# enoche/MMRec

Hardware: AMD Instinct MI355X
Metric: GCN-layer edges/sec (3-layer user-item CSR SpMM, d=64, fp32) (higher is better)
Workload: dtype f32

## Files before the change

### include/mmrec_hip.h

```cpp
#ifndef MMREC_HIP_H
#define MMREC_HIP_H

#include <stddef.h>
#include <stdint.h>

#ifdef __cplusplus
extern "C" {
#endif

#define MMREC_ABI_VERSION 16
#define MMREC_EMB_DIM 64

#define MMREC_ERR_BAD_ARG 10001
#define MMREC_ERR_UNSUPPORTED 10002

typedef void* mmrec_stream_t;

int mmrec_abi_version(void);
const char* mmrec_error_string(int err);

#ifndef MMREC_SPMM_CHUNK
#define MMREC_SPMM_CHUNK 512
#endif
#define MMREC_SPMM_LONG_ROW_DEFAULT 32

int mmrec_spmm_csr_f32(const int32_t* rowptr, const int32_t* colidx, const float* vals,
                       const float* X, float* Y, const float* Z, const float* acc_in, float* acc_out,
                       int32_t n_rows, int32_t d, float alpha, float beta, float acc_scale,
                       int32_t long_row_threshold, const int32_t* long_rows,
                       const int32_t* long_chunk_ptr, int32_t n_long, int32_t n_chunks,
                       float* partials, int32_t* long_tickets, mmrec_stream_t stream);

int mmrec_spmm_rows_f32(const int32_t* rowptr, const int32_t* colidx, const float* vals, const float* X,
                        const float* Z, int32_t z_compact, const int64_t* rows, int32_t n_list, int32_t d,
                        int32_t long_row_threshold, float* Y, mmrec_stream_t stream);
int mmrec_spmm_rows_any_f32(const int32_t* rowptr, const int32_t* colidx, const float* vals, const float* X,
                            const float* Z, int32_t z_compact, const int64_t* rows, int32_t n_list, int32_t d,
                            int32_t long_row_threshold, int32_t max_row_chunks, float* Y, mmrec_stream_t stream);
int mmrec_spmm_push_rows_f32(const int32_t* rowptr, const int32_t* colidx, const float* vals, const float* G,
                             float g_scale, const int64_t* rows, int32_t n_list, int32_t d, float* dX, float* dZ,
                             mmrec_stream_t stream);

int mmrec_spmm_csr_f32_layergcn(const int32_t* rowptr, const int32_t* colidx, const float* vals, const float* X,
                                float* Y, const float* ego, float* scaled, float* w, const float* acc_in,
                                float* acc_out, int32_t n_rows, int32_t d, int32_t long_row_threshold,
                                const int32_t* long_rows, const int32_t* long_chunk_ptr, int32_t n_long,
                                int32_t n_chunks, float* partials, int32_t* long_tickets, mmrec_stream_t stream);
int mmrec_spmm_csr_sched_f32(const int32_t* rowptr, const int32_t* colidx, const float* vals, const float* X, float* Y,
                             const float* Z, const float* acc_in, float* acc_out, int32_t n_rows, int32_t d, float alpha,
                             float beta, float acc_scale, int32_t long_row_threshold, const int32_t* long_rows,
                             const int32_t* long_chunk_ptr, int32_t n_long, int32_t n_chunks, float* partials,
                             int32_t* long_tickets, const int32_t* sched_row, const int32_t* sched_span,
                             const int32_t* sched_col, const float* sched_val, int32_t n_short, mmrec_stream_t stream);
int mmrec_spmm_csr_sched_f32_layergcn(const int32_t* rowptr, const int32_t* colidx, const float* vals, const float* X,
                                      float* Y, const float* ego, float* scaled, float* w, const float* acc_in,
                                      float* acc_out, int32_t n_rows, int32_t d, int32_t long_row_threshold,
                                      const int32_t* long_rows, const int32_t* long_chunk_ptr, int32_t n_long,
                                      int32_t n_chunks, float* partials, int32_t* long_tickets, const int32_t* sched_row,
                                      const int32_t* sched_span, const int32_t* sched_col, const float* sched_val,
                                      int32_t n_short, mmrec_stream_t stream);
int mmrec_spmm_row_keys(const int32_t* rowptr, const int32_t* colidx, const int32_t* col_degree, int32_t n_rows,
                        int32_t long_row_threshold, int32_t key_deg_max, int32_t* key, int32_t* key_degree,
                        mmrec_stream_t stream);
int mmrec_spmm_plan_count(const int32_t* rowptr_host, int32_t n_rows, int32_t long_row_threshold,
                          int32_t* n_long, int32_t* n_chunks);
int mmrec_spmm_plan_fill(const int32_t* rowptr_host, int32_t n_rows, int32_t long_row_threshold,
                         int32_t* long_rows, int32_t* long_chunk_ptr);

int mmrec_cos_scale_fwd_f32(const float* E, const float* Ego, float* Out, float* w, float* acc,
                            int32_t n_rows, int32_t d, mmrec_stream_t stream);
int mmrec_cos_scale_bwd_f32(const float* dOut, const float* E, const float* Ego, const float* w,
                            float* dE, float* dEgo_accum, int32_t n_rows, int32_t d,
                            mmrec_stream_t stream);

#define MMREC_BPR_LOGSIG 0
#define MMREC_BPR_GAMMA 1

size_t mmrec_bpr_workspace_bytes(int32_t batch);
int mmrec_bpr_fwd_f32(const float* U, const float* P, const float* N, const int64_t* users,
                      const int64_t* pos, const int64_t* neg, int32_t batch, int32_t d,
                      int32_t variant, float scale, float* loss_out, float* coef, void* workspace,
                      mmrec_stream_t stream);
int mmrec_bpr_bwd_f32(const float* U, const float* P, const float* N, const int64_t* users,
                      const int64_t* pos, const int64_t* neg, int32_t batch, int32_t d,
                      const float* coef, const float* grad_scalar, float scale, float* dU, float* dP,
                      float* dN, mmrec_stream_t stream);

int mmrec_bpr_dots_f32(const float* U, const float* P, const float* N, const int64_t* users,
                       const int64_t* pos, const int64_t* neg, int32_t batch, int32_t d, float* dots,
                       mmrec_stream_t stream);
int mmrec_bpr_loss_from_dots_f32(const float* dots, int32_t batch, int32_t variant, float scale,
                                 float* loss_out, float* coef, void* workspace, mmrec_stream_t stream);

int mmrec_gather_sqnorm_fwd_f32(const float* E, const int64_t* ids, int32_t batch, int32_t d,
                                float* out, void* workspace, mmrec_stream_t stream);
int mmrec_gather_scale_add_bwd_f32(const float* E, const int64_t* ids, int32_t batch, int32_t d,
                                   const float* coef_scalar, float* dE, mmrec_stream_t stream);
#define MMREC_ROWS_REG_MAX_TERMS 6
size_t mmrec_rows_reg_workspace_bytes(int32_t n_terms, int32_t max_batch);
int mmrec_rows_reg_fwd_f32(const float* const* E, const int64_t* const* ids, const int32_t* batch, int32_t n_terms, int32_t d,
                           int32_t mode, float scale, float* out, float* coef, void* workspace, mmrec_stream_t stream);
int mmrec_rows_reg_bwd_f32(const float* const* E, const int64_t* const* ids, const int32_t* batch, int32_t n_terms, int32_t d,
                           const float* coef, const float* g, float* const* dE, mmrec_stream_t stream);

#define MMREC_BPR_MAX_TERMS 4
size_t mmrec_bpr_multi_workspace_bytes(int32_t n_terms, int32_t batch);
int mmrec_bpr_multi_fwd_f32(const float* U, const int64_t* users, const float* const* I, const int64_t* const* pos,
                            const int64_t* const* neg, const float* w, int32_t n_terms, int32_t batch, int32_t d, int32_t variant,
                            float scale, float* total, float* losses, float* coef, void* workspace, mmrec_stream_t stream);
int mmrec_bpr_multi_bwd_f32(const float* U, const int64_t* users, const float* const* I, const int64_t* const* pos,
                            const int64_t* const* neg, const float* w, int32_t n_terms, int32_t batch, int32_t d, const float* coef,
                            const float* grad_scalar, float scale, float* dU, float* const* dI, mmrec_stream_t stream);

#define MMREC_COSINE_MAX_TERMS 8
size_t mmrec_cosine_multi_workspace_bytes(int32_t n_terms, int32_t max_batch);
int mmrec_cosine_multi_fwd_f32(const float* const* X, const int64_t* const* ix, const float* const* Y, const int64_t* const* iy,
                               const float* w, const int32_t* batch, int32_t n_terms, int32_t d, float* out, float* coef,
                               void* workspace, mmrec_stream_t stream);
int mmrec_cosine_multi_bwd_f32(const float* const* X, const int64_t* const* ix, const float* const* Y, const int64_t* const* iy,
                               const float* w, const int32_t* batch, int32_t n_terms, int32_t d, const float* coef,
                               const float* grad_scalar, float* const* dX, mmrec_stream_t stream);

int mmrec_row_normalize_fwd_f32(const float* X, int64_t n, int32_t d, float eps, float* Y, float* inv, mmrec_stream_t stream);
int mmrec_row_normalize_bwd_f32(const float* Y, const float* G, const float* inv, int64_t n, int32_t d, float* dX,
                                mmrec_stream_t stream);

int mmrec_cat_leaky_fwd_f32(const float* A, const float* B, const float* R, int64_t n, int32_t wa, int32_t wb, float slope,
                            float* out, mmrec_stream_t stream);
int mmrec_cat_leaky_bwd_f32(const float* A, const float* B, const float* dOut, int64_t n, int32_t wa, int32_t wb, float slope,
                            float* dA, float* dB, float* dR, mmrec_stream_t stream);


size_t mmrec_infonce_workspace_bytes(int32_t batch);
int mmrec_infonce_fwd_f32(const float* E1, const float* E2, const int64_t* ids, int32_t batch,
                          int32_t d, float tau, float* loss, void* workspace, mmrec_stream_t stream);
int mmrec_infonce_bwd_f32(const int64_t* ids, int32_t batch, int32_t d, float tau,
                          const float* grad_loss, float* dE1, float* dE2, void* workspace,
                          mmrec_stream_t stream);

size_t mmrec_linear_workspace_bytes(int32_t n, int32_t F, int32_t out);
int mmrec_linear_fwd_f32(const float* X, const float* W, const float* b, float* Y, int32_t n,
                         int32_t F, int32_t out, void* workspace, mmrec_stream_t stream);
int mmrec_linear_fwd_split_f32(const float* X, const float* W, const float* b, float* Y, int32_t n, int32_t F,
                               int32_t out, void* workspace, mmrec_stream_t stream);
size_t mmrec_linear_bwd_split_workspace_bytes(int32_t n, int32_t F, int32_t out);
int mmrec_linear_bwd_split_f32(const float* dY, const float* X, const float* W, float* dW, float* db, float* dX, int32_t n,
                               int32_t F, int32_t out, void* workspace, mmrec_stream_t stream);
int mmrec_linear_bwd_w_f32(const float* dY, const float* X, float* dW, float* db, int32_t n,
                           int32_t F, int32_t out, void* workspace, mmrec_stream_t stream);
int mmrec_linear_bwd_x_f32(const float* dY, const float* W, float* dX, int32_t n, int32_t F,
                           int32_t out, mmrec_stream_t stream);
size_t mmrec_linear_rows_workspace_bytes(int32_t n, int32_t F, int32_t out);
int mmrec_linear_rows_fwd_f32(const float* T, int64_t n_table, const int64_t* ids, const float* W, const float* b, float* Y,
                              int32_t n, int32_t F, int32_t out, int32_t split, void* workspace, mmrec_stream_t stream);
int mmrec_linear_rows_bwd_f32(const float* dY, const float* T, int64_t n_table, const int64_t* ids, const float* W, float* dW,
                              float* db, float* dX, int32_t n, int32_t F, int32_t out, void* workspace, mmrec_stream_t stream);
int mmrec_gemm_nt_f32(const float* A, const float* B, const float* bias, float* C, int32_t M, int32_t N,
                      int32_t K, int32_t ldc, mmrec_stream_t stream);

int mmrec_edge_dot_f32(const float* A, int64_t n_a, const float* B, int64_t n_b,
                       const int64_t* rows, const int64_t* cols, int64_t n_edges, int32_t d,
                       float* out, mmrec_stream_t stream);
int mmrec_edge_dot_bwd_f32(const float* g, const float* A, int64_t n_a, const float* B, int64_t n_b,
                           const int64_t* rows, const int64_t* cols, int64_t n_edges, int32_t d,
                           float* dA, float* dB, mmrec_stream_t stream);

int32_t mmrec_segment_softmax_group_max(void);
int mmrec_segment_softmax_f32(const int32_t* rowptr, int32_t n_rows, const int64_t* perm, const int32_t* long_rows,
                              int32_t n_long, const float* score, int64_t n_edges, float eps, float* out,
                              mmrec_stream_t stream);
int mmrec_segment_softmax_bwd_f32(const int32_t* rowptr, int32_t n_rows, const int64_t* perm, const int32_t* long_rows,
                                  int32_t n_long, const float* alpha, const float* g, int64_t n_edges, float* ds,
                                  mmrec_stream_t stream);

int32_t mmrec_edge_attention_group_max(void);
int mmrec_edge_attention_f32(const int32_t* rowptr, int32_t n_rows, const int32_t* colidx, const int64_t* perm,
                             const int32_t* long_rows, int32_t n_long, const float* Q, int64_t n_q, const float* KV,
                             int64_t n_kv, int32_t d, int64_t n_edges, float eps, float* Y, float* alpha,
                             mmrec_stream_t stream);

int mmrec_edge_attention_bwd_f32(const int32_t* rowptr, int32_t n_rows, const int32_t* colidx, const int64_t* perm,
                                 const int32_t* long_rows, int32_t n_long, const int32_t* rowptr_t, const int32_t* rowidx_t,
                                 const int64_t* perm_t, const int32_t* long_cols, int32_t n_long_t, const float* Q, int64_t n_q,
                                 const float* KV, int64_t n_kv, const float* Y, const float* alpha, const float* dY,
                                 const float* dAlpha, int32_t d, int64_t n_edges, float* ds, float* dQ, float* dKV,
                                 const float* dKV_base, mmrec_stream_t stream);

#define MMREC_TOPK_MAX 128
#define MMREC_TOPK_MAX_OTHER 64
#define MMREC_TOPK_NO_FILTER 1
size_t mmrec_topk_workspace_bytes(int32_t nq, int32_t nc, int32_t kd, int32_t k);
int mmrec_score_topk_f32(const float* Q, const float* C, int32_t nq, int32_t nc, int32_t kd,
                         const int32_t* mask_rowptr, const int32_t* mask_col, int32_t k,
                         int64_t* out_idx, float* out_val, void* workspace, int32_t flags,
                         mmrec_stream_t stream);
size_t mmrec_topk_prepared_bytes(int32_t nc, int32_t kd);
int mmrec_topk_prepare_f32(const float* C, int32_t nc, int32_t kd, void* prepared, mmrec_stream_t stream);
int mmrec_score_topk_prepared_f32(const float* Q, const float* C, const void* prepared, int32_t nq, int32_t nc,
                                  int32_t kd, const int32_t* mask_rowptr, const int32_t* mask_col, int32_t k,
                                  int64_t* out_idx, float* out_val, void* workspace, int32_t flags,
                                  mmrec_stream_t stream);
#define MMREC_TOPK_HINT_COLD 1
#define MMREC_TOPK_HINT_KEEP 2
int mmrec_score_topk_hinted_f32(const float* Q, const float* C, const void* prepared, int32_t nq, int32_t nc,
                                int32_t kd, const int32_t* mask_rowptr, const int32_t* mask_col, int32_t k,
                                int32_t* hint, int32_t hint_k, const int64_t* hint_rows,
                                int64_t* out_idx, float* out_val, void* workspace, int32_t* queue_counts,
                                int32_t flags, mmrec_stream_t stream);

int mmrec_scatter_add_rows_sorted_f32(const int64_t* order, const int64_t* ids, const float* rows, int32_t n, int32_t d,
                                      float* out, mmrec_stream_t stream);

int mmrec_degree_count_i32(const int64_t* ids, int64_t n, int32_t* counts, int32_t n_bins,
                           mmrec_stream_t stream);
int mmrec_edge_norm_f32(const int64_t* eu, const int64_t* ei, int64_t n_edges, const int32_t* deg_u,
                        const int32_t* deg_i, float* val, mmrec_stream_t stream);
int mmrec_bipartite_expand(const int64_t* eu, const int64_t* ei, const float* w, int64_t n_edges,
                           int32_t n_users, int32_t* rows, int32_t* cols, float* vals,
                           mmrec_stream_t stream);
size_t mmrec_coo_to_csr_workspace_bytes(int64_t nnz, int32_t n_rows);
int mmrec_coo_to_csr(const int32_t* rows, const int32_t* cols, const float* vals, int64_t nnz,
                     int32_t n_rows, int32_t* rowptr, int32_t* colidx, float* vals_out,
                     void* workspace, mmrec_stream_t stream);

int mmrec_sample_negatives_i64(const int64_t* users, int32_t batch, const int32_t* hist_rowptr,
                               const int32_t* hist_col, const int32_t* cand_items, int32_t n_cand,
                               uint64_t seed, uint64_t counter, int64_t* out_neg,
                               mmrec_stream_t stream);
int mmrec_topk_metrics_f64(const int64_t* topk_idx, int32_t n_users, int32_t k,
                           const int32_t* gt_rowptr, const int32_t* gt_col, const double* discount,
                           const double* idcg_cum, const int32_t* ks, int32_t n_ks, uint8_t* hit_out,
                           double* out_per_user, mmrec_stream_t stream);

int mmrec_adam_step_f32(float* p, const float* g, float* m, float* v, int64_t n, float lr, float beta1,
                        float beta2, float eps, float weight_decay, int64_t step,
                        mmrec_stream_t stream);

int mmrec_adam_prepare(int64_t* step_dev, const float* lr_dev, float beta1, float beta2, float* hyper_dev,
                       mmrec_stream_t stream);
int mmrec_adam_step_dev_f32(float* p, const float* g, float* m, float* v, int64_t n, const float* hyper_dev,
                            float beta1, float beta2, float eps, float weight_decay,
                            mmrec_stream_t stream);

int mmrec_adam_multi_step_f32(float* const* p, const float* const* g, float* const* m, float* const* v,
                              const int64_t* n, int32_t n_tensors, const float* lr, const int64_t* step,
                              float beta1, float beta2, float eps, float weight_decay, mmrec_stream_t stream);
int mmrec_adam_multi_step_dev_f32(float* const* p, const float* const* g, float* const* m, float* const* v,
                                  const int64_t* n, int32_t n_tensors, const float* hyper_dev, float beta1,
                                  float beta2, float eps, float weight_decay, mmrec_stream_t stream);

int mmrec_host_sample_negatives(uint32_t* mt_state, int32_t* mt_index, const int64_t* users, int32_t batch,
                                const int64_t* hist_rowptr, const int64_t* hist_items, const int64_t* all_items,
                                int32_t n_all_items, int64_t* out);

int mmrec_host_random_sample_range(uint32_t* mt_state, int32_t* mt_index, int32_t n, int32_t k, int64_t* out,
                                   int32_t* scratch);

size_t mmrec_cosine_workspace_bytes(int32_t batch);
int mmrec_cosine_fwd_f32(const float* X, const int64_t* ix, const float* Y, const int64_t* iy, int32_t batch, int32_t d,
                         float scale, float* out, float* coef, void* workspace, mmrec_stream_t stream);
int mmrec_cosine_bwd_f32(const float* X, const int64_t* ix, const float* Y, const int64_t* iy, int32_t batch, int32_t d,
                         const float* coef, const float* grad_scalar, float scale, float* dX, mmrec_stream_t stream);

#define MMREC_ADAM_ROWS_MAX_IDS 16000
int mmrec_adam_hist_set(float* hist, int32_t t, float lr, float beta1, float beta2, mmrec_stream_t stream);
int mmrec_adam_rows_owner(const int64_t* ids, int32_t n, int32_t* owner, mmrec_stream_t stream);
int mmrec_adam_rows_catchup_f32(float* p, float* m, float* v, const int64_t* ids, int32_t* owner, int32_t n_ids,
                                int32_t n_rows, int32_t F, int32_t* last_step, const float* hist, int32_t t_now,
                                float beta1, float beta2, float eps, float weight_decay, mmrec_stream_t stream);
int mmrec_adam_rows_step_f32(float* p, float* m, float* v, const int64_t* ids, int32_t* owner, const float* g,
                             int32_t n_ids, int32_t F, int32_t* last_step, int32_t t, float lr, float beta1,
                             float beta2, float eps, float weight_decay, int32_t presummed, mmrec_stream_t stream);
int mmrec_adam_hist_set_dev(float* hist, int32_t capacity, const int64_t* step_dev, const float* hyper_dev,
                            int32_t* overflow, mmrec_stream_t stream);
int mmrec_adam_rows_catchup_dev_f32(float* p, float* m, float* v, const int64_t* ids, int32_t* owner, int32_t n_ids,
                                    int32_t n_rows, int32_t F, int32_t* last_step, const float* hist, int32_t capacity,
                                    const int64_t* step_dev, float beta1, float beta2, float eps, float weight_decay,
                                    mmrec_stream_t stream);
int mmrec_adam_rows_step_dev_f32(float* p, float* m, float* v, const int64_t* ids, int32_t* owner, const float* g,
                                 int32_t n_ids, int32_t F, int32_t* last_step, int32_t capacity, const int64_t* step_dev,
                                 const float* hyper_dev, float beta1, float beta2, float eps, float weight_decay,
                                 int32_t presummed, mmrec_stream_t stream);
int mmrec_adam_rows_fastforward_f32(float* p, float* m, float* v, const int64_t* ids, int32_t* owner, int32_t n_ids,
                                    int32_t n_rows, int32_t F, int32_t* last_step, const float* hist, int32_t t_now,
                                    float beta1, float beta2, float eps, float weight_decay, mmrec_stream_t stream);
int mmrec_adam_rows_fastforward_dev_f32(float* p, float* m, float* v, const int64_t* ids, int32_t* owner, int32_t n_ids,
                                        int32_t n_rows, int32_t F, int32_t* last_step, const float* hist,
                                        int32_t capacity, const int64_t* step_dev, float beta1, float beta2, float eps,
                                        float weight_decay, mmrec_stream_t stream);

#ifdef __cplusplus
}
#endif
#endif
```

### mmrec_amd/_lib.py

```python
from __future__ import annotations

import ctypes
import os
from ctypes import c_char_p, c_float, c_int32, c_int64, c_size_t, c_uint64, c_void_p

import torch

_PKG = os.path.dirname(os.path.abspath(__file__))
LIB_PATH = os.environ.get("MMREC_HIP_LIB") or os.path.join(_PKG, "lib", "libmmrec_hip.so")
ABI_VERSION = 16

_P = c_void_p

SIGNATURES = {
    "mmrec_abi_version": (c_int32, []),
    "mmrec_error_string": (c_char_p, [c_int32]),
    "mmrec_spmm_csr_f32": (c_int32, [_P, _P, _P, _P, _P, _P, _P, _P, c_int32, c_int32, c_float,
                                     c_float, c_float, c_int32, _P, _P, c_int32, c_int32, _P, _P, _P]),
    "mmrec_spmm_csr_f32_layergcn": (c_int32, [_P, _P, _P, _P, _P, _P, _P, _P, _P, _P, c_int32, c_int32, c_int32,
                                              _P, _P, c_int32, c_int32, _P, _P, _P]),
    "mmrec_spmm_csr_sched_f32": (c_int32, [_P, _P, _P, _P, _P, _P, _P, _P, c_int32, c_int32, c_float,
                                           c_float, c_float, c_int32, _P, _P, c_int32, c_int32, _P, _P,
                                           _P, _P, _P, _P, c_int32, _P]),
    "mmrec_spmm_csr_sched_f32_layergcn": (c_int32, [_P, _P, _P, _P, _P, _P, _P, _P, _P, _P, c_int32, c_int32, c_int32,
                                                    _P, _P, c_int32, c_int32, _P, _P, _P, _P, _P, _P, c_int32, _P]),
    "mmrec_spmm_row_keys": (c_int32, [_P, _P, _P, c_int32, c_int32, c_int32, _P, _P, _P]),
    "mmrec_spmm_plan_count": (c_int32, [_P, c_int32, c_int32, _P, _P]),
    "mmrec_spmm_plan_fill": (c_int32, [_P, c_int32, c_int32, _P, _P]),
    "mmrec_cos_scale_fwd_f32": (c_int32, [_P, _P, _P, _P, _P, c_int32, c_int32, _P]),
    "mmrec_cos_scale_bwd_f32": (c_int32, [_P, _P, _P, _P, _P, _P, c_int32, c_int32, _P]),
    "mmrec_bpr_workspace_bytes": (c_size_t, [c_int32]),
    "mmrec_bpr_fwd_f32": (c_int32, [_P, _P, _P, _P, _P, _P, c_int32, c_int32, c_int32, c_float, _P,
                                    _P, _P, _P]),
    "mmrec_spmm_rows_f32": (c_int32, [_P, _P, _P, _P, _P, c_int32, _P, c_int32, c_int32, c_int32, _P, _P]),
    "mmrec_spmm_rows_any_f32": (c_int32, [_P, _P, _P, _P, _P, c_int32, _P, c_int32, c_int32, c_int32, c_int32, _P, _P]),
    "mmrec_spmm_push_rows_f32": (c_int32, [_P, _P, _P, _P, c_float, _P, c_int32, c_int32, _P, _P, _P]),
    "mmrec_bpr_dots_f32": (c_int32, [_P, _P, _P, _P, _P, _P, c_int32, c_int32, _P, _P]),
    "mmrec_bpr_loss_from_dots_f32": (c_int32, [_P, c_int32, c_int32, c_float, _P, _P, _P, _P]),
    "mmrec_bpr_bwd_f32": (c_int32, [_P, _P, _P, _P, _P, _P, c_int32, c_int32, _P, _P, c_float, _P, _P,
                                    _P, _P]),
    "mmrec_gather_sqnorm_fwd_f32": (c_int32, [_P, _P, c_int32, c_int32, _P, _P, _P]),
    "mmrec_gather_scale_add_bwd_f32": (c_int32, [_P, _P, c_int32, c_int32, _P, _P, _P]),
    "mmrec_infonce_workspace_bytes": (c_size_t, [c_int32]),
    "mmrec_infonce_fwd_f32": (c_int32, [_P, _P, _P, c_int32, c_int32, c_float, _P, _P, _P]),
    "mmrec_infonce_bwd_f32": (c_int32, [_P, c_int32, c_int32, c_float, _P, _P, _P, _P, _P]),
    "mmrec_linear_workspace_bytes": (c_size_t, [c_int32, c_int32, c_int32]),
    "mmrec_linear_fwd_f32": (c_int32, [_P, _P, _P, _P, c_int32, c_int32, c_int32, _P, _P]),
    "mmrec_linear_fwd_split_f32": (c_int32, [_P, _P, _P, _P, c_int32, c_int32, c_int32, _P, _P]),
    "mmrec_linear_bwd_split_workspace_bytes": (c_size_t, [c_int32, c_int32, c_int32]),
    "mmrec_linear_bwd_split_f32": (c_int32, [_P, _P, _P, _P, _P, _P, c_int32, c_int32, c_int32, _P, _P]),
    "mmrec_linear_bwd_w_f32": (c_int32, [_P, _P, _P, _P, c_int32, c_int32, c_int32, _P, _P]),
    "mmrec_linear_bwd_x_f32": (c_int32, [_P, _P, _P, c_int32, c_int32, c_int32, _P]),
    "mmrec_linear_rows_workspace_bytes": (c_size_t, [c_int32, c_int32, c_int32]),
    "mmrec_linear_rows_fwd_f32": (c_int32, [_P, c_int64, _P, _P, _P, _P, c_int32, c_int32, c_int32, c_int32, _P, _P]),
    "mmrec_linear_rows_bwd_f32": (c_int32, [_P, _P, c_int64, _P, _P, _P, _P, _P, c_int32, c_int32, c_int32, _P, _P]),
    "mmrec_edge_dot_f32": (c_int32, [_P, c_int64, _P, c_int64, _P, _P, c_int64, c_int32, _P, _P]),
    "mmrec_edge_dot_bwd_f32": (c_int32, [_P, _P, c_int64, _P, c_int64, _P, _P, c_int64, c_int32, _P, _P, _P]),
    "mmrec_segment_softmax_group_max": (c_int32, []),
    "mmrec_segment_softmax_f32": (c_int32, [_P, c_int32, _P, _P, c_int32, _P, c_int64, c_float, _P, _P]),
    "mmrec_segment_softmax_bwd_f32": (c_int32, [_P, c_int32, _P, _P, c_int32, _P, _P, c_int64, _P, _P]),
    "mmrec_edge_attention_group_max": (c_int32, []),
    "mmrec_edge_attention_f32": (c_int32, [_P, c_int32, _P, _P, _P, c_int32, _P, c_int64, _P, c_int64, c_int32, c_int64, c_float,
                                           _P, _P, _P]),
    "mmrec_edge_attention_bwd_f32": (c_int32, [_P, c_int32, _P, _P, _P, c_int32, _P, _P, _P, _P, c_int32, _P, c_int64, _P, c_int64,
                                               _P, _P, _P, _P, c_int32, c_int64, _P, _P, _P, _P, _P]),
    "mmrec_gemm_nt_f32": (c_int32, [_P, _P, _P, _P, c_int32, c_int32, c_int32, c_int32, _P]),
    "mmrec_topk_workspace_bytes": (c_size_t, [c_int32, c_int32, c_int32, c_int32]),
    "mmrec_score_topk_f32": (c_int32, [_P, _P, c_int32, c_int32, c_int32, _P, _P, c_int32, _P, _P, _P,
                                       c_int32, _P]),
    "mmrec_scatter_add_rows_sorted_f32": (c_int32, [_P, _P, _P, c_int32, c_int32, _P, _P]),
    "mmrec_topk_prepared_bytes": (c_size_t, [c_int32, c_int32]),
    "mmrec_topk_prepare_f32": (c_int32, [_P, c_int32, c_int32, _P, _P]),
    "mmrec_score_topk_prepared_f32": (c_int32, [_P, _P, _P, c_int32, c_int32, c_int32, _P, _P, c_int32, _P, _P, _P,
                                                c_int32, _P]),
    "mmrec_score_topk_hinted_f32": (c_int32, [_P, _P, _P, c_int32, c_int32, c_int32, _P, _P, c_int32, _P, c_int32, _P,
                                              _P, _P, _P, _P, c_int32, _P]),
    "mmrec_degree_count_i32": (c_int32, [_P, c_int64, _P, c_int32, _P]),
    "mmrec_edge_norm_f32": (c_int32, [_P, _P, c_int64, _P, _P, _P, _P]),
    "mmrec_bipartite_expand": (c_int32, [_P, _P, _P, c_int64, c_int32, _P, _P, _P, _P]),
    "mmrec_coo_to_csr_workspace_bytes": (c_size_t, [c_int64, c_int32]),
    "mmrec_coo_to_csr": (c_int32, [_P, _P, _P, c_int64, c_int32, _P, _P, _P, _P, _P]),
    "mmrec_sample_negatives_i64": (c_int32, [_P, c_int32, _P, _P, _P, c_int32, c_uint64, c_uint64, _P, _P]),
    "mmrec_topk_metrics_f64": (c_int32, [_P, c_int32, c_int32, _P, _P, _P, _P, _P, c_int32, _P, _P, _P]),
    "mmrec_adam_step_f32": (c_int32, [_P, _P, _P, _P, c_int64, c_float, c_float, c_float, c_float, c_float,
                                      c_int64, _P]),
    "mmrec_adam_prepare": (c_int32, [_P, _P, c_float, c_float, _P, _P]),
    "mmrec_adam_step_dev_f32": (c_int32, [_P, _P, _P, _P, c_int64, _P, c_float, c_float, c_float, c_float, _P]),
    "mmrec_adam_multi_step_f32": (c_int32, [_P, _P, _P, _P, _P, c_int32, _P, _P, c_float, c_float, c_float,
                                            c_float, _P]),
    "mmrec_adam_multi_step_dev_f32": (c_int32, [_P, _P, _P, _P, _P, c_int32, _P, c_float, c_float, c_float,
                                                c_float, _P]),
    "mmrec_host_sample_negatives": (c_int32, [_P, _P, _P, c_int32, _P, _P, _P, c_int32, _P]),
    "mmrec_host_random_sample_range": (c_int32, [_P, _P, c_int32, c_int32, _P, _P]),
    "mmrec_cosine_workspace_bytes": (c_size_t, [c_int32]),
    "mmrec_cosine_fwd_f32": (c_int32, [_P, _P, _P, _P, c_int32, c_int32, c_float, _P, _P, _P, _P]),
    "mmrec_cosine_bwd_f32": (c_int32, [_P, _P, _P, _P, c_int32, c_int32, _P, _P, c_float, _P, _P]),
    "mmrec_bpr_multi_workspace_bytes": (c_size_t, [c_int32, c_int32]),
    "mmrec_bpr_multi_fwd_f32": (c_int32, [_P, _P, _P, _P, _P, _P, c_int32, c_int32, c_int32, c_int32, c_float, _P, _P, _P, _P, _P]),
    "mmrec_bpr_multi_bwd_f32": (c_int32, [_P, _P, _P, _P, _P, _P, c_int32, c_int32, c_int32, _P, _P, c_float, _P, _P, _P]),
    "mmrec_cosine_multi_workspace_bytes": (c_size_t, [c_int32, c_int32]),
    "mmrec_cosine_multi_fwd_f32": (c_int32, [_P, _P, _P, _P, _P, _P, c_int32, c_int32, _P, _P, _P, _P]),
    "mmrec_cosine_multi_bwd_f32": (c_int32, [_P, _P, _P, _P, _P, _P, c_int32, c_int32, _P, _P, _P, _P]),
    "mmrec_row_normalize_fwd_f32": (c_int32, [_P, c_int64, c_int32, c_float, _P, _P, _P]),
    "mmrec_row_normalize_bwd_f32": (c_int32, [_P, _P, _P, c_int64, c_int32, _P, _P]),
    "mmrec_cat_leaky_fwd_f32": (c_int32, [_P, _P, _P, c_int64, c_int32, c_int32, c_float, _P, _P]),
    "mmrec_cat_leaky_bwd_f32": (c_int32, [_P, _P, _P, c_int64, c_int32, c_int32, c_float, _P, _P, _P, _P]),
    "mmrec_rows_reg_workspace_bytes": (c_size_t, [c_int32, c_int32]),
    "mmrec_rows_reg_fwd_f32": (c_int32, [_P, _P, _P, c_int32, c_int32, c_int32, c_float, _P, _P, _P, _P]),
    "mmrec_rows_reg_bwd_f32": (c_int32, [_P, _P, _P, c_int32, c_int32, _P, _P, _P, _P]),
    "mmrec_adam_hist_set": (c_int32, [_P, c_int32, c_float, c_float, c_float, _P]),
    "mmrec_adam_rows_owner": (c_int32, [_P, c_int32, _P, _P]),
    "mmrec_adam_rows_catchup_f32": (c_int32, [_P, _P, _P, _P, _P, c_int32, c_int32, c_int32, _P, _P, c_int32, c_float,
                                              c_float, c_float, c_float, _P]),
    "mmrec_adam_rows_step_f32": (c_int32, [_P, _P, _P, _P, _P, _P, c_int32, c_int32, _P, c_int32, c_float, c_float,
                                           c_float, c_float, c_float, c_int32, _P]),
    "mmrec_adam_hist_set_dev": (c_int32, [_P, c_int32, _P, _P, _P, _P]),
    "mmrec_adam_rows_catchup_dev_f32": (c_int32, [_P, _P, _P, _P, _P, c_int32, c_int32, c_int32, _P, _P, c_int32, _P, c_float,
                                                  c_float, c_float, c_float, _P]),
    "mmrec_adam_rows_step_dev_f32": (c_int32, [_P, _P, _P, _P, _P, _P, c_int32, c_int32, _P, c_int32, _P, _P, c_float, c_float,
                                               c_float, c_float, c_int32, _P]),
    "mmrec_adam_rows_fastforward_f32": (c_int32, [_P, _P, _P, _P, _P, c_int32, c_int32, c_int32, _P, _P, c_int32, c_float,
                                                  c_float, c_float, c_float, _P]),
    "mmrec_adam_rows_fastforward_dev_f32": (c_int32, [_P, _P, _P, _P, _P, c_int32, c_int32, c_int32, _P, _P, c_int32, _P,
                                                      c_float, c_float, c_float, c_float, _P]),
}

_lib = None


class MMRecHipError(RuntimeError):
    pass


def load():
    global _lib
    if _lib is not None:
        return _lib
    if not os.path.exists(LIB_PATH):
        raise MMRecHipError(
            "libmmrec_hip.so not found at %s: run `python -m mmrec_amd.build`; there is no CPU or "
            "eager fallback for the hot path" % LIB_PATH)
    lib = ctypes.CDLL(LIB_PATH)
    for name, (res, args) in SIGNATURES.items():
        fn = getattr(lib, name)
        fn.restype = res
        fn.argtypes = args
    got = lib.mmrec_abi_version()
    if got != ABI_VERSION:
        raise MMRecHipError("libmmrec_hip.so ABI %d != expected %d: rebuild" % (got, ABI_VERSION))
    _lib = lib
    return lib


def check(err: int, what: str):
    if err != 0:
        msg = load().mmrec_error_string(int(err))
        raise MMRecHipError("%s failed: [%d] %s" % (what, err, msg.decode() if msg else "?"))
```

### mmrec_amd/csrc/spmm.hip

```cpp
#include "common.h"
#include "spmm_narrow.h"

#ifndef MMREC_SPMM_RPG
#define MMREC_SPMM_RPG(n_rows) ((n_rows) <= (1 << 18) ? 1 : 4)
#endif

namespace {

__device__ __forceinline__ void st_coherent(float4* p, float4 v) {
    unsigned long long* q = reinterpret_cast<unsigned long long*>(p);
    const unsigned long long lo = ((unsigned long long)__float_as_uint(v.y) << 32) | __float_as_uint(v.x);
    const unsigned long long hi = ((unsigned long long)__float_as_uint(v.w) << 32) | __float_as_uint(v.z);
    __hip_atomic_store(q, lo, __ATOMIC_RELAXED, __HIP_MEMORY_SCOPE_AGENT);
    __hip_atomic_store(q + 1, hi, __ATOMIC_RELAXED, __HIP_MEMORY_SCOPE_AGENT);
}
__device__ __forceinline__ float4 ld_coherent(const float4* p) {
    unsigned long long* q = reinterpret_cast<unsigned long long*>(const_cast<float4*>(p));
    const unsigned long long lo = __hip_atomic_load(q, __ATOMIC_RELAXED, __HIP_MEMORY_SCOPE_AGENT);
    const unsigned long long hi = __hip_atomic_load(q + 1, __ATOMIC_RELAXED, __HIP_MEMORY_SCOPE_AGENT);
    return make_float4(__uint_as_float((unsigned)lo), __uint_as_float((unsigned)(lo >> 32)),
                       __uint_as_float((unsigned)hi), __uint_as_float((unsigned)(hi >> 32)));
}

struct RowEpilogue {
    const float* Z;
    float* Y;
    const float* acc_in;
    float* acc_out;
    float alpha, beta, acc_scale;
    const float* ego;
    float* scaled;
    float* w_out;
};

struct RowSchedule {
    const int32_t* row;
    const int2* span;
    const int32_t* col;
    const float* val;
    int n_short;
};

template <int DCH, bool LG>
__device__ __forceinline__ void store_row(const RowEpilogue& ep, int row, int lane16, const float4 (&sum)[DCH]) {
    if (DCH == 1 && LG) {
        const size_t off = (size_t)row * 16 + lane16;
        const float4 y = f4_scale(ep.alpha, sum[0]);
        const float4 g = reinterpret_cast<const float4*>(ep.ego)[off];
        const float dot = row16_sum(f4_dot(y, g));
        const float ne = fmaxf(sqrtf(row16_sum(f4_dot(y, y))), 1e-8f);
        const float ng = fmaxf(sqrtf(row16_sum(f4_dot(g, g))), 1e-8f);
        const float w = dot / (ne * ng);
        const float4 o = f4_scale(w, y);
        if (ep.Y) reinterpret_cast<float4*>(ep.Y)[off] = y;
        reinterpret_cast<float4*>(ep.scaled)[off] = o;
        if (lane16 == 0) ep.w_out[row] = w;
        if (ep.acc_out)
            reinterpret_cast<float4*>(ep.acc_out)[off] =
                ep.acc_in ? f4_add(reinterpret_cast<const float4*>(ep.acc_in)[off], o) : o;
        return;
    }
#pragma unroll
    for (int ch = 0; ch < DCH; ++ch) {
        const size_t off = (size_t)row * (16 * DCH) + ch * 16 + lane16;
        float4 y = f4_scale(ep.alpha, sum[ch]);
        if (ep.Z) y = f4_fma(ep.beta, reinterpret_cast<const float4*>(ep.Z)[off], y);
        if (ep.Y) reinterpret_cast<float4*>(ep.Y)[off] = y;
        if (ep.acc_out) {
            const float4 a = reinterpret_cast<const float4*>(ep.acc_in)[off];
            reinterpret_cast<float4*>(ep.acc_out)[off] = f4_scale(ep.acc_scale, f4_add(a, y));
        }
    }
}

template <int DCH>
__device__ __forceinline__ void gather_span(const int32_t* __restrict__ colidx,
                                            const float* __restrict__ vals,
                                            const float4* __restrict__ X4, int s, int e, int lane16,
                                            float4 (&acc)[DCH]) {
    constexpr int NB = DCH == 1 ? 8 : (DCH <= 2 ? 4 : (DCH <= 4 ? 2 : 1));
    for (int base = s; base < e; base += 16) {
        const int k = base + lane16;
        int c = 0;
        float v = 0.f;
        if (k < e) {
            c = colidx[k];
            v = vals[k];
        }
        const int cnt = min(16, e - base);
        for (int j0 = 0; j0 < cnt; j0 += NB) {
            float4 x[NB][DCH];
            float vv[NB];
#pragma unroll
            for (int u = 0; u < NB; ++u) {
                const int j = j0 + u;
                const int cj = __shfl(c, j, 16);
                vv[u] = __shfl(v, j, 16);
#pragma unroll
                for (int ch = 0; ch < DCH; ++ch)
                    x[u][ch] = (j < cnt) ? X4[(size_t)cj * (16 * DCH) + ch * 16 + lane16] : f4_zero();
            }
#pragma unroll
            for (int u = 0; u < NB; ++u)
#pragma unroll
                for (int ch = 0; ch < DCH; ++ch) acc[ch] = f4_fma(vv[u], x[u][ch], acc[ch]);
        }
    }
}

template <int DCH, bool COHERENT, bool LG>
__device__ __forceinline__ void reduce_long_row(const float* __restrict__ partials, int c0, int c1, int row,
                                                const RowEpilogue& ep, float4 (*red)[16 * DCH]) {
    const int lane16 = threadIdx.x & 15, g = threadIdx.x >> 4;
#pragma unroll
    for (int ch = 0; ch < DCH; ++ch) {
        float4 t = f4_zero();
        for (int c = c0 + g; c < c1; c += 16) {
            const float4* src = reinterpret_cast<const float4*>(partials) + (size_t)c * (16 * DCH) + ch * 16 + lane16;
            t = f4_add(t, COHERENT ? ld_coherent(src) : *src);
        }
        red[g][ch * 16 + lane16] = t;
    }
    __syncthreads();
    if (g == 0) {
        float4 r[DCH];
#pragma unroll
        for (int ch = 0; ch < DCH; ++ch) {
            r[ch] = red[0][ch * 16 + lane16];
#pragma unroll
            for (int k = 1; k < 16; ++k) r[ch] = f4_add(r[ch], red[k][ch * 16 + lane16]);
        }
        store_row<DCH, LG>(ep, row, lane16, r);
    }
}

template <int DCH, bool LG, bool SCHED>
__global__ __launch_bounds__(256) void spmm_rows_kernel(
    const int32_t* __restrict__ rowptr, const int32_t* __restrict__ colidx,
    const float* __restrict__ vals, const float* __restrict__ X, RowEpilogue ep, int n_rows,
    int long_t, int rows_per_group, const int32_t* __restrict__ long_rows,
    const int32_t* __restrict__ long_chunk_ptr, int n_long, int n_chunks,
    float* __restrict__ partials, int32_t* __restrict__ tickets, RowSchedule sched) {
    __shared__ float4 red[16][16 * DCH];
    __shared__ int s_last;
    const int lane16 = threadIdx.x & 15;
    const int g = threadIdx.x >> 4;
    const float4* X4 = reinterpret_cast<const float4*>(X);
    if ((int)blockIdx.x < n_chunks) {
        const int chunk = blockIdx.x;
        int lo = 0, hi = n_long;
        while (hi - lo > 1) {
            const int mid = (lo + hi) >> 1;
            if (long_chunk_ptr[mid] <= chunk) lo = mid; else hi = mid;
        }
        const int row = long_rows[lo];
        const int cs = rowptr[row] + (chunk - long_chunk_ptr[lo]) * MMREC_SPMM_CHUNK;
        const int ce = min(cs + MMREC_SPMM_CHUNK, rowptr[row + 1]);
        float4 acc[DCH];
#pragma unroll
        for (int ch = 0; ch < DCH; ++ch) acc[ch] = f4_zero();
        for (int base = cs + g * 16; base < ce; base += 256)
            gather_span<DCH>(colidx, vals, X4, base, min(base + 16, ce), lane16, acc);
#pragma unroll
        for (int ch = 0; ch < DCH; ++ch) red[g][ch * 16 + lane16] = acc[ch];
        __syncthreads();
        if (g == 0) {
            float4 t[DCH];
#pragma unroll
            for (int ch = 0; ch < DCH; ++ch) {
                t[ch] = red[0][ch * 16 + lane16];
#pragma unroll
                for (int i = 1; i < 16; ++i) t[ch] = f4_add(t[ch], red[i][ch * 16 + lane16]);
            }
            if (long_chunk_ptr[lo + 1] - long_chunk_ptr[lo] == 1) {
                store_row<DCH, LG>(ep, row, lane16, t);
            } else {
#pragma unroll
                for (int ch = 0; ch < DCH; ++ch) {
                    float4* dst = reinterpret_cast<float4*>(partials) + (size_t)chunk * (16 * DCH) + ch * 16 + lane16;
                    if (tickets) st_coherent(dst, t[ch]); else *dst = t[ch];
                }
            }
        }
        const int c0 = long_chunk_ptr[lo], c1 = long_chunk_ptr[lo + 1];
        if (!tickets || c1 - c0 == 1) return;
        if (threadIdx.x < 64) {
            __atomic_signal_fence(__ATOMIC_SEQ_CST);
            __builtin_amdgcn_s_waitcnt(0);
            __atomic_signal_fence(__ATOMIC_SEQ_CST);
            __builtin_amdgcn_fence(__ATOMIC_RELEASE, "workgroup");
            if (threadIdx.x == 0)
                s_last = __hip_atomic_fetch_add(tickets + lo, 1, __ATOMIC_RELAXED, __HIP_MEMORY_SCOPE_AGENT) == c1 - c0 - 1;
        }
        __syncthreads();
        if (!s_last) return;
        __builtin_amdgcn_fence(__ATOMIC_ACQUIRE, "workgroup");
        reduce_long_row<DCH, true, LG>(partials, c0, c1, row, ep, red);
        if (threadIdx.x == 0) __hip_atomic_store(tickets + lo, 0, __ATOMIC_RELAXED, __HIP_MEMORY_SCOPE_AGENT);
        return;
    }
    if (SCHED) {
        const int slot0 = ((int)blockIdx.x - n_chunks) * 16 * rows_per_group + g;
#pragma unroll 1
        for (int i = 0; i < rows_per_group; ++i) {
            const int slot = slot0 + i * 16;
            if (slot >= sched.n_short) break;
            const int row = sched.row[slot];
            const int2 se = sched.span[slot];
            float4 acc[DCH];
#pragma unroll
            for (int ch = 0; ch < DCH; ++ch) acc[ch] = f4_zero();
            gather_span<DCH>(sched.col, sched.val, X4, se.x, se.y, lane16, acc);
            store_row<DCH, LG>(ep, row, lane16, acc);
        }
        return;
    }
    const int row0 = ((int)blockIdx.x - n_chunks) * 16 * rows_per_group + g;
#pragma unroll 1
    for (int i = 0; i < rows_per_group; ++i) {
        const int row = row0 + i * 16;
        if (row >= n_rows) break;
        const int s = rowptr[row], e = rowptr[row + 1];
        if (e - s > long_t) continue;
        float4 acc[DCH];
#pragma unroll
        for (int ch = 0; ch < DCH; ++ch) acc[ch] = f4_zero();
        gather_span<DCH>(colidx, vals, X4, s, e, lane16, acc);
        store_row<DCH, LG>(ep, row, lane16, acc);
    }
}

template <int DCH, bool LG>
__global__ __launch_bounds__(256) void spmm_long_reduce_kernel(
    const int32_t* __restrict__ long_rows, const int32_t* __restrict__ long_chunk_ptr, int n_long,
    const float* __restrict__ partials, RowEpilogue ep) {
    __shared__ float4 red[16][16 * DCH];
    const int i = blockIdx.x;
    const int c0 = long_chunk_ptr[i], c1 = long_chunk_ptr[i + 1];
    if (c1 - c0 <= 1) return;
    reduce_long_row<DCH, false, LG>(partials, c0, c1, long_rows[i], ep, red);
}

template <int DCH, bool LG = false, bool SCHED = false>
void launch_spmm(hipStream_t s, int blocks, int nch, const int32_t* rowptr, const int32_t* colidx,
                 const float* vals, const float* X, const RowEpilogue& ep, int n_rows, int long_t,
                 int rows_per_group, const int32_t* long_rows, const int32_t* long_chunk_ptr, int n_long,
                 float* partials, int32_t* tickets, const RowSchedule& sched = RowSchedule{}) {
    if (blocks + nch > 0)
        hipLaunchKernelGGL((spmm_rows_kernel<DCH, LG, SCHED>), dim3(blocks + nch), dim3(256), 0, s, rowptr, colidx, vals, X,
                           ep, n_rows, long_t, rows_per_group, long_rows, long_chunk_ptr, n_long, nch, partials, tickets,
                           sched);
    if (!tickets && n_long > 0 && nch > n_long)
        hipLaunchKernelGGL((spmm_long_reduce_kernel<DCH, LG>), dim3(n_long), dim3(256), 0, s, long_rows,
                           long_chunk_ptr, n_long, partials, ep);
}

__global__ __launch_bounds__(256) void cos_scale_fwd_kernel(const float* __restrict__ E,
                                                            const float* __restrict__ Ego,
                                                            float* __restrict__ Out,
                                                            float* __restrict__ W,
                                                            float* __restrict__ acc, int n_rows) {
    const int lane16 = threadIdx.x & 15;
    const int row = blockIdx.x * 16 + (threadIdx.x >> 4);
    if (row >= n_rows) return;
    const size_t off = (size_t)row * 16 + lane16;
    const float4 e = reinterpret_cast<const float4*>(E)[off];
    const float4 g = reinterpret_cast<const float4*>(Ego)[off];
    const float dot = row16_sum(f4_dot(e, g));
    const float ne = fmaxf(sqrtf(row16_sum(f4_dot(e, e))), 1e-8f);
    const float ng = fmaxf(sqrtf(row16_sum(f4_dot(g, g))), 1e-8f);
    const float w = dot / (ne * ng);
    const float4 o = f4_scale(w, e);
    reinterpret_cast<float4*>(Out)[off] = o;
    if (lane16 == 0) W[row] = w;
    if (acc) reinterpret_cast<float4*>(acc)[off] = f4_add(reinterpret_cast<float4*>(acc)[off], o);
}

__global__ __launch_bounds__(256) void cos_scale_bwd_kernel(
    const float* __restrict__ dOut, const float* __restrict__ E, const float* __restrict__ Ego,
    const float* __restrict__ W, float* __restrict__ dE, float* __restrict__ dEgo, int n_rows) {
    const int lane16 = threadIdx.x & 15;
    const int row = blockIdx.x * 16 + (threadIdx.x >> 4);
    if (row >= n_rows) return;
    const size_t off = (size_t)row * 16 + lane16;
    const float4 e = reinterpret_cast<const float4*>(E)[off];
    const float4 g = reinterpret_cast<const float4*>(Ego)[off];
    const float4 d = reinterpret_cast<const float4*>(dOut)[off];
    const float w = W[row];
    const float ne_raw = sqrtf(row16_sum(f4_dot(e, e)));
    const float ng_raw = sqrtf(row16_sum(f4_dot(g, g)));
    const float ne = fmaxf(ne_raw, 1e-8f), ng = fmaxf(ng_raw, 1e-8f);
    const float dw = row16_sum(f4_dot(d, e));
    const float inv = 1.0f / (ne * ng);
    const float ce = (ne_raw > 1e-8f) ? w / (ne * ne) : 0.f;
    const float cg = (ng_raw > 1e-8f) ? w / (ng * ng) : 0.f;
    float4 de = f4_scale(w, d);
    de = f4_fma(dw * inv, g, de);
    de = f4_fma(-dw * ce, e, de);
    reinterpret_cast<float4*>(dE)[off] = de;
    float4 dg = reinterpret_cast<float4*>(dEgo)[off];
    dg = f4_fma(dw * inv, e, dg);
    dg = f4_fma(-dw * cg, g, dg);
    reinterpret_cast<float4*>(dEgo)[off] = dg;
}

__global__ __launch_bounds__(256) void spmm_row_keys_kernel(const int32_t* __restrict__ rowptr,
                                                            const int32_t* __restrict__ colidx,
                                                            const int32_t* __restrict__ col_degree, int n_rows, int long_t,
                                                            int deg_max, int32_t* __restrict__ key,
                                                            int32_t* __restrict__ key_degree) {
    const int lane16 = threadIdx.x & 15;
    const int row = blockIdx.x * 16 + (threadIdx.x >> 4);
    if (row >= n_rows) return;
    const int s = rowptr[row], e = rowptr[row + 1];
    int bd = 0, bp = INT32_MAX, bc = -1;
    if (e - s <= long_t)
        for (int k = s + lane16; k < e; k += 16) {
            const int c = colidx[k];
            const int dg = col_degree[c];
            if (dg <= deg_max && dg > bd) {
                bd = dg;
                bp = k;
                bc = c;
            }
        }
#pragma unroll
    for (int m = 8; m > 0; m >>= 1) {
        const int od = __shfl_xor(bd, m, 16), op = __shfl_xor(bp, m, 16), oc = __shfl_xor(bc, m, 16);
        if (od > bd || (od == bd && op < bp)) {
            bd = od;
            bp = op;
            bc = oc;
        }
    }
    if (lane16 == 0) {
        key[row] = bc;
        key_degree[row] = bd;
    }
}

}

extern "C" int mmrec_spmm_csr_f32(const int32_t* rowptr, const int32_t* colidx, const float* vals,
                                  const float* X, float* Y, const float* Z, const float* acc_in,
                                  float* acc_out, int32_t n_rows, int32_t d, float alpha, float beta,
                                  float acc_scale, int32_t long_row_threshold,
                                  const int32_t* long_rows, const int32_t* long_chunk_ptr,
                                  int32_t n_long, int32_t n_chunks, float* partials, int32_t* long_tickets,
                                  mmrec_stream_t stream) {
    const bool narrow = d == 8 || d == 16 || d == 32;
    if (!narrow && (d <= 0 || d % MMREC_EMB_DIM || d / MMREC_EMB_DIM > 6)) return MMREC_ERR_UNSUPPORTED;
    if (n_rows < 0 || n_long < 0 || n_chunks < 0 || long_row_threshold < 0) return MMREC_ERR_BAD_ARG;
    if (n_rows == 0) return 0;
    if (!rowptr || !X || (!Y && !acc_out)) return MMREC_ERR_BAD_ARG;
    if (acc_out && !acc_in) return MMREC_ERR_BAD_ARG;
    if (n_long > 0 && (!long_rows || !long_chunk_ptr || !partials || n_chunks <= 0))
        return MMREC_ERR_BAD_ARG;
    if (Y == X || acc_out == X) return MMREC_ERR_BAD_ARG;
    if (narrow)
        return spmm_narrow_launch(rowptr, colidx, vals, X, Y, Z, acc_in, acc_out, n_rows, d, alpha, beta, acc_scale,
                                  n_long > 0 ? long_row_threshold : INT32_MAX, long_rows, long_chunk_ptr, n_long,
                                  n_long > 0 ? n_chunks : 0, partials, mmrec_stream(stream));
    RowEpilogue ep{Z, Y, acc_in, acc_out, alpha, Z ? beta : 0.f, acc_scale, nullptr, nullptr, nullptr};
    hipStream_t s = mmrec_stream(stream);
    const int rows_per_group = MMREC_SPMM_RPG(n_rows);
    const int blocks = (n_rows + 16 * rows_per_group - 1) / (16 * rows_per_group);
    const int long_t = n_long > 0 ? long_row_threshold : INT32_MAX;
    const int nch = n_long > 0 ? n_chunks : 0;
    int32_t* tickets = n_long > 0 ? long_tickets : nullptr;
#define MMREC_SPMM_CASE(D)                                                                               \
    case D:                                                                                              \
        launch_spmm<D>(s, blocks, nch, rowptr, colidx, vals, X, ep, n_rows, long_t, rows_per_group,      \
                       long_rows, long_chunk_ptr, n_long, partials, tickets);                            \
        break;
    switch (d / MMREC_EMB_DIM) {
        MMREC_SPMM_CASE(1) MMREC_SPMM_CASE(2) MMREC_SPMM_CASE(3) MMREC_SPMM_CASE(4) MMREC_SPMM_CASE(5)
        MMREC_SPMM_CASE(6)
    }
#undef MMREC_SPMM_CASE
    MMREC_RETURN_LAUNCH_STATUS();
}

extern "C" int mmrec_spmm_rows_f32(const int32_t* rowptr, const int32_t* colidx, const float* vals, const float* X,
                                   const float* Z, int32_t z_compact, const int64_t* rows, int32_t n_list, int32_t d,
                                   int32_t long_row_threshold, float* Y, mmrec_stream_t stream) {
    if (d != 8 && d != 16 && d != 32 && d != 64) return MMREC_ERR_UNSUPPORTED;
    if (n_list < 0 || long_row_threshold < 0) return MMREC_ERR_BAD_ARG;
    if (n_list == 0) return 0;
    if (!rowptr || !X || !rows || !Y || Y == X) return MMREC_ERR_BAD_ARG;
    return spmm_pull_rows_launch(rowptr, colidx, vals, X, Z, z_compact, rows, n_list, d, long_row_threshold, Y, mmrec_stream(stream));
}

extern "C" int mmrec_spmm_rows_any_f32(const int32_t* rowptr, const int32_t* colidx, const float* vals, const float* X,
                                       const float* Z, int32_t z_compact, const int64_t* rows, int32_t n_list, int32_t d,
                                       int32_t long_row_threshold, int32_t max_row_chunks, float* Y, mmrec_stream_t stream) {
    if (d != 8 && d != 16 && d != 32 && d != 64) return MMREC_ERR_UNSUPPORTED;
    if (n_list < 0 || long_row_threshold < 0 || max_row_chunks < 1) return MMREC_ERR_BAD_ARG;
    if (n_list == 0) return 0;
    if (!rowptr || !X || !rows || !Y || Y == X) return MMREC_ERR_BAD_ARG;
    return spmm_pull_rows_launch(rowptr, colidx, vals, X, Z, z_compact, rows, n_list, d, long_row_threshold, Y, mmrec_stream(stream),
                                 max_row_chunks);
}

extern "C" int mmrec_spmm_push_rows_f32(const int32_t* rowptr, const int32_t* colidx, const float* vals, const float* G,
                                        float g_scale, const int64_t* rows, int32_t n_list, int32_t d, float* dX, float* dZ,
                                        mmrec_stream_t stream) {
    if (d != 8 && d != 16 && d != 32 && d != 64) return MMREC_ERR_UNSUPPORTED;
    if (n_list < 0) return MMREC_ERR_BAD_ARG;
    if (n_list == 0) return 0;
    if (!rowptr || !G || !rows || (!dX && !dZ)) return MMREC_ERR_BAD_ARG;
    return spmm_push_rows_launch(rowptr, colidx, vals, G, g_scale, rows, n_list, d, dX, dZ, mmrec_stream(stream));
}

extern "C" int mmrec_spmm_csr_f32_layergcn(const int32_t* rowptr, const int32_t* colidx, const float* vals,
                                           const float* X, float* Y, const float* ego, float* scaled, float* w,
                                           const float* acc_in, float* acc_out, int32_t n_rows, int32_t d,
                                           int32_t long_row_threshold, const int32_t* long_rows,
                                           const int32_t* long_chunk_ptr, int32_t n_long, int32_t n_chunks,
                                           float* partials, int32_t* long_tickets, mmrec_stream_t stream) {
    if (d != MMREC_EMB_DIM) return MMREC_ERR_UNSUPPORTED;
    if (n_rows < 0 || n_long < 0 || n_chunks < 0 || long_row_threshold < 0) return MMREC_ERR_BAD_ARG;
    if (n_rows == 0) return 0;
    if (!rowptr || !X || !ego || !scaled || !w) return MMREC_ERR_BAD_ARG;
    if (n_long > 0 && (!long_rows || !long_chunk_ptr || !partials || n_chunks <= 0)) return MMREC_ERR_BAD_ARG;
    if (Y == X || scaled == X || acc_out == X) return MMREC_ERR_BAD_ARG;
    RowEpilogue ep{nullptr, Y, acc_in, acc_out, 1.f, 0.f, 1.f, ego, scaled, w};
    hipStream_t s = mmrec_stream(stream);
    const int rows_per_group = MMREC_SPMM_RPG(n_rows);
    const int blocks = (n_rows + 16 * rows_per_group - 1) / (16 * rows_per_group);
    const int long_t = n_long > 0 ? long_row_threshold : INT32_MAX;
    const int nch = n_long > 0 ? n_chunks : 0;
    int32_t* tickets = n_long > 0 ? long_tickets : nullptr;
    launch_spmm<1, true>(s, blocks, nch, rowptr, colidx, vals, X, ep, n_rows, long_t, rows_per_group, long_rows,
                         long_chunk_ptr, n_long, partials, tickets);
    MMREC_RETURN_LAUNCH_STATUS();
}

namespace {
bool sched_args_ok(const int32_t* sched_row, const int32_t* sched_span, const int32_t* sched_col, const float* sched_val,
                   int32_t n_short, int32_t n_rows) {
    if (n_short < 0 || n_short > n_rows) return false;
    return n_short == 0 || (sched_row && sched_span && sched_col && sched_val);
}
}

extern "C" int mmrec_spmm_csr_sched_f32(const int32_t* rowptr, const int32_t* colidx, const float* vals,
                                        const float* X, float* Y, const float* Z, const float* acc_in,
                                        float* acc_out, int32_t n_rows, int32_t d, float alpha, float beta,
                                        float acc_scale, int32_t long_row_threshold,
                                        const int32_t* long_rows, const int32_t* long_chunk_ptr,
                                        int32_t n_long, int32_t n_chunks, float* partials, int32_t* long_tickets,
                                        const int32_t* sched_row, const int32_t* sched_span, const int32_t* sched_col,
                                        const float* sched_val, int32_t n_short, mmrec_stream_t stream) {
    if (d <= 0 || d % MMREC_EMB_DIM || d / MMREC_EMB_DIM > 6) return MMREC_ERR_UNSUPPORTED;
    if (n_rows < 0 || n_long < 0 || n_chunks < 0 || long_row_threshold < 0) return MMREC_ERR_BAD_ARG;
    if (n_rows == 0) return 0;
    if (!rowptr || !X || (!Y && !acc_out)) return MMREC_ERR_BAD_ARG;
    if (acc_out && !acc_in) return MMREC_ERR_BAD_ARG;
    if (n_long > 0 && (!long_rows || !long_chunk_ptr || !partials || n_chunks <= 0))
        return MMREC_ERR_BAD_ARG;
    if (!sched_args_ok(sched_row, sched_span, sched_col, sched_val, n_short, n_rows)) return MMREC_ERR_BAD_ARG;
    if (Y == X || acc_out == X) return MMREC_ERR_BAD_ARG;
    RowEpilogue ep{Z, Y, acc_in, acc_out, alpha, Z ? beta : 0.f, acc_scale, nullptr, nullptr, nullptr};
    const RowSchedule sched{sched_row, reinterpret_cast<const int2*>(sched_span), sched_col, sched_val, n_short};
    hipStream_t s = mmrec_stream(stream);
    const int rows_per_group = MMREC_SPMM_RPG(n_rows);
    const int blocks = (n_short + 16 * rows_per_group - 1) / (16 * rows_per_group);
    const int long_t = n_long > 0 ? long_row_threshold : INT32_MAX;
    const int nch = n_long > 0 ? n_chunks : 0;
    int32_t* tickets = n_long > 0 ? long_tickets : nullptr;
#define MMREC_SPMM_CASE(D)                                                                                      \
    case D:                                                                                                     \
        launch_spmm<D, false, true>(s, blocks, nch, rowptr, colidx, vals, X, ep, n_rows, long_t, rows_per_group, \
                                    long_rows, long_chunk_ptr, n_long, partials, tickets, sched);               \
        break;
    switch (d / MMREC_EMB_DIM) {
        MMREC_SPMM_CASE(1) MMREC_SPMM_CASE(2) MMREC_SPMM_CASE(3) MMREC_SPMM_CASE(4) MMREC_SPMM_CASE(5)
        MMREC_SPMM_CASE(6)
    }
#undef MMREC_SPMM_CASE
    MMREC_RETURN_LAUNCH_STATUS();
}

extern "C" int mmrec_spmm_csr_sched_f32_layergcn(const int32_t* rowptr, const int32_t* colidx, const float* vals,
                                                 const float* X, float* Y, const float* ego, float* scaled, float* w,
                                                 const float* acc_in, float* acc_out, int32_t n_rows, int32_t d,
                                                 int32_t long_row_threshold, const int32_t* long_rows,
                                                 const int32_t* long_chunk_ptr, int32_t n_long, int32_t n_chunks,
                                                 float* partials, int32_t* long_tickets, const int32_t* sched_row,
                                                 const int32_t* sched_span, const int32_t* sched_col,
                                                 const float* sched_val, int32_t n_short, mmrec_stream_t stream) {
    if (d != MMREC_EMB_DIM) return MMREC_ERR_UNSUPPORTED;
    if (n_rows < 0 || n_long < 0 || n_chunks < 0 || long_row_threshold < 0) return MMREC_ERR_BAD_ARG;
    if (n_rows == 0) return 0;
    if (!rowptr || !X || !ego || !scaled || !w) return MMREC_ERR_BAD_ARG;
    if (n_long > 0 && (!long_rows || !long_chunk_ptr || !partials || n_chunks <= 0)) return MMREC_ERR_BAD_ARG;
    if (!sched_args_ok(sched_row, sched_span, sched_col, sched_val, n_short, n_rows)) return MMREC_ERR_BAD_ARG;
    if (Y == X || scaled == X || acc_out == X) return MMREC_ERR_BAD_ARG;
    RowEpilogue ep{nullptr, Y, acc_in, acc_out, 1.f, 0.f, 1.f, ego, scaled, w};
    const RowSchedule sched{sched_row, reinterpret_cast<const int2*>(sched_span), sched_col, sched_val, n_short};
    hipStream_t s = mmrec_stream(stream);
    const int rows_per_group = MMREC_SPMM_RPG(n_rows);
    const int blocks = (n_short + 16 * rows_per_group - 1) / (16 * rows_per_group);
    const int long_t = n_long > 0 ? long_row_threshold : INT32_MAX;
    const int nch = n_long > 0 ? n_chunks : 0;
    int32_t* tickets = n_long > 0 ? long_tickets : nullptr;
    launch_spmm<1, true, true>(s, blocks, nch, rowptr, colidx, vals, X, ep, n_rows, long_t, rows_per_group, long_rows,
                               long_chunk_ptr, n_long, partials, tickets, sched);
    MMREC_RETURN_LAUNCH_STATUS();
}

extern "C" int mmrec_spmm_row_keys(const int32_t* rowptr, const int32_t* colidx, const int32_t* col_degree,
                                   int32_t n_rows, int32_t long_row_threshold, int32_t key_deg_max, int32_t* key,
                                   int32_t* key_degree, mmrec_stream_t stream) {
    if (n_rows < 0 || long_row_threshold < 0 || key_deg_max < 0) return MMREC_ERR_BAD_ARG;
    if (n_rows == 0) return 0;
    if (!rowptr || !colidx || !col_degree || !key || !key_degree) return MMREC_ERR_BAD_ARG;
    hipLaunchKernelGGL(spmm_row_keys_kernel, dim3((n_rows + 15) / 16), dim3(256), 0, mmrec_stream(stream), rowptr, colidx,
                       col_degree, n_rows, long_row_threshold, key_deg_max, key, key_degree);
    MMREC_RETURN_LAUNCH_STATUS();
}

extern "C" int mmrec_spmm_plan_count(const int32_t* rowptr_host, int32_t n_rows,
                                     int32_t long_row_threshold, int32_t* n_long, int32_t* n_chunks) {
    if (!rowptr_host || !n_long || !n_chunks || n_rows < 0) return MMREC_ERR_BAD_ARG;
    int32_t nl = 0, nc = 0;
    for (int32_t r = 0; r < n_rows; ++r) {
        const int32_t deg = rowptr_host[r + 1] - rowptr_host[r];
        if (deg > long_row_threshold) {
            ++nl;
            nc += (deg + MMREC_SPMM_CHUNK - 1) / MMREC_SPMM_CHUNK;
        }
    }
    *n_long = nl;
    *n_chunks = nc;
    return 0;
}

extern "C" int mmrec_spmm_plan_fill(const int32_t* rowptr_host, int32_t n_rows,
                                    int32_t long_row_threshold, int32_t* long_rows,
                                    int32_t* long_chunk_ptr) {
    if (!rowptr_host || !long_rows || !long_chunk_ptr || n_rows < 0) return MMREC_ERR_BAD_ARG;
    int32_t nl = 0, nc = 0;
    for (int32_t r = 0; r < n_rows; ++r) {
        const int32_t deg = rowptr_host[r + 1] - rowptr_host[r];
        if (deg > long_row_threshold) {
            long_rows[nl] = r;
            long_chunk_ptr[nl] = nc;
            ++nl;
            nc += (deg + MMREC_SPMM_CHUNK - 1) / MMREC_SPMM_CHUNK;
        }
    }
    long_chunk_ptr[nl] = nc;
    return 0;
}

extern "C" int mmrec_cos_scale_fwd_f32(const float* E, const float* Ego, float* Out, float* w,
                                       float* acc, int32_t n_rows, int32_t d, mmrec_stream_t stream) {
    if (d != MMREC_EMB_DIM) return MMREC_ERR_UNSUPPORTED;
    if (n_rows < 0 || (n_rows > 0 && (!E || !Ego || !Out || !w))) return MMREC_ERR_BAD_ARG;
    if (n_rows == 0) return 0;
    hipLaunchKernelGGL(cos_scale_fwd_kernel, dim3((n_rows + 15) / 16), dim3(256), 0,
                       mmrec_stream(stream), E, Ego, Out, w, acc, n_rows);
    MMREC_RETURN_LAUNCH_STATUS();
}

extern "C" int mmrec_cos_scale_bwd_f32(const float* dOut, const float* E, const float* Ego,
                                       const float* w, float* dE, float* dEgo_accum, int32_t n_rows,
                                       int32_t d, mmrec_stream_t stream) {
    if (d != MMREC_EMB_DIM) return MMREC_ERR_UNSUPPORTED;
    if (n_rows < 0 || (n_rows > 0 && (!dOut || !E || !Ego || !w || !dE || !dEgo_accum)))
        return MMREC_ERR_BAD_ARG;
    if (n_rows == 0) return 0;
    hipLaunchKernelGGL(cos_scale_bwd_kernel, dim3((n_rows + 15) / 16), dim3(256), 0,
                       mmrec_stream(stream), dOut, E, Ego, w, dE, dEgo_accum, n_rows);
    MMREC_RETURN_LAUNCH_STATUS();
}
```

### mmrec_amd/hip_ops.py

```python
from __future__ import annotations

import ctypes

import numpy as np
import torch

from . import _lib

EMB_DIM = 64
LINEAR_F16X3_DEFAULT = True
LINEAR_F16X3 = LINEAR_F16X3_DEFAULT
SLICE_WIDTHS = (8, 16, 32)
SPMM_CHUNK = 512
LONG_ROW_DEFAULT = None


def default_long_row_threshold(n_cols):
    import os
    forced = os.environ.get("MMREC_LONG_ROW_THRESHOLD")
    if forced:
        return int(forced)
    return 16 if n_cols <= (1 << 18) else 32


ROW_SCHEDULE_MIN_COLS = 1 << 18
SPMM_KEY_DEG_MAX = 128


def spmm_key_deg_max():
    import os
    forced = os.environ.get("MMREC_SPMM_KEY_DEG_MAX")
    return int(forced) if forced else SPMM_KEY_DEG_MAX


TOPK_MAX = 128
BPR_LOGSIG, BPR_GAMMA = 0, 1

DETERMINISTIC_DEFAULT = False
DETERMINISTIC = DETERMINISTIC_DEFAULT
_TORCH_DET_BY_US = False


def set_deterministic(flag=True):
    global DETERMINISTIC, _TORCH_DET_BY_US
    DETERMINISTIC = bool(flag)
    if DETERMINISTIC and not torch.are_deterministic_algorithms_enabled():
        torch.use_deterministic_algorithms(True, warn_only=True)
        _TORCH_DET_BY_US = True
    elif not DETERMINISTIC and _TORCH_DET_BY_US:
        torch.use_deterministic_algorithms(False)
        _TORCH_DET_BY_US = False


def scatter_add_rows(ids, rows, out):
    lib = _lib.load()
    _chk(ids, torch.int64, "ids", 1)
    rows, out = _chk(rows.contiguous(), torch.float32, "rows", 2), _chk(out, torch.float32, "out", 2)
    order = torch.sort(ids, stable=True)[1]
    _lib.check(lib.mmrec_scatter_add_rows_sorted_f32(_p(order), _p(ids), _p(rows), ids.numel(), rows.shape[1], _p(out),
                                                     _stream()), "scatter_add_rows_sorted")
    return out


def _p(t):
    return None if t is None else ctypes.c_void_p(t.data_ptr())


def _stream():
    return ctypes.c_void_p(torch.cuda.current_stream().cuda_stream)


def _chk(t, dtype, name, dim=None):
    if not isinstance(t, torch.Tensor) or not t.is_cuda:
        raise _lib.MMRecHipError("%s must be a device tensor (the hot path has no CPU fallback)" % name)
    if t.dtype != dtype:
        raise _lib.MMRecHipError("%s must be %s, got %s" % (name, dtype, t.dtype))
    if not t.is_contiguous():
        raise _lib.MMRecHipError("%s must be contiguous" % name)
    if dim is not None and t.dim() != dim:
        raise _lib.MMRecHipError("%s must be %d-d" % (name, dim))
    return t


def _ws(nbytes, device):
    return torch.empty(max(int(nbytes), 16), dtype=torch.uint8, device=device)


class CsrGraph:

    def __init__(self, rowptr, colidx, vals, n_rows, n_cols, symmetric=False,
                 long_row_threshold=LONG_ROW_DEFAULT, rowptr_host=None, row_schedule=None):
        self.rowptr = _chk(rowptr, torch.int32, "rowptr", 1)
        self.colidx = _chk(colidx, torch.int32, "colidx", 1)
        self.vals = _chk(vals, torch.float32, "vals", 1)
        self.n_rows, self.n_cols = int(n_rows), int(n_cols)
        self.nnz = int(colidx.numel())
        self.symmetric = bool(symmetric)
        self.long_row_threshold = int(default_long_row_threshold(self.n_cols) if long_row_threshold is None
                                      else long_row_threshold)
        self._t = self if symmetric else None
        self.row_schedule = bool(self.n_cols > ROW_SCHEDULE_MIN_COLS if row_schedule is None else row_schedule)
        self._plan(rowptr_host)

    def _plan(self, rowptr_host):
        lib = _lib.load()
        rp = rowptr_host if rowptr_host is not None else self.rowptr.cpu().numpy()
        rp = np.ascontiguousarray(rp, dtype=np.int32)
        self.rowptr_host = rp
        n_long, n_chunks = ctypes.c_int32(0), ctypes.c_int32(0)
        _lib.check(lib.mmrec_spmm_plan_count(rp.ctypes.data_as(ctypes.c_void_p), self.n_rows,
                                             self.long_row_threshold, ctypes.byref(n_long),
                                             ctypes.byref(n_chunks)), "spmm_plan_count")
        self.n_long, self.n_chunks = n_long.value, n_chunks.value
        dev = self.rowptr.device
        if self.n_long > 0:
            lr = np.empty(self.n_long, dtype=np.int32)
            cp = np.empty(self.n_long + 1, dtype=np.int32)
            _lib.check(lib.mmrec_spmm_plan_fill(rp.ctypes.data_as(ctypes.c_void_p), self.n_rows,
                                                self.long_row_threshold,
                                                lr.ctypes.data_as(ctypes.c_void_p),
                                                cp.ctypes.data_as(ctypes.c_void_p)), "spmm_plan_fill")
            self.long_rows = torch.from_numpy(lr).to(dev)
            self.long_chunk_ptr = torch.from_numpy(cp).to(dev)
            self.max_row_chunks = int(np.diff(cp).max())
            self.long_tickets = torch.zeros(self.n_long, dtype=torch.int32, device=dev)
        else:
            self.long_rows = self.long_chunk_ptr = self.long_tickets = None
            self.max_row_chunks = 1
        self._partials = {}
        self.sched = None
        if self.row_schedule:
            self._plan_schedule()

    def _plan_schedule(self):
        lib = _lib.load()
        dev, n = self.rowptr.device, self.n_rows
        deg = (self.rowptr[1:] - self.rowptr[:-1])
        short = torch.nonzero(deg <= self.long_row_threshold).squeeze(1)
        key = torch.full((n,), -1, dtype=torch.int32, device=dev)
        kdeg = torch.zeros(n, dtype=torch.int32, device=dev)
        if self.nnz > 0 and n > 0:
            if self.symmetric and self.n_cols == n:
                coldeg = deg.contiguous()
            else:
                coldeg = torch.bincount(self.colidx, minlength=self.n_cols).to(torch.int32)
            _lib.check(lib.mmrec_spmm_row_keys(_p(self.rowptr), _p(self.colidx), _p(coldeg), n, self.long_row_threshold,
                                               spmm_key_deg_max(), _p(key), _p(kdeg), _stream()), "spmm_row_keys")
        self.row_key, self.row_key_degree = key, kdeg
        k, kd, dg = key[short].long(), kdeg[short].long(), deg[short].long()
        first = self.colidx[self.rowptr[:-1][short].long().clamp_(max=max(self.nnz - 1, 0))].long() if self.nnz > 0 else k
        ref = torch.where(k >= 0, k, torch.where(dg > 0, first, torch.full_like(k, -1)))
        band = (ref <= short).long()
        comp = (band << 62) | (((1 << 31) - 1 - kd) << 31) | k.clamp(min=0)
        order = torch.sort(comp, stable=True)[1]
        rows = short[order]
        lens = dg[order]
        end = torch.cumsum(lens, 0)
        begin = end - lens
        total = int(end[-1].item()) if rows.numel() else 0
        src0 = self.rowptr[:-1].long()[rows]
        pos = torch.arange(total, dtype=torch.int64, device=dev) + torch.repeat_interleave(src0 - begin, lens, output_size=total)
        self.sched = {
            "row": rows.to(torch.int32).contiguous(),
            "span": torch.stack([begin, end], 1).to(torch.int32).contiguous(),
            "col": self.colidx.index_select(0, pos) if total else torch.zeros(1, dtype=torch.int32, device=dev),
            "val": self.vals.index_select(0, pos) if total else torch.zeros(1, dtype=torch.float32, device=dev),
            "n_short": int(rows.numel()),
            "vals_of": self.vals,
        }

    def scheduled(self, d):
        sc = self.sched
        return sc if sc is not None and d % EMB_DIM == 0 and sc["vals_of"] is self.vals else None

    def schedule_bytes(self):
        return 0 if self.sched is None else sum(self.sched[k].numel() * self.sched[k].element_size() for k in ("row", "span", "col", "val"))

    def checked(self, rc, what):
        try:
            _lib.check(rc, what)
        except _lib.MMRecHipError:
            if self.long_tickets is not None:
                try:
                    self.long_tickets.zero_()
                except RuntimeError:
                    pass
            raise

    def partials_for(self, d):
        if self.n_long == 0:
            return None
        if d not in self._partials:
            self._partials[d] = torch.empty(self.n_chunks * d, dtype=torch.float32, device=self.rowptr.device)
        return self._partials[d]

    @classmethod
    def from_coo_host(cls, idx, val, n_rows, n_cols, device, symmetric=False, **kw):
        idx = np.asarray(idx, dtype=np.int64)
        val = np.asarray(val, dtype=np.float32)
        order = np.argsort(idx[0], kind="stable")
        rowptr = np.zeros(n_rows + 1, dtype=np.int64)
        np.cumsum(np.bincount(idx[0], minlength=n_rows), out=rowptr[1:])
        rp = rowptr.astype(np.int32)
        return cls(torch.from_numpy(rp).to(device),
                   torch.from_numpy(idx[1][order].astype(np.int32)).to(device),
                   torch.from_numpy(val[order]).to(device), n_rows, n_cols, symmetric=symmetric,
                   rowptr_host=rp, **kw)

    @classmethod
    def from_coo_device(cls, rows, cols, vals, n_rows, n_cols, symmetric=False, **kw):
        lib = _lib.load()
        _chk(rows, torch.int32, "rows", 1), _chk(cols, torch.int32, "cols", 1)
        _chk(vals, torch.float32, "vals", 1)
        nnz, dev = rows.numel(), rows.device
        rowptr = torch.empty(n_rows + 1, dtype=torch.int32, device=dev)
        colidx = torch.empty(nnz, dtype=torch.int32, device=dev)
        vout = torch.empty(nnz, dtype=torch.float32, device=dev)
        ws = _ws(lib.mmrec_coo_to_csr_workspace_bytes(nnz, n_rows), dev)
        _lib.check(lib.mmrec_coo_to_csr(_p(rows), _p(cols), _p(vals), nnz, n_rows, _p(rowptr),
                                        _p(colidx), _p(vout), _p(ws), _stream()), "coo_to_csr")
        return cls(rowptr, colidx, vout, n_rows, n_cols, symmetric=symmetric, **kw)

    def to_coo_host(self):
        rp = self.rowptr_host.astype(np.int64)
        rows = np.repeat(np.arange(self.n_rows, dtype=np.int64), np.diff(rp))
        return np.stack([rows, self.colidx.cpu().numpy().astype(np.int64)]), self.vals.cpu().numpy()

    def transpose(self):
        if self._t is None:
            idx, val = self.to_coo_host()
            self._t = CsrGraph.from_coo_host(idx[::-1], val, self.n_cols, self.n_rows,
                                             self.rowptr.device,
                                             long_row_threshold=self.long_row_threshold)
            self._t._t = self
        return self._t

    def row_block(self, r0, r1):
        rp = self.rowptr_host.astype(np.int64)
        s, e = int(rp[r0]), int(rp[r1])
        rph = (rp[r0:r1 + 1] - s).astype(np.int32)
        dev = self.rowptr.device
        return CsrGraph(torch.from_numpy(rph).to(dev), self.colidx[s:e].contiguous(),
                        self.vals[s:e].contiguous(), r1 - r0, self.n_cols,
                        long_row_threshold=self.long_row_threshold, rowptr_host=rph, row_schedule=self.row_schedule)


def _mode_labels(rows, lab_c, n_rows, n_labels):
    key = rows.astype(np.int64) * n_labels + lab_c
    key.sort()
    start = np.flatnonzero(np.concatenate([[True], key[1:] != key[:-1]]))
    cnt = np.diff(np.concatenate([start, [key.shape[0]]]))
    k = key[start]
    r, lab = k // n_labels, k % n_labels
    o = np.lexsort((lab, -cnt, r))
    r_s = r[o]
    first = np.concatenate([[True], r_s[1:] != r_s[:-1]])
    out = np.full(n_rows, -1, dtype=np.int64)
    out[r_s[first]] = lab[o][first]
    return out


def _mode_labels_device(rows, lab_c, n_rows, n_labels):
    key, _ = torch.sort(rows * n_labels + lab_c)
    uk, cnt = torch.unique_consecutive(key, return_counts=True)
    r, lab = torch.div(uk, n_labels, rounding_mode='floor'), uk % n_labels
    cmax = int(cnt.max().item()) + 1
    if n_rows * cmax * n_labels >= 2 ** 62:
        raise OverflowError("label-propagation key does not fit 63 bits")
    k2, _ = torch.sort(r * (cmax * n_labels) + (cmax - cnt) * n_labels + lab)
    r2 = torch.div(k2, cmax * n_labels, rounding_mode='floor')
    first = torch.ones_like(r2, dtype=torch.bool)
    first[1:] = r2[1:] != r2[:-1]
    out = torch.full((n_rows,), -1, dtype=torch.int64, device=rows.device)
    out[r2[first]] = (k2 % n_labels)[first]
    return out


def locality_order(rowptr_host, colidx_host, n, how, n_left=None, iters=4, device=None):
    rp = np.asarray(rowptr_host, dtype=np.int64)
    deg = np.diff(rp)
    ci = np.asarray(colidx_host, dtype=np.int64)
    if how == "degree":
        order = np.argsort(-deg, kind="stable")
    elif how == "rcm":
        import scipy.sparse as sp
        from scipy.sparse.csgraph import reverse_cuthill_mckee
        a = sp.csr_matrix((np.ones(ci.shape[0], dtype=np.int8), ci.astype(np.int32), rp.astype(np.int32)), shape=(n, n))
        order = np.asarray(reverse_cuthill_mckee(a, symmetric_mode=True), dtype=np.int64)
    elif how == "community" and device is not None and torch.device(device).type == "cuda":
        dev = torch.device(device)
        rows = torch.repeat_interleave(torch.arange(n, dtype=torch.int64, device=dev), torch.from_numpy(deg).to(dev))
        cols = torch.from_numpy(ci).to(dev)
        lab = torch.arange(n, dtype=torch.int64, device=dev)
        sides = [None] if not n_left else [rows < n_left, rows >= n_left]
        for _ in range(int(iters)):
            for side in sides:
                r_s, c_s = (rows, cols) if side is None else (rows[side], cols[side])
                new = _mode_labels_device(r_s, lab[c_s], n, n)
                lab = torch.where(new >= 0, new, lab)
        order = torch.sort(lab, stable=True)[1].cpu().numpy()
    elif how == "community":
        rows = np.repeat(np.arange(n, dtype=np.int64), deg)
        lab = np.arange(n, dtype=np.int64)
        sides = [slice(None)] if not n_left else [rows < n_left, rows >= n_left]
        for _ in range(int(iters)):
            for side in sides:
                new = _mode_labels(rows[side], lab[ci[side]], n, n)
                lab = np.where(new >= 0, new, lab)
        order = np.lexsort((np.arange(n), lab))
    else:
        raise ValueError("reorder must be 'degree', 'rcm' or 'community', got %r" % (how,))
    perm = np.empty(n, dtype=np.int64)
    perm[order] = np.arange(n, dtype=np.int64)
    return perm


class PermutedGraph:

    def __init__(self, g: CsrGraph, reorder, n_left=None):
        if g.n_rows != g.n_cols:
            raise _lib.MMRecHipError("PermutedGraph needs a square graph")
        dev, n = g.rowptr.device, g.n_rows
        idx, val = g.to_coo_host()
        perm = locality_order(g.rowptr_host, idx[1], n, reorder, n_left=n_left)
        self.base, self.reorder = g, reorder
        self.perm = torch.from_numpy(perm).to(dev)
        inv = np.empty(n, dtype=np.int64)
        inv[perm] = np.arange(n, dtype=np.int64)
        self.inv = torch.from_numpy(inv).to(dev)
        self.graph = CsrGraph.from_coo_host(np.stack([perm[idx[0]], perm[idx[1]]]), val, n, n, dev, symmetric=g.symmetric,
                                            long_row_threshold=g.long_row_threshold)
        self.n_rows = self.n_cols = n
        self.nnz = g.nnz

    def to_new(self, X):
        return X.index_select(0, self.inv)

    def to_old(self, Xp):
        return Xp.index_select(0, self.perm)


def spmm_raw(g: CsrGraph, X, Y=None, Z=None, acc_in=None, acc_out=None, alpha=1.0, beta=1.0,
             acc_scale=1.0):
    lib = _lib.load()
    _chk(X, torch.float32, "X", 2)
    d = X.shape[1]
    if (d not in SLICE_WIDTHS and (d % EMB_DIM or d > 6 * EMB_DIM)) or X.shape[0] < g.n_cols:
        raise _lib.MMRecHipError("X must be [>=%d, 64*k <= 384 (or a feature slice of 8 / 16 / 32 columns)], got %s" %
                                 (g.n_cols, tuple(X.shape)))
    for t, nm in ((Y, "Y"), (Z, "Z"), (acc_in, "acc_in"), (acc_out, "acc_out")):
        if t is not None:
            _chk(t, torch.float32, nm, 2)
            if t.shape[0] < g.n_rows or t.shape[1] != d:
                raise _lib.MMRecHipError("%s must be [>=%d, %d]" % (nm, g.n_rows, d))
    sc = g.scheduled(d)
    if sc is not None:
        g.checked(lib.mmrec_spmm_csr_sched_f32(_p(g.rowptr), _p(g.colidx), _p(g.vals), _p(X), _p(Y), _p(Z),
                                               _p(acc_in), _p(acc_out), g.n_rows, d, float(alpha),
                                               float(beta), float(acc_scale), g.long_row_threshold,
                                               _p(g.long_rows), _p(g.long_chunk_ptr), g.n_long, g.n_chunks,
                                               _p(g.partials_for(d)), _p(g.long_tickets), _p(sc["row"]), _p(sc["span"]),
                                               _p(sc["col"]), _p(sc["val"]), sc["n_short"], _stream()), "spmm_csr_sched_f32")
        return Y if Y is not None else acc_out
    g.checked(lib.mmrec_spmm_csr_f32(_p(g.rowptr), _p(g.colidx), _p(g.vals), _p(X), _p(Y), _p(Z),
                                     _p(acc_in), _p(acc_out), g.n_rows, d, float(alpha),
                                     float(beta), float(acc_scale), g.long_row_threshold,
                                     _p(g.long_rows), _p(g.long_chunk_ptr), g.n_long, g.n_chunks,
                                     _p(g.partials_for(d)), _p(g.long_tickets), _stream()), "spmm_csr_f32")
    return Y if Y is not None else acc_out


ROWS_MAX_CHUNKS = 480


def rows_servable(g: CsrGraph, d):
    if d not in SLICE_WIDTHS + (EMB_DIM,):
        return False
    return g.n_chunks == g.n_long or (d == EMB_DIM and g.max_row_chunks <= ROWS_MAX_CHUNKS)


def spmm_rows_raw(g: CsrGraph, X, rows, Z=None, z_compact=False):
    lib = _lib.load()
    _chk(X, torch.float32, "X", 2), _chk(rows, torch.int64, "rows", 1)
    d = X.shape[1]
    if not rows_servable(g, d) or X.shape[0] < g.n_cols:
        raise _lib.MMRecHipError("spmm_rows: graph with multi-chunk rows, or X not [>=%d, 8 / 16 / 32 / 64]" % g.n_cols)
    if Z is not None and (_chk(Z, torch.float32, "Z", 2).shape[0] < (rows.numel() if z_compact else g.n_rows) or Z.shape[1] != d):
        raise _lib.MMRecHipError("Z must be [>=%d, %d]" % (rows.numel() if z_compact else g.n_rows, d))
    Y = torch.empty(rows.numel(), d, dtype=torch.float32, device=X.device)
    long_t = g.long_row_threshold if g.n_long > 0 else 2 ** 31 - 1
    if g.n_chunks == g.n_long:
        _lib.check(lib.mmrec_spmm_rows_f32(_p(g.rowptr), _p(g.colidx), _p(g.vals), _p(X), _p(Z), 1 if z_compact else 0, _p(rows),
                                           rows.numel(), d, long_t, _p(Y), _stream()), "spmm_rows_f32")
    else:
        _lib.check(lib.mmrec_spmm_rows_any_f32(_p(g.rowptr), _p(g.colidx), _p(g.vals), _p(X), _p(Z), 1 if z_compact else 0, _p(rows),
                                               rows.numel(), d, long_t, g.max_row_chunks, _p(Y), _stream()), "spmm_rows_any_f32")
    return Y


def spmm_push_rows_raw(g: CsrGraph, G, rows, dX=None, dZ=None, scale=1.0):
    lib = _lib.load()
    _chk(G, torch.float32, "G", 2), _chk(rows, torch.int64, "rows", 1)
    d = G.shape[1]
    if G.shape[0] != rows.numel() or d not in SLICE_WIDTHS + (EMB_DIM,):
        raise _lib.MMRecHipError("G must be [len(rows), 8 / 16 / 32 / 64]")
    for t, nm, n in ((dX, "dX", g.n_cols), (dZ, "dZ", g.n_rows)):
        if t is not None and (_chk(t, torch.float32, nm, 2).shape[0] < n or t.shape[1] != d):
            raise _lib.MMRecHipError("%s must be [>=%d, %d]" % (nm, n, d))
    _lib.check(lib.mmrec_spmm_push_rows_f32(_p(g.rowptr), _p(g.colidx), _p(g.vals), _p(G), float(scale), _p(rows), rows.numel(),
                                            d, _p(dX), _p(dZ), _stream()), "spmm_push_rows_f32")


class _SpmmRows(torch.autograd.Function):

    @staticmethod
    def forward(ctx, X, Z_rows, g, rows):
        ctx.g, ctx.x_shape, ctx.has_z = g, tuple(X.shape), Z_rows is not None
        ctx.save_for_backward(rows)
        return spmm_rows_raw(g, X.contiguous(), rows, None if Z_rows is None else Z_rows.contiguous(), z_compact=True)

    @staticmethod
    def backward(ctx, dY):
        rows, = ctx.saved_tensors
        dY = dY.contiguous()
        dX = None
        if ctx.needs_input_grad[0]:
            dX = torch.zeros(ctx.x_shape, dtype=dY.dtype, device=dY.device)
            spmm_push_rows_raw(ctx.g, dY, rows, dX=dX)
        return dX, (dY if ctx.has_z and ctx.needs_input_grad[1] else None), None, None


def spmm_rows(g: CsrGraph, X, rows, Z_rows=None):
    if DETERMINISTIC or isinstance(g, PermutedGraph) or not rows_servable(g, X.shape[1]):
        out = spmm(g, X).index_select(0, rows)
        return out if Z_rows is None else out + Z_rows
    return _SpmmRows.apply(X, Z_rows, g, rows)


class _SpMM(torch.autograd.Function):
    @staticmethod
    def forward(ctx, X, Z, g):
        ctx.g, ctx.has_z, ctx.x_rows = g, Z is not None, X.shape[0]
        X = X.contiguous()
        Y = torch.empty(g.n_rows, X.shape[1], dtype=torch.float32, device=X.device)
        spmm_raw(g, X, Y=Y, Z=None if Z is None else Z.contiguous(), beta=1.0)
        return Y

    @staticmethod
    def backward(ctx, dY):
        dY = dY.contiguous()
        gt = ctx.g.transpose()
        dX = None
        if ctx.needs_input_grad[0]:
            alloc = torch.empty if ctx.x_rows == gt.n_rows else torch.zeros
            dX = alloc(ctx.x_rows, dY.shape[1], dtype=torch.float32, device=dY.device)
            spmm_raw(gt, dY, Y=dX)
        return dX, (dY if ctx.has_z and ctx.needs_input_grad[1] else None), None


def spmm(g: CsrGraph, X, Z=None):
    if isinstance(g, PermutedGraph):
        out = spmm(g.graph, g.to_new(X), None if Z is None else g.to_new(Z))
        return g.to_old(out)
    d = X.shape[1]
    if d % EMB_DIM and d not in SLICE_WIDTHS:
        pad = EMB_DIM - d % EMB_DIM
        Xp = torch.nn.functional.pad(X, (0, pad))
        Zp = None if Z is None else torch.nn.functional.pad(Z, (0, pad))
        return _SpMM.apply(Xp, Zp, g)[:, :d]
    return _SpMM.apply(X, Z, g)


class _LightGCNMean(torch.autograd.Function):

    @staticmethod
    def forward(ctx, E0, g, n_layers):
        ctx.g, ctx.L = g, int(n_layers)
        E0 = E0.contiguous()
        L = ctx.L
        if L == 0:
            return E0.clone()
        acc = torch.empty_like(E0)
        bufs = [torch.empty_like(E0) if L > 1 else None, torch.empty_like(E0) if L > 2 else None]
        cur = E0
        for layer in range(1, L + 1):
            last = layer == L
            Y = None if last else bufs[(layer - 1) % 2]
            spmm_raw(g, cur, Y=Y, acc_in=E0 if layer == 1 else acc, acc_out=acc,
                     acc_scale=1.0 / (L + 1) if last else 1.0)
            cur = Y
        return acc

    @staticmethod
    def backward(ctx, dOut):
        L, gt = ctx.L, ctx.g.transpose()
        dOut = dOut.contiguous()
        if L == 0:
            return dOut, None, None
        s = 1.0 / (L + 1)
        bufs = [torch.empty_like(dOut), torch.empty_like(dOut) if L > 1 else None]
        t = dOut
        for j in range(L):
            out = bufs[j % 2]
            spmm_raw(gt, t, Y=out, Z=dOut, alpha=s if j == 0 else 1.0, beta=s)
            t = out
        return t, None, None


def lightgcn_mean(g, E0, n_layers):
    if isinstance(g, PermutedGraph):
        return g.to_old(_LightGCNMean.apply(g.to_new(E0), g.graph, n_layers))
    return _LightGCNMean.apply(E0, g, n_layers)


def row_blocks_of_one_buffer(ts):
    if any(t is None or not t.is_contiguous() or t.dtype != ts[0].dtype for t in ts):
        return False
    base = ts[0].untyped_storage().data_ptr()
    end = ts[0].data_ptr()
    for t in ts:
        if t.untyped_storage().data_ptr() != base or t.data_ptr() != end:
            return False
        end += t.numel() * t.element_size()
    return end <= base + ts[0].untyped_storage().nbytes()


class _LightGCNMeanParts(torch.autograd.Function):

    @staticmethod
    def forward(ctx, g, n_layers, *parts):
        ctx.sizes = [p.shape[0] for p in parts]
        if row_blocks_of_one_buffer(parts):
            E0 = parts[0].detach().as_strided((sum(ctx.sizes), parts[0].shape[1]), (parts[0].shape[1], 1))
        else:
            E0 = torch.cat([p.detach() for p in parts], dim=0)
        ctx.g, ctx.L = g, int(n_layers)
        out = _LightGCNMean.forward(ctx, E0, g, n_layers)
        return tuple(out.split(ctx.sizes))

    @staticmethod
    def backward(ctx, *grads):
        like = next(x for x in grads if x is not None)
        n, d = sum(ctx.sizes), like.shape[1]
        if row_blocks_of_one_buffer(grads):
            dOut = grads[0].as_strided((n, d), (d, 1))
        else:
            dOut = torch.empty((n, d), dtype=like.dtype, device=like.device)
            for dst, src in zip(dOut.split(ctx.sizes), grads):
                dst.zero_() if src is None else dst.copy_(src)
        t = _LightGCNMean.backward(ctx, dOut)[0]
        return (None, None) + tuple(t.split(ctx.sizes))


def lightgcn_mean_parts(g: CsrGraph, parts, n_layers):
    return _LightGCNMeanParts.apply(g, n_layers, *parts)


ROWS_LAST_LAYER = True


class _LightGCNMeanPartsRows(torch.autograd.Function):

    @staticmethod
    def forward(ctx, g, n_layers, rows, *parts):
        ctx.sizes = [p.shape[0] for p in parts]
        if row_blocks_of_one_buffer(parts):
            E0 = parts[0].detach().as_strided((sum(ctx.sizes), parts[0].shape[1]), (parts[0].shape[1], 1))
        else:
            E0 = torch.cat([p.detach() for p in parts], dim=0)
        ctx.save_for_backward(rows)
        L = int(n_layers)
        if L >= 1 and ROWS_LAST_LAYER and rows_servable(g, E0.shape[1]) and E0.shape[0] == g.n_rows == g.n_cols:
            ctx.g, ctx.L = g, L
            E0 = E0.contiguous()
            cur, acc = E0, E0
            if L > 1:
                acc = torch.empty_like(E0)
                bufs = [torch.empty_like(E0), torch.empty_like(E0) if L > 2 else None]
                for layer in range(1, L):
                    Y = bufs[(layer - 1) % 2]
                    spmm_raw(g, cur, Y=Y, acc_in=E0 if layer == 1 else acc, acc_out=acc, acc_scale=1.0)
                    cur = Y
            return spmm_rows_raw(g, cur, rows, Z=acc) * (1.0 / (L + 1))
        out = _LightGCNMean.forward(ctx, E0, g, n_layers)
        return out.index_select(0, rows)

    @staticmethod
    def backward(ctx, dRows):
        rows, = ctx.saved_tensors
        L, g = ctx.L, ctx.g
        dRows = dRows.contiguous()
        n, d = sum(ctx.sizes), dRows.shape[1]
        s = 1.0 / (L + 1)
        t = torch.zeros((n, d), dtype=dRows.dtype, device=dRows.device)
        if L == 0:
            spmm_push_rows_raw(g, dRows, rows, dZ=t)
            return (None, None, None) + tuple(t.split(ctx.sizes))
        spmm_push_rows_raw(g, dRows, rows, dX=t, dZ=t, scale=s)
        gt = g.transpose()
        for _ in range(1, L):
            out = torch.empty_like(t)
            spmm_raw(gt, t, Y=out)
            spmm_push_rows_raw(g, dRows, rows, dZ=out, scale=s)
            t = out
        return (None, None, None) + tuple(t.split(ctx.sizes))


class _MeanPartsRowsThenItemRows(torch.autograd.Function):

    @staticmethod
    def forward(ctx, g, n_layers, rows, mm, item_rows, b, user_table, item_table):
        import types
        inner = types.SimpleNamespace(saved=None)
        inner.save_for_backward = lambda *t: setattr(inner, 'saved', t)
        at = _LightGCNMeanPartsRows.forward(inner, g, n_layers, rows, user_table, item_table)
        ia = spmm_rows_raw(mm, item_table.detach().contiguous(), item_rows, at[b:].contiguous(), z_compact=True)
        ctx.inner = types.SimpleNamespace(sizes=inner.sizes, g=inner.g, L=inner.L)
        ctx.mm, ctx.b = mm, int(b)
        ctx.save_for_backward(rows, item_rows)
        return at[:b].contiguous(), ia

    @staticmethod
    def backward(ctx, d_user_rows, d_ia):
        rows, item_rows = ctx.saved_tensors
        inner = ctx.inner
        inner.saved_tensors = (rows,)
        d_ia = d_ia.contiguous()
        d_rows = torch.cat((d_user_rows.contiguous(), d_ia), dim=0)
        grads = _LightGCNMeanPartsRows.backward(inner, d_rows)
        d_user_table, d_item_table = grads[3], grads[4]
        spmm_push_rows_raw(ctx.mm, d_ia, item_rows, dX=d_item_table)
        return None, None, None, None, None, None, d_user_table, d_item_table


def lightgcn_mean_rows_then_item_rows(g: CsrGraph, user_table, item_table, n_layers, users, item_rows, mm: CsrGraph):
    b, nu, d = users.shape[0], user_table.shape[0], user_table.shape[1]
    rows = torch.cat((users, item_rows + nu))
    fast = (not DETERMINISTIC and not isinstance(g, PermutedGraph) and not isinstance(mm, PermutedGraph) and d == EMB_DIM
            and int(n_layers) >= 1 and ROWS_LAST_LAYER and rows_servable(g, d) and rows_servable(mm, d)
            and user_table.shape[0] + item_table.shape[0] == g.n_rows == g.n_cols and mm.n_rows == mm.n_cols == item_table.shape[0])
    if not fast:
        at = lightgcn_mean_parts_rows(g, (user_table, item_table), n_layers, rows)
        return at[:b], spmm_rows(mm, item_table, item_rows, Z_rows=at[b:])
    return _MeanPartsRowsThenItemRows.apply(g, n_layers, rows, mm, item_rows, b, user_table, item_table)


def lightgcn_mean_parts_rows(g: CsrGraph, parts, n_layers, rows):
    if DETERMINISTIC or isinstance(g, PermutedGraph) or parts[0].shape[1] not in SLICE_WIDTHS + (EMB_DIM,):
        return torch.cat(lightgcn_mean_parts(g, parts, n_layers), dim=0).index_select(0, rows)
    return _LightGCNMeanPartsRows.apply(g, n_layers, rows, *parts)


class _LayerGCNSum(torch.autograd.Function):

    @staticmethod
    def forward(ctx, E0, g, n_layers):
        lib = _lib.load()
        E0 = E0.contiguous()
        L, n = int(n_layers), E0.shape[0]
        if E0.shape[1] != EMB_DIM or E0.shape[0] != g.n_rows or g.n_cols != g.n_rows:
            raise _lib.MMRecHipError("layergcn_sum needs E0 [n, %d] over a square graph of n rows" % EMB_DIM)
        acc = torch.zeros_like(E0) if L == 0 else torch.empty_like(E0)
        need_y = any(ctx.needs_input_grad)
        ys, ws = [], []
        cur = E0
        for layer in range(L):
            y = torch.empty_like(E0) if need_y else None
            out, w = torch.empty_like(E0), torch.empty(n, dtype=torch.float32, device=E0.device)
            args = (_p(g.rowptr), _p(g.colidx), _p(g.vals), _p(cur), _p(y), _p(E0), _p(out), _p(w),
                    _p(acc) if layer > 0 else None, _p(acc), g.n_rows, EMB_DIM, g.long_row_threshold, _p(g.long_rows),
                    _p(g.long_chunk_ptr), g.n_long, g.n_chunks, _p(g.partials_for(EMB_DIM)), _p(g.long_tickets))
            sc = g.scheduled(EMB_DIM)
            if sc is not None:
                g.checked(lib.mmrec_spmm_csr_sched_f32_layergcn(*args, _p(sc["row"]), _p(sc["span"]), _p(sc["col"]), _p(sc["val"]),
                                                                sc["n_short"], _stream()), "spmm_sched_layergcn")
            else:
                g.checked(lib.mmrec_spmm_csr_f32_layergcn(*args, _stream()), "spmm_layergcn")
            ys.append(y), ws.append(w)
            cur = out
        ctx.g, ctx.L = g, L
        if need_y:
            ctx.save_for_backward(E0, *ys, *ws)
        return acc

    @staticmethod
    def backward(ctx, dSum):
        lib = _lib.load()
        L, gt = ctx.L, ctx.g.transpose()
        saved = ctx.saved_tensors
        E0, ys, ws = saved[0], saved[1:1 + L], saved[1 + L:]
        dSum = dSum.contiguous()
        n = E0.shape[0]
        dEgo = torch.zeros_like(E0)
        dOut = dSum
        for layer in range(L - 1, -1, -1):
            dY = torch.empty_like(E0)
            _lib.check(lib.mmrec_cos_scale_bwd_f32(_p(dOut), _p(ys[layer]), _p(E0), _p(ws[layer]),
                                                   _p(dY), _p(dEgo), n, EMB_DIM, _stream()),
                       "cos_scale_bwd")
            nxt = torch.empty_like(E0)
            spmm_raw(gt, dY, Y=nxt, Z=dSum if layer > 0 else dEgo, beta=1.0)
            dOut = nxt
        return dOut, None, None


def layergcn_sum(g: CsrGraph, E0, n_layers):
    return _LayerGCNSum.apply(E0, g, n_layers)


class _LayerGCNSumParts(torch.autograd.Function):

    @staticmethod
    def forward(ctx, g, n_layers, *parts):
        ctx.sizes = [p.shape[0] for p in parts]
        if row_blocks_of_one_buffer(parts):
            E0 = parts[0].detach().as_strided((sum(ctx.sizes), parts[0].shape[1]), (parts[0].shape[1], 1))
        else:
            E0 = torch.cat([p.detach() for p in parts], dim=0)
        return tuple(_LayerGCNSum.forward(ctx, E0, g, n_layers).split(ctx.sizes))

    @staticmethod
    def backward(ctx, *grads):
        like = next(x for x in grads if x is not None)
        n, d = sum(ctx.sizes), like.shape[1]
        if row_blocks_of_one_buffer(grads):
            dSum = grads[0].as_strided((n, d), (d, 1))
        else:
            dSum = torch.empty((n, d), dtype=like.dtype, device=like.device)
            for dst, src in zip(dSum.split(ctx.sizes), grads):
                dst.zero_() if src is None else dst.copy_(src)
        t = _LayerGCNSum.backward(ctx, dSum)[0]
        return (None, None) + tuple(t.split(ctx.sizes))


def layergcn_sum_parts(g: CsrGraph, parts, n_layers):
    return _LayerGCNSumParts.apply(g, n_layers, *parts)


def _bpr_bwd_deterministic(U, I, users, pos, neg, coef, g, scale, dU, dI):
    lib = _lib.load()
    B, d = users.numel(), U.shape[1]
    ar = torch.arange(B, device=U.device)
    Ug = U.index_select(0, users)
    Ig = torch.cat((I.index_select(0, pos), I.index_select(0, neg)), 0)
    dUg = torch.zeros_like(Ug) if dU is not None else None
    dIg = torch.zeros_like(Ig) if dI is not None else None
    arn = (ar + B).contiguous()
    _lib.check(lib.mmrec_bpr_bwd_f32(_p(Ug), _p(Ig), _p(Ig), _p(ar), _p(ar), _p(arn), B, d, _p(coef), _p(g), scale, _p(dUg),
                                     _p(dIg), _p(dIg), _stream()), "bpr_bwd")
    if dU is not None:
        scatter_add_rows(users, dUg, dU)
    if dI is not None:
        scatter_add_rows(torch.cat((pos, neg)), dIg, dI)


class _BprLoss(torch.autograd.Function):
    @staticmethod
    def forward(ctx, U, I, users, pos, neg, variant, scale):
        lib = _lib.load()
        U, I = _chk(U.contiguous(), torch.float32, "U", 2), _chk(I.contiguous(), torch.float32, "I", 2)
        for t, nm in ((users, "users"), (pos, "pos"), (neg, "neg")):
            _chk(t, torch.int64, nm, 1)
        B, dev = users.numel(), U.device
        loss = torch.empty((), dtype=torch.float32, device=dev)
        coef = torch.empty(max(B, 1), dtype=torch.float32, device=dev)
        ws = _ws(lib.mmrec_bpr_workspace_bytes(B), dev)
        if U.shape[1] != I.shape[1] or U.shape[1] % EMB_DIM:
            raise _lib.MMRecHipError("U and I need the same row width, a multiple of %d" % EMB_DIM)
        _lib.check(lib.mmrec_bpr_fwd_f32(_p(U), _p(I), _p(I), _p(users), _p(pos), _p(neg), B, U.shape[1],
                                         int(variant), float(scale), _p(loss), _p(coef), _p(ws),
                                         _stream()), "bpr_fwd")
        ctx.save_for_backward(U, I, users, pos, neg, coef)
        ctx.scale = float(scale)
        return loss

    @staticmethod
    def backward(ctx, g):
        lib = _lib.load()
        U, I, users, pos, neg, coef = ctx.saved_tensors
        g = g.contiguous().to(torch.float32)
        dU = torch.zeros_like(U) if ctx.needs_input_grad[0] else None
        dI = torch.zeros_like(I) if ctx.needs_input_grad[1] else None
        if DETERMINISTIC:
            _bpr_bwd_deterministic(U, I, users, pos, neg, coef, g, ctx.scale, dU, dI)
            return dU, dI, None, None, None, None, None
        _lib.check(lib.mmrec_bpr_bwd_f32(_p(U), _p(I), _p(I), _p(users), _p(pos), _p(neg),
                                         users.numel(), U.shape[1], _p(coef), _p(g), ctx.scale, _p(dU),
                                         _p(dI), _p(dI), _stream()), "bpr_bwd")
        return dU, dI, None, None, None, None, None


class _BprLossShared(torch.autograd.Function):

    @staticmethod
    def forward(ctx, U, users, variant, scale, n_terms, joint, sum_over_ranks, *flat):
        lib = _lib.load()
        ctx.joint = bool(joint)
        U = _chk(U.contiguous(), torch.float32, "U", 2)
        _chk(users, torch.int64, "users", 1)
        B, dev = users.numel(), U.device
        tables, ids, coefs, losses = [], [], [], []
        ws = _ws(lib.mmrec_bpr_workspace_bytes(B), dev)
        d = U.shape[1]
        sliced = sum_over_ranks is not None
        if sliced:
            dots = torch.empty((n_terms, 2, max(B, 1)), dtype=torch.float32, device=dev)
        for t in range(n_terms):
            I, pos, neg = flat[3 * t], flat[3 * t + 1], flat[3 * t + 2]
            I = _chk(I.contiguous(), torch.float32, "I", 2)
            _chk(pos, torch.int64, "pos", 1), _chk(neg, torch.int64, "neg", 1)
            if d != I.shape[1] or (d % EMB_DIM and not (sliced and d in SLICE_WIDTHS)):
                raise _lib.MMRecHipError("U and I need the same row width, a multiple of %d%s" %
                                         (EMB_DIM, " or a slice of 8 / 16 / 32 columns" if sliced else ""))
            tables.append(I), ids.extend((pos, neg))
            if sliced:
                _lib.check(lib.mmrec_bpr_dots_f32(_p(U), _p(I), _p(I), _p(users), _p(pos), _p(neg), B, d, _p(dots[t]),
                                                  _stream()), "bpr_dots")
                continue
            loss = torch.empty((), dtype=torch.float32, device=dev)
            coef = torch.empty(max(B, 1), dtype=torch.float32, device=dev)
            _lib.check(lib.mmrec_bpr_fwd_f32(_p(U), _p(I), _p(I), _p(users), _p(pos), _p(neg), B, d,
                                             int(variant), float(scale), _p(loss), _p(coef), _p(ws), _stream()), "bpr_fwd")
            coefs.append(coef), losses.append(loss)
        if sliced:
            sum_over_ranks(dots)
            for t in range(n_terms):
                loss = torch.empty((), dtype=torch.float32, device=dev)
                coef = torch.empty(max(B, 1), dtype=torch.float32, device=dev)
                _lib.check(lib.mmrec_bpr_loss_from_dots_f32(_p(dots[t]), B, int(variant), float(scale), _p(loss), _p(coef),
                                                            _p(ws), _stream()), "bpr_loss_from_dots")
                coefs.append(coef), losses.append(loss)
        ctx.save_for_backward(U, users, *tables, *ids, *coefs)
        ctx.scale, ctx.n_terms = float(scale), n_terms
        return tuple(losses)

    @staticmethod
    def backward(ctx, *gs):
        lib = _lib.load()
        n = ctx.n_terms
        saved = ctx.saved_tensors
        U, users = saved[0], saved[1]
        tables, ids, coefs = saved[2:2 + n], saved[2 + n:2 + 3 * n], saved[2 + 3 * n:]
        dU = dI0 = None
        if ctx.joint and ctx.needs_input_grad[0] and ctx.needs_input_grad[7]:
            both = torch.zeros((U.shape[0] + tables[0].shape[0], U.shape[1]), dtype=U.dtype, device=U.device)
            dU, dI0 = both[:U.shape[0]], both[U.shape[0]:]
        elif ctx.needs_input_grad[0]:
            dU = torch.zeros_like(U)
        out = []
        for t in range(n):
            I, pos, neg = tables[t], ids[2 * t], ids[2 * t + 1]
            need_i = ctx.needs_input_grad[7 + 3 * t]
            own = dI0 if t == 0 and dI0 is not None else None
            if gs[t] is None or (dU is None and not need_i):
                out.extend(((own if own is not None else torch.zeros_like(I)) if need_i else None, None, None))
                continue
            dI = (own if own is not None else torch.zeros_like(I)) if need_i else None
            g = gs[t].contiguous().to(torch.float32)
            if DETERMINISTIC:
                _bpr_bwd_deterministic(U, I, users, pos, neg, coefs[t], g, ctx.scale, dU, dI)
            else:
                _lib.check(lib.mmrec_bpr_bwd_f32(_p(U), _p(I), _p(I), _p(users), _p(pos), _p(neg), users.numel(), U.shape[1],
                                                 _p(coefs[t]), _p(g), ctx.scale, _p(dU), _p(dI), _p(dI), _stream()), "bpr_bwd")
            out.extend((dI, None, None))
        return (dU, None, None, None, None, None, None) + tuple(out)


class _BprWeightedTotal(torch.autograd.Function):

    @staticmethod
    def forward(ctx, U, users, variant, scale, weights, joint, *flat):
        lib = _lib.load()
        n = len(weights)
        U = _chk(U.contiguous(), torch.float32, "U", 2)
        _chk(users, torch.int64, "users", 1)
        B, d, dev = users.numel(), U.shape[1], U.device
        tables = [_chk(flat[3 * t].contiguous(), torch.float32, "I", 2) for t in range(n)]
        pos, neg = [flat[3 * t + 1] for t in range(n)], [flat[3 * t + 2] for t in range(n)]
        for t in range(n):
            _chk(pos[t], torch.int64, "pos", 1), _chk(neg[t], torch.int64, "neg", 1)
            if tables[t].shape[1] != d or d % EMB_DIM or pos[t].numel() != B or neg[t].numel() != B:
                raise _lib.MMRecHipError("U and every table need the same row width (a multiple of %d), every id list B entries" % EMB_DIM)
        ptrs = lambda ts: (ctypes.c_void_p * n)(*[t.data_ptr() for t in ts])
        ctx.arrays = (ptrs(tables), ptrs(pos), ptrs(neg), (ctypes.c_float * n)(*[float(w) for w in weights]))
        total = torch.empty((), dtype=torch.float32, device=dev)
        coef = torch.empty(n, max(B, 1), dtype=torch.float32, device=dev)
        ws = _ws(lib.mmrec_bpr_multi_workspace_bytes(n, B), dev)
        _lib.check(lib.mmrec_bpr_multi_fwd_f32(_p(U), _p(users), *ctx.arrays, n, B, d, int(variant), float(scale), _p(total), None,
                                               _p(coef), _p(ws), _stream()), "bpr_multi_fwd")
        ctx.save_for_backward(U, users, coef, *tables, *pos, *neg)
        ctx.n, ctx.scale, ctx.joint = n, float(scale), bool(joint)
        return total

    @staticmethod
    def backward(ctx, g):
        lib = _lib.load()
        n = ctx.n
        U, users, coef = ctx.saved_tensors[:3]
        tables = ctx.saved_tensors[3:3 + n]
        g = g.contiguous().to(torch.float32)
        need_u = ctx.needs_input_grad[0]
        need_i = [ctx.needs_input_grad[6 + 3 * t] for t in range(n)]
        dU = None
        grads = [None] * n
        if ctx.joint and need_u and need_i[0]:
            both = torch.zeros((U.shape[0] + tables[0].shape[0], U.shape[1]), dtype=U.dtype, device=U.device)
            dU, grads[0] = both[:U.shape[0]], both[U.shape[0]:]
        elif need_u:
            dU = torch.zeros_like(U)
        shared = {}
        for t in range(n):
            if need_i[t] and grads[t] is None:
                key = tables[t].data_ptr()
                if key not in shared:
                    shared[key] = torch.zeros_like(tables[t])
                grads[t] = shared[key]
        dI = (ctypes.c_void_p * n)(*[None if x is None else x.data_ptr() for x in grads])
        _lib.check(lib.mmrec_bpr_multi_bwd_f32(_p(U), _p(users), *ctx.arrays, n, users.numel(), U.shape[1], _p(coef), _p(g), ctx.scale,
                                               _p(dU), dI, _stream()), "bpr_multi_bwd")
        out, seen = [dU, None, None, None, None, None], set()
        for t in range(n):
            gi = grads[t]
            if gi is not None and id(gi) in seen:
                gi = None
            elif gi is not None:
                seen.add(id(gi))
            out += [gi, None, None]
        return tuple(out)


def bpr_weighted_total(U, users, terms, weights, variant=BPR_LOGSIG, reduction="mean", joint_grad=False):
    terms = list(terms)
    if DETERMINISTIC or not 1 <= len(terms) <= 4 or not _one_buffer_per_table([I for I, _, _ in terms]):
        losses = bpr_losses_shared_users(U, users, terms, variant, reduction, joint_grad=joint_grad)
        total = 0.0
        for w, l in zip(weights, losses):
            total = total + w * l
        return total
    B = users.numel()
    scale = 1.0 / max(B, 1) if reduction == "mean" else 1.0
    flat = [x for term in terms for x in term]
    return _BprWeightedTotal.apply(U, users, variant, scale, tuple(float(w) for w in weights), joint_grad, *flat)


def bpr_losses_shared_users(U, users, terms, variant=BPR_LOGSIG, reduction="mean", joint_grad=False, sum_over_ranks=None):
    B = users.numel()
    scale = 1.0 / max(B, 1) if reduction == "mean" else 1.0
    flat = [x for term in terms for x in term]
    return _BprLossShared.apply(U, users, variant, scale, len(terms), joint_grad, sum_over_ranks, *flat)


def bpr_loss(U, I, users, pos, neg, variant=BPR_LOGSIG, reduction="mean"):
    B = users.numel()
    scale = 1.0 / max(B, 1) if reduction == "mean" else 1.0
    return _BprLoss.apply(U, I, users, pos, neg, variant, scale)


class _InfoNCE(torch.autograd.Function):
    @staticmethod
    def forward(ctx, E1, E2, ids, tau):
        lib = _lib.load()
        E1, E2 = _chk(E1.contiguous(), torch.float32, "E1", 2), _chk(E2.contiguous(), torch.float32, "E2", 2)
        _chk(ids, torch.int64, "ids", 1)
        if E1.shape != E2.shape or E1.shape[1] != EMB_DIM:
            raise _lib.MMRecHipError("InfoNCE views must both be [n, %d]" % EMB_DIM)
        B = ids.numel()
        loss = torch.empty((), dtype=torch.float32, device=E1.device)
        ws = _ws(lib.mmrec_infonce_workspace_bytes(B), E1.device)
        _lib.check(lib.mmrec_infonce_fwd_f32(_p(E1), _p(E2), _p(ids), B, EMB_DIM, float(tau), _p(loss),
                                             _p(ws), _stream()), "infonce_fwd")
        ctx.save_for_backward(ids, ws)
        ctx.tau, ctx.shape = float(tau), E1.shape
        return loss

    @staticmethod
    def backward(ctx, g):
        lib = _lib.load()
        ids, ws = ctx.saved_tensors
        g = g.contiguous().to(torch.float32)
        dE1 = torch.zeros(ctx.shape, dtype=torch.float32, device=g.device) if ctx.needs_input_grad[0] else None
        dE2 = torch.zeros(ctx.shape, dtype=torch.float32, device=g.device) if ctx.needs_input_grad[1] else None
        if DETERMINISTIC:
            B = ids.numel()
            ar = torch.arange(B, device=g.device)
            r1 = torch.zeros(B, EMB_DIM, dtype=torch.float32, device=g.device) if dE1 is not None else None
            r2 = torch.zeros(B, EMB_DIM, dtype=torch.float32, device=g.device) if dE2 is not None else None
            _lib.check(lib.mmrec_infonce_bwd_f32(_p(ar), B, EMB_DIM, ctx.tau, _p(g), _p(r1), _p(r2), _p(ws), _stream()),
                       "infonce_bwd")
            if dE1 is not None:
                scatter_add_rows(ids, r1, dE1)
            if dE2 is not None:
                scatter_add_rows(ids, r2, dE2)
            return dE1, dE2, None, None
        _lib.check(lib.mmrec_infonce_bwd_f32(_p(ids), ids.numel(), EMB_DIM, ctx.tau, _p(g), _p(dE1),
                                             _p(dE2), _p(ws), _stream()), "infonce_bwd")
        return dE1, dE2, None, None


def infonce(E1, E2, ids, tau):
    return _InfoNCE.apply(E1, E2, ids, tau)


class _GatherSqNorm(torch.autograd.Function):
    @staticmethod
    def forward(ctx, E, ids):
        lib = _lib.load()
        E = _chk(E.contiguous(), torch.float32, "E", 2)
        _chk(ids, torch.int64, "ids", 1)
        out = torch.empty((), dtype=torch.float32, device=E.device)
        ws = _ws(4 * ids.numel(), E.device)
        _lib.check(lib.mmrec_gather_sqnorm_fwd_f32(_p(E), _p(ids), ids.numel(), E.shape[1], _p(out),
                                                   _p(ws), _stream()), "gather_sqnorm_fwd")
        ctx.save_for_backward(E, ids)
        return out

    @staticmethod
    def backward(ctx, g):
        lib = _lib.load()
        E, ids = ctx.saved_tensors
        coef = (2.0 * g).contiguous().to(torch.float32)
        dE = torch.zeros_like(E)
        if DETERMINISTIC:
            return scatter_add_rows(ids, E.index_select(0, ids) * coef, dE), None
        _lib.check(lib.mmrec_gather_scale_add_bwd_f32(_p(E), _p(ids), ids.numel(), E.shape[1], _p(coef),
                                                      _p(dE), _stream()), "gather_scale_add_bwd")
        return dE, None


def gather_sqnorm(E, ids):
    return _GatherSqNorm.apply(E, ids)


class _RowsReg(torch.autograd.Function):

    @staticmethod
    def forward(ctx, mode, scale, *flat):
        lib = _lib.load()
        tables = [_chk(flat[2 * t].contiguous(), torch.float32, "E", 2) for t in range(len(flat) // 2)]
        ids = [None if flat[2 * t + 1] is None else _chk(flat[2 * t + 1], torch.int64, "ids", 1) for t in range(len(flat) // 2)]
        n, d, dev = len(tables), tables[0].shape[1], tables[0].device
        if any(E.shape[1] != d for E in tables) or d % EMB_DIM:
            raise _lib.MMRecHipError("rows_reg: every table needs the same row width, a multiple of %d" % EMB_DIM)
        batch = (ctypes.c_int32 * n)(*[E.shape[0] if i is None else i.numel() for E, i in zip(tables, ids)])
        ctx.arrays = ((ctypes.c_void_p * n)(*[E.data_ptr() for E in tables]),
                      (ctypes.c_void_p * n)(*[None if i is None else i.data_ptr() for i in ids]), batch)
        out = torch.empty((), dtype=torch.float32, device=dev)
        coef = torch.empty(n, dtype=torch.float32, device=dev)
        ws = _ws(lib.mmrec_rows_reg_workspace_bytes(n, max(batch)), dev)
        _lib.check(lib.mmrec_rows_reg_fwd_f32(ctx.arrays[0], ctx.arrays[1], batch, n, d, int(mode), float(scale), _p(out), _p(coef),
                                              _p(ws), _stream()), "rows_reg_fwd")
        ctx.save_for_backward(coef, *tables, *[i for i in ids if i is not None])
        ctx.n = n
        return out

    @staticmethod
    def backward(ctx, g):
        lib = _lib.load()
        n = ctx.n
        coef, tables = ctx.saved_tensors[0], ctx.saved_tensors[1:1 + n]
        g = g.contiguous().to(torch.float32)
        grads, first, out = {}, {}, [None, None]
        for t, E in enumerate(tables):
            if E.data_ptr() not in grads:
                grads[E.data_ptr()], first[E.data_ptr()] = torch.zeros_like(E), t
        dE = (ctypes.c_void_p * n)(*[grads[E.data_ptr()].data_ptr() for E in tables])
        _lib.check(lib.mmrec_rows_reg_bwd_f32(ctx.arrays[0], ctx.arrays[1], ctx.arrays[2], n, tables[0].shape[1], _p(coef), _p(g), dE,
                                              _stream()), "rows_reg_bwd")
        for t, E in enumerate(tables):
            out += [grads[E.data_ptr()] if (first[E.data_ptr()] == t and ctx.needs_input_grad[2 + 2 * t]) else None, None]
        return tuple(out)


ROWS_REG_SQUARED, ROWS_REG_NORM = 0, 1


def _one_buffer_per_table(tables):
    seen = []
    for E in tables:
        if not E.is_contiguous():
            return False
        lo = E.data_ptr()
        span = (lo, lo + E.numel() * E.element_size(), tuple(E.shape), bool(E.requires_grad))
        for other in seen:
            if span[0] < other[1] and other[0] < span[1] and span != other:
                return False
        seen.append(span)
    return True


def rows_reg(terms, mode, scale=1.0):
    terms = list(terms)
    same_rows = len({E.shape[1] for E, _ in terms}) == 1
    if (DETERMINISTIC or len(terms) > 6 or not terms or not same_rows or any(not E.is_contiguous() for E, _ in terms)
            or not _one_buffer_per_table([E for E, _ in terms])):
        total = 0.0
        for E, ids in terms:
            s = (E * E).sum() if ids is None else gather_sqnorm(E, ids)
            total = total + (s if mode == ROWS_REG_SQUARED else torch.sqrt(s))
        return scale * total
    flat = [x for E, ids in terms for x in (E, None if ids is None else ids.contiguous())]
    return _RowsReg.apply(mode, scale, *flat)


class _RowNormalize(torch.autograd.Function):
    @staticmethod
    def forward(ctx, X, eps):
        lib = _lib.load()
        X = _chk(X.contiguous(), torch.float32, "X", 2)
        if X.shape[1] % 4:
            raise _lib.MMRecHipError("row_normalize: rows of a multiple of 4 floats")
        Y = torch.empty_like(X)
        inv = torch.empty(max(X.shape[0], 1), dtype=torch.float32, device=X.device)
        _lib.check(lib.mmrec_row_normalize_fwd_f32(_p(X), X.shape[0], X.shape[1], float(eps), _p(Y), _p(inv), _stream()),
                   "row_normalize_fwd")
        ctx.save_for_backward(Y, inv)
        return Y

    @staticmethod
    def backward(ctx, G):
        lib = _lib.load()
        Y, inv = ctx.saved_tensors
        G = G.contiguous()
        dX = torch.empty_like(Y)
        _lib.check(lib.mmrec_row_normalize_bwd_f32(_p(Y), _p(G), _p(inv), Y.shape[0], Y.shape[1], _p(dX), _stream()),
                   "row_normalize_bwd")
        return dX, None


def row_normalize(X, eps=1e-12):
    return _RowNormalize.apply(X, eps)


class _CatLeaky(torch.autograd.Function):
    @staticmethod
    def forward(ctx, A, B, R, slope):
        lib = _lib.load()
        A, B = _chk(A.contiguous(), torch.float32, "A", 2), _chk(B.contiguous(), torch.float32, "B", 2)
        if R is not None:
            R = _chk(R.contiguous(), torch.float32, "R", 2)
        n, wa, wb = A.shape[0], A.shape[1], B.shape[1]
        if B.shape[0] != n or (R is not None and R.shape != B.shape) or wa % 4 or wb % 4:
            raise _lib.MMRecHipError("cat_leaky: A [n, wa], B [n, wb], R [n, wb] with wa, wb multiples of 4")
        out = torch.empty(n, wa + wb, dtype=torch.float32, device=A.device)
        _lib.check(lib.mmrec_cat_leaky_fwd_f32(_p(A), _p(B), _p(R), n, wa, wb, float(slope), _p(out), _stream()), "cat_leaky_fwd")
        ctx.save_for_backward(A, B)
        ctx.slope = float(slope)
        return out

    @staticmethod
    def backward(ctx, dOut):
        lib = _lib.load()
        A, B = ctx.saved_tensors
        dOut = dOut.contiguous()
        dA = torch.empty_like(A) if ctx.needs_input_grad[0] else None
        dB = torch.empty_like(B) if ctx.needs_input_grad[1] else None
        dR = torch.empty_like(B) if ctx.needs_input_grad[2] else None
        _lib.check(lib.mmrec_cat_leaky_bwd_f32(_p(A), _p(B), _p(dOut), A.shape[0], A.shape[1], B.shape[1], ctx.slope, _p(dA), _p(dB),
                                               _p(dR), _stream()), "cat_leaky_bwd")
        return dA, dB, dR, None


def cat_leaky(A, B, R=None, slope=0.01):
    return _CatLeaky.apply(A, B, R, slope)


class _CosineMean(torch.autograd.Function):
    @staticmethod
    def forward(ctx, X, ix, Y, iy):
        lib = _lib.load()
        X, Y = _chk(X.contiguous(), torch.float32, "X", 2), _chk(Y.contiguous(), torch.float32, "Y", 2)
        for t, nm in ((ix, "ix"), (iy, "iy")):
            if t is not None:
                _chk(t, torch.int64, nm, 1)
        B = ix.numel() if ix is not None else (iy.numel() if iy is not None else X.shape[0])
        if X.shape[1] != Y.shape[1] or X.shape[1] % EMB_DIM:
            raise _lib.MMRecHipError("X and Y need the same row width, a multiple of %d" % EMB_DIM)
        if (ix is None and X.shape[0] != B) or (iy is None and Y.shape[0] != B):
            raise _lib.MMRecHipError("an operand without an index must have one row per sample")
        out = torch.empty((), dtype=torch.float32, device=X.device)
        coef = torch.empty(max(B, 1), 2, dtype=torch.float32, device=X.device)
        ws = _ws(lib.mmrec_cosine_workspace_bytes(B), X.device)
        _lib.check(lib.mmrec_cosine_fwd_f32(_p(X), _p(ix), _p(Y), _p(iy), B, X.shape[1], 1.0 / max(B, 1), _p(out),
                                            _p(coef), _p(ws), _stream()), "cosine_fwd")
        ctx.save_for_backward(X, Y, coef, *[t for t in (ix, iy) if t is not None])
        ctx.has = (ix is not None, iy is not None)
        ctx.B = B
        return out

    @staticmethod
    def backward(ctx, g):
        lib = _lib.load()
        X, Y, coef, *idx = ctx.saved_tensors
        ix = idx.pop(0) if ctx.has[0] else None
        iy = idx.pop(0) if ctx.has[1] else None
        dX = torch.zeros_like(X)
        g = g.contiguous().to(torch.float32)
        if DETERMINISTIC and ix is not None:
            Xg = X.index_select(0, ix)
            Yg = Y.index_select(0, iy) if iy is not None else Y
            rows = torch.zeros_like(Xg)
            _lib.check(lib.mmrec_cosine_bwd_f32(_p(Xg), None, _p(Yg), None, ctx.B, X.shape[1], _p(coef), _p(g),
                                                1.0 / max(ctx.B, 1), _p(rows), _stream()), "cosine_bwd")
            return scatter_add_rows(ix, rows, dX), None, None, None
        _lib.check(lib.mmrec_cosine_bwd_f32(_p(X), _p(ix), _p(Y), _p(iy), ctx.B, X.shape[1], _p(coef), _p(g),
                                            1.0 / max(ctx.B, 1), _p(dX), _stream()), "cosine_bwd")
        return dX, None, None, None


class _CosineMeans(torch.autograd.Function):

    @staticmethod
    def forward(ctx, weights, *flat):
        lib = _lib.load()
        n = len(weights)
        X = [_chk(flat[4 * t].contiguous(), torch.float32, "X", 2) for t in range(n)]
        Y = [_chk(flat[4 * t + 2].contiguous(), torch.float32, "Y", 2) for t in range(n)]
        ix, iy = [flat[4 * t + 1] for t in range(n)], [flat[4 * t + 3] for t in range(n)]
        d, dev = X[0].shape[1], X[0].device
        batch = []
        for t in range(n):
            for i, nm in ((ix[t], "ix"), (iy[t], "iy")):
                if i is not None:
                    _chk(i, torch.int64, nm, 1)
            B = ix[t].numel() if ix[t] is not None else (iy[t].numel() if iy[t] is not None else X[t].shape[0])
            if X[t].shape[1] != d or Y[t].shape[1] != d or d % EMB_DIM:
                raise _lib.MMRecHipError("cosine_means: every operand needs the same row width, a multiple of %d" % EMB_DIM)
            if (ix[t] is None and X[t].shape[0] != B) or (iy[t] is None and Y[t].shape[0] != B):
                raise _lib.MMRecHipError("an operand without an index must have one row per sample")
            batch.append(B)
        ptrs = lambda ts: (ctypes.c_void_p * n)(*[None if t is None else t.data_ptr() for t in ts])
        ctx.arrays = (ptrs(X), ptrs(ix), ptrs(Y), ptrs(iy), (ctypes.c_float * n)(*[float(w) for w in weights]), (ctypes.c_int32 * n)(*batch))
        out = torch.empty((), dtype=torch.float32, device=dev)
        coef = torch.empty(n, max(max(batch), 1), 2, dtype=torch.float32, device=dev)
        ws = _ws(lib.mmrec_cosine_multi_workspace_bytes(n, max(batch)), dev)
        _lib.check(lib.mmrec_cosine_multi_fwd_f32(*ctx.arrays, n, d, _p(out), _p(coef), _p(ws), _stream()), "cosine_multi_fwd")
        ctx.save_for_backward(coef, *X, *Y, *[i for i in ix + iy if i is not None])
        ctx.n = n
        return out

    @staticmethod
    def backward(ctx, g):
        lib = _lib.load()
        n = ctx.n
        coef, X = ctx.saved_tensors[0], ctx.saved_tensors[1:1 + n]
        g = g.contiguous().to(torch.float32)
        grads, first = {}, {}
        for t, x in enumerate(X):
            if ctx.needs_input_grad[1 + 4 * t] and x.data_ptr() not in grads:
                grads[x.data_ptr()], first[x.data_ptr()] = torch.zeros_like(x), t
        dX = (ctypes.c_void_p * n)(*[grads[x.data_ptr()].data_ptr() if x.data_ptr() in grads else None for x in X])
        _lib.check(lib.mmrec_cosine_multi_bwd_f32(*ctx.arrays, n, X[0].shape[1], _p(coef), _p(g), dX, _stream()), "cosine_multi_bwd")
        out = [None]
        for t, x in enumerate(X):
            out += [grads[x.data_ptr()] if first.get(x.data_ptr()) == t else None, None, None, None]
        return tuple(out)


def cosine_means(terms):
    terms = list(terms)
    if DETERMINISTIC or not terms or len(terms) > 8 or not _one_buffer_per_table([X for X, *_ in terms]):
        total = 0.0
        for X, ix, Y, iy, w in terms:
            total = total + w * cosine_mean(X, ix, Y, iy)
        return total
    flat = [a for X, ix, Y, iy, _ in terms for a in (X, ix, Y.detach(), iy)]
    return _CosineMeans.apply(tuple(float(w) for *_, w in terms), *flat)


def cosine_mean(X, ix, Y, iy):
    return _CosineMean.apply(X, ix, Y.detach(), iy)


LINEAR_SPLIT_MIN_F = 1024


class _Linear(torch.autograd.Function):
    @staticmethod
    def forward(ctx, X, W, b):
        lib = _lib.load()
        X = _chk(X.contiguous(), torch.float32, "X", 2)
        W = _chk(W.contiguous(), torch.float32, "W", 2)
        n, F = X.shape
        if W.shape != (64, F):
            raise _lib.MMRecHipError("W must be [64, %d], got %s" % (F, tuple(W.shape)))
        if b is not None:
            b = _chk(b.contiguous(), torch.float32, "b", 1)
        Y = torch.empty(n, 64, dtype=torch.float32, device=X.device)
        ws = _ws(lib.mmrec_linear_workspace_bytes(n, F, 64), X.device)
        fwd = lib.mmrec_linear_fwd_split_f32 if (LINEAR_F16X3 and F >= LINEAR_SPLIT_MIN_F) else lib.mmrec_linear_fwd_f32
        _lib.check(fwd(_p(X), _p(W), _p(b), _p(Y), n, F, 64, _p(ws), _stream()), "linear_fwd")
        ctx.save_for_backward(X, W)
        ctx.has_b = b is not None
        return Y

    @staticmethod
    def backward(ctx, dY):
        lib = _lib.load()
        X, W = ctx.saved_tensors
        n, F = X.shape
        dY = dY.contiguous()
        dX = dW = db = None
        want_w = ctx.needs_input_grad[1] or (ctx.has_b and ctx.needs_input_grad[2])
        if want_w:
            dW = torch.empty_like(W)
            db = torch.empty(64, dtype=torch.float32, device=X.device) if ctx.has_b else None
        if ctx.needs_input_grad[0]:
            dX = torch.empty_like(X)
        if LINEAR_F16X3 and n > 0 and F % 128 == 0:
            ws = _ws(lib.mmrec_linear_bwd_split_workspace_bytes(n, F, 64), X.device)
            _lib.check(lib.mmrec_linear_bwd_split_f32(_p(dY), _p(X), _p(W), _p(dW), _p(db), _p(dX), n, F, 64, _p(ws),
                                                      _stream()), "linear_bwd_split")
            return dX, dW, db
        if want_w:
            ws = _ws(lib.mmrec_linear_workspace_bytes(n, F, 64), X.device)
            _lib.check(lib.mmrec_linear_bwd_w_f32(_p(dY), _p(X), _p(dW), _p(db), n, F, 64, _p(ws),
                                                  _stream()), "linear_bwd_w")
        if dX is not None:
            _lib.check(lib.mmrec_linear_bwd_x_f32(_p(dY), _p(W), _p(dX), n, F, 64, _stream()),
                       "linear_bwd_x")
        return dX, dW, db


class _LinearWide(torch.autograd.Function):

    @staticmethod
    def forward(ctx, X, W, b):
        lib = _lib.load()
        X = _chk(X.contiguous(), torch.float32, "X", 2)
        W = _chk(W.contiguous(), torch.float32, "W", 2)
        n, F = X.shape
        out = W.shape[0]
        if W.shape[1] != F or out % 64 or F % 32:
            raise _lib.MMRecHipError("wide linear needs W [64 j, F], F %% 32 == 0; got W %s, X %s" %
                                     (tuple(W.shape), tuple(X.shape)))
        if b is not None:
            b = _chk(b.contiguous(), torch.float32, "b", 1)
        Y = torch.empty(n, out, dtype=torch.float32, device=X.device)
        _lib.check(lib.mmrec_gemm_nt_f32(_p(X), _p(W), _p(b), _p(Y), n, out, F, out, _stream()), "gemm_nt")
        ctx.save_for_backward(X, W)
        ctx.has_b = b is not None
        return Y

    @staticmethod
    def backward(ctx, dY):
        lib = _lib.load()
        X, W = ctx.saved_tensors
        n, F = X.shape
        out = W.shape[0]
        dY = dY.contiguous()
        dX = dW = db = None
        if ctx.needs_input_grad[1] or (ctx.has_b and ctx.needs_input_grad[2]):
            dW = torch.empty_like(W)
            db = torch.empty(out, dtype=torch.float32, device=X.device) if ctx.has_b else None
            ws = _ws(lib.mmrec_linear_workspace_bytes(n, F, out), X.device)
            _lib.check(lib.mmrec_linear_bwd_w_f32(_p(dY), _p(X), _p(dW), _p(db), n, F, out, _p(ws),
                                                  _stream()), "linear_bwd_w")
        if ctx.needs_input_grad[0]:
            dX = torch.empty_like(X)
            Wt = W.t().contiguous()
            _lib.check(lib.mmrec_gemm_nt_f32(_p(dY), _p(Wt), None, _p(dX), n, F, out, F, _stream()), "gemm_nt")
        return dX, dW, db


def linear(X, W, b=None):
    if W.shape[0] == 64:
        return _Linear.apply(X, W, b)
    return _LinearWide.apply(X, W, b)


def linear_rows_served(table, ids, W):
    return (LINEAR_F16X3 and isinstance(table, torch.Tensor) and table.is_cuda and table.dtype == torch.float32 and
            table.dim() == 2 and table.is_contiguous() and W.is_cuda and W.dtype == torch.float32 and W.dim() == 2 and
            W.shape[0] == 64 and W.shape[1] == table.shape[1] and table.shape[1] % 128 == 0 and
            isinstance(ids, torch.Tensor) and ids.is_cuda and ids.dtype == torch.int64 and ids.dim() == 1)


def _linear_rows_fwd(table, ids, W, b):
    lib = _lib.load()
    n, F = ids.numel(), table.shape[1]
    Y = torch.empty(n, 64, dtype=torch.float32, device=table.device)
    ws = _ws(lib.mmrec_linear_rows_workspace_bytes(n, F, 64), table.device)
    split = 1 if F >= LINEAR_SPLIT_MIN_F else 0
    _lib.check(lib.mmrec_linear_rows_fwd_f32(_p(table), table.shape[0], _p(ids), _p(W), _p(b), _p(Y), n, F, 64, split, _p(ws),
                                             _stream()), "linear_rows_fwd")
    return Y


def _linear_rows_bwd(dY, table, ids, W, want_w, has_b, want_x):
    lib = _lib.load()
    n, F = ids.numel(), table.shape[1]
    dY = dY.contiguous()
    dW = db = dX = None
    if want_w:
        dW = torch.empty_like(W)
        db = torch.empty(64, dtype=torch.float32, device=W.device) if has_b else None
    if want_x:
        dX = torch.empty(n, F, dtype=torch.float32, device=W.device)
    if want_w or want_x:
        ws = _ws(lib.mmrec_linear_rows_workspace_bytes(n, F, 64), W.device)
        _lib.check(lib.mmrec_linear_rows_bwd_f32(_p(dY), _p(table), table.shape[0], _p(ids), _p(W), _p(dW), _p(db), _p(dX), n, F,
                                                 64, _p(ws), _stream()), "linear_rows_bwd")
    return dW, db, dX


class _LinearRows(torch.autograd.Function):
    @staticmethod
    def forward(ctx, table, ids, W, b):
        W = _chk(W.contiguous(), torch.float32, "W", 2)
        if b is not None:
            b = _chk(b.contiguous(), torch.float32, "b", 1)
        ids = ids.contiguous()
        ctx.save_for_backward(table, ids, W)
        ctx.has_b = b is not None
        return _linear_rows_fwd(table, ids, W, b)

    @staticmethod
    def backward(ctx, dY):
        table, ids, W = ctx.saved_tensors
        want_w = ctx.needs_input_grad[2] or (ctx.has_b and ctx.needs_input_grad[3])
        dW, db, dX = _linear_rows_bwd(dY, table, ids, W, want_w, ctx.has_b, ctx.needs_input_grad[0])
        dT = None
        if dX is not None:
            dT = torch.zeros_like(table).index_put_((ids,), dX, accumulate=True)
        return dT, None, dW, db


def linear_rows(table, ids, W, b=None):
    if linear_rows_served(table, ids, W):
        return _LinearRows.apply(table, ids, W, b)
    return linear(table.index_select(0, ids), W, b)


def mask_to_csr(mask, n_rows, device):
    m = mask.detach().cpu().numpy() if isinstance(mask, torch.Tensor) else np.asarray(mask)
    m = m.astype(np.int64)
    order = np.lexsort((m[1], m[0]))
    rowptr = np.zeros(n_rows + 1, dtype=np.int64)
    np.cumsum(np.bincount(m[0], minlength=n_rows), out=rowptr[1:])
    return (torch.from_numpy(rowptr.astype(np.int32)).to(device),
            torch.from_numpy(m[1][order].astype(np.int32)).to(device))


TOPK_NO_FILTER = 1


class TopkCandidates:

    def __init__(self, C):
        lib = _lib.load()
        self.C = _chk(C.contiguous(), torch.float32, "C", 2)
        nc, kd = self.C.shape
        nbytes = lib.mmrec_topk_prepared_bytes(nc, kd)
        self.prepared = None
        if nbytes:
            self.prepared = _ws(nbytes, self.C.device)
            _lib.check(lib.mmrec_topk_prepare_f32(_p(self.C), nc, kd, _p(self.prepared), _stream()), "topk_prepare")


def topk_hint_served(nc, kd, k):
    return k <= TOPK_MAX and _lib.load().mmrec_topk_prepared_bytes(int(nc), int(kd)) > 0


TOPK_HINT_COLD, TOPK_HINT_KEEP = 1, 2


def topk_hint_width(k):
    return 64 if k <= 64 else 128


def score_topk(Q, C, k, mask_rowptr=None, mask_col=None, return_values=False, use_filter=True, hint=None, hint_rows=None,
               queue_counts=None, hint_cold=False, hint_update=True):
    lib = _lib.load()
    Q = _chk(Q.contiguous(), torch.float32, "Q", 2)
    prepared = None
    if isinstance(C, TopkCandidates):
        C, prepared = C.C, (C.prepared if use_filter else None)
    C = _chk(C.contiguous(), torch.float32, "C", 2)
    nq, kd = Q.shape
    nc = C.shape[0]
    if C.shape[1] != kd:
        raise _lib.MMRecHipError("Q and C must share the inner dim")
    if mask_rowptr is not None:
        _chk(mask_rowptr, torch.int32, "mask_rowptr", 1)
        if mask_col is None or mask_col.numel() == 0:
            mask_col = torch.zeros(1, dtype=torch.int32, device=Q.device)
        _chk(mask_col, torch.int32, "mask_col", 1)
    if hint is not None and not (use_filter and nc >= k and topk_hint_served(nc, kd, k)):
        hint = None
    if hint is not None:
        _chk(hint, torch.int32, "hint", 2)
        if hint.shape[1] < k or hint.shape[1] > TOPK_MAX:
            raise _lib.MMRecHipError("hint rows hold k <= hk <= %d ids, got %d for k = %d" % (TOPK_MAX, hint.shape[1], k))
        if hint_rows is not None:
            _chk(hint_rows, torch.int64, "hint_rows", 1)
            if hint_rows.numel() != nq:
                raise _lib.MMRecHipError("hint_rows: one row index per query")
        elif hint.shape[0] != nq:
            raise _lib.MMRecHipError("hint: one row per query (or pass hint_rows)")
        if queue_counts is not None:
            _chk(queue_counts, torch.int32, "queue_counts", 1)
    if nq > 2 * TOPK_QUERY_BLOCK and use_filter and (prepared is not None or lib.mmrec_topk_prepared_bytes(nc, kd) > 0):
        return _score_topk_blocked(Q, C, prepared, k, mask_rowptr, mask_col, return_values, hint, hint_rows, queue_counts,
                                   hint_cold, hint_update)
    idx = torch.empty(nq, k, dtype=torch.int64, device=Q.device)
    val = torch.empty(nq, k, dtype=torch.float32, device=Q.device) if return_values else None
    ws = _ws(lib.mmrec_topk_workspace_bytes(nq, nc, kd, k), Q.device)
    if hint is not None:
        _lib.check(lib.mmrec_score_topk_hinted_f32(_p(Q), _p(C), _p(prepared), nq, nc, kd, _p(mask_rowptr), _p(mask_col), k,
                                                   _p(hint), hint.shape[1], _p(hint_rows), _p(idx), _p(val), _p(ws),
                                                   _p(queue_counts), (TOPK_HINT_COLD if hint_cold else 0) |
                                                   (0 if hint_update else TOPK_HINT_KEEP), _stream()), "score_topk_hinted")
    elif prepared is not None:
        _lib.check(lib.mmrec_score_topk_prepared_f32(_p(Q), _p(C), _p(prepared), nq, nc, kd, _p(mask_rowptr), _p(mask_col), k,
                                                     _p(idx), _p(val), _p(ws), 0, _stream()), "score_topk_prepared")
    else:
        _lib.check(lib.mmrec_score_topk_f32(_p(Q), _p(C), nq, nc, kd, _p(mask_rowptr), _p(mask_col), k,
                                            _p(idx), _p(val), _p(ws), 0 if use_filter else TOPK_NO_FILTER, _stream()),
                   "score_topk")
    return (idx, val) if return_values else idx


TOPK_QUERY_BLOCK = 65536


def _score_topk_blocked(Q, C, prepared, k, mask_rowptr, mask_col, return_values, hint=None, hint_rows=None, queue_counts=None,
                        hint_cold=False, hint_update=True):
    nq = Q.shape[0]
    cands = TopkCandidates.__new__(TopkCandidates)
    cands.C = C
    cands.prepared = prepared if prepared is not None else TopkCandidates(C).prepared
    starts = list(range(0, nq, TOPK_QUERY_BLOCK))
    offs = None
    if mask_rowptr is not None:
        offs = mask_rowptr[torch.tensor(starts + [nq], device=mask_rowptr.device)].cpu().tolist()
    idx = torch.empty(nq, k, dtype=torch.int64, device=Q.device)
    val = torch.empty(nq, k, dtype=torch.float32, device=Q.device) if return_values else None
    for j, a in enumerate(starts):
        b = min(a + TOPK_QUERY_BLOCK, nq)
        rp = col = None
        if mask_rowptr is not None:
            rp = (mask_rowptr[a:b + 1] - offs[j]).contiguous()
            col = mask_col[offs[j]:max(offs[j + 1], offs[j] + 1)].contiguous()
        h = hr = None
        if hint is not None:
            h, hr = (hint, hint_rows[a:b]) if hint_rows is not None else (hint[a:b], None)
        out = score_topk(Q[a:b], cands, k, rp, col, return_values=return_values, hint=h, hint_rows=hr, queue_counts=queue_counts,
                         hint_cold=hint_cold, hint_update=hint_update)
        if return_values:
            idx[a:b], val[a:b] = out
        else:
            idx[a:b] = out
    return (idx, val) if return_values else idx


def degree_count(ids, n_bins):
    lib = _lib.load()
    _chk(ids, torch.int64, "ids", 1)
    counts = torch.zeros(n_bins, dtype=torch.int32, device=ids.device)
    _lib.check(lib.mmrec_degree_count_i32(_p(ids), ids.numel(), _p(counts), n_bins, _stream()),
               "degree_count")
    return counts


def edge_norm_values(eu, ei, n_users, n_items):
    lib = _lib.load()
    du, di = degree_count(eu, n_users), degree_count(ei, n_items)
    val = torch.empty(eu.numel(), dtype=torch.float32, device=eu.device)
    _lib.check(lib.mmrec_edge_norm_f32(_p(eu), _p(ei), eu.numel(), _p(du), _p(di), _p(val), _stream()),
               "edge_norm")
    return val


def bipartite_graph_from_edges(eu, ei, n_users, n_items, long_row_threshold=LONG_ROW_DEFAULT):
    lib = _lib.load()
    eu, ei = _chk(eu.contiguous(), torch.int64, "eu", 1), _chk(ei.contiguous(), torch.int64, "ei", 1)
    E, dev = eu.numel(), eu.device
    w = edge_norm_values(eu, ei, n_users, n_items)
    rows = torch.empty(2 * E, dtype=torch.int32, device=dev)
    cols = torch.empty(2 * E, dtype=torch.int32, device=dev)
    vals = torch.empty(2 * E, dtype=torch.float32, device=dev)
    _lib.check(lib.mmrec_bipartite_expand(_p(eu), _p(ei), _p(w), E, n_users, _p(rows), _p(cols),
                                          _p(vals), _stream()), "bipartite_expand")
    n = n_users + n_items
    return CsrGraph.from_coo_device(rows, cols, vals, n, n, symmetric=True,
                                    long_row_threshold=long_row_threshold)


class DynGraph:

    def __init__(self, rows, cols, n_rows, n_cols, long_row_threshold=LONG_ROW_DEFAULT):
        _chk(rows, torch.int64, "rows", 1), _chk(cols, torch.int64, "cols", 1)
        self.rows, self.cols, self.n_rows, self.n_cols = rows, cols, int(n_rows), int(n_cols)
        dev = rows.device
        zeros = torch.zeros(rows.numel(), dtype=torch.float32, device=dev)

        def build(r, c, nr, nc):
            perm = torch.sort(r, stable=True)[1]
            rowptr = torch.zeros(nr + 1, dtype=torch.int64, device=dev)
            rowptr[1:] = torch.cumsum(torch.bincount(r, minlength=nr), 0)
            g = CsrGraph(rowptr.to(torch.int32), c[perm].to(torch.int32).contiguous(), zeros, nr, nc,
                         long_row_threshold=long_row_threshold, row_schedule=False)
            return g, perm
        self.fwd, self.perm = build(rows, cols, self.n_rows, self.n_cols)
        self.bwd, self.perm_t = build(cols, rows, self.n_cols, self.n_rows)


class _SpMMVals(torch.autograd.Function):
    @staticmethod
    def forward(ctx, X, vals, dyn):
        X = X.contiguous()
        dyn.fwd.vals = vals.detach()[dyn.perm].contiguous()
        Y = torch.empty(dyn.n_rows, X.shape[1], dtype=torch.float32, device=X.device)
        spmm_raw(dyn.fwd, X, Y=Y)
        ctx.dyn = dyn
        ctx.save_for_backward(X, vals)
        return Y

    @staticmethod
    def backward(ctx, dY):
        dyn = ctx.dyn
        X, vals = ctx.saved_tensors
        dY = dY.contiguous()
        dX = dvals = None
        if ctx.needs_input_grad[0]:
            dyn.bwd.vals = vals.detach()[dyn.perm_t].contiguous()
            dX = torch.empty(dyn.n_cols, X.shape[1], dtype=torch.float32, device=dY.device)
            spmm_raw(dyn.bwd, dY, Y=dX)
        if ctx.needs_input_grad[1]:
            if edge_dot_served(dY, X, dyn.rows, dyn.cols):
                dvals = _edge_dot_fwd(dY, X, dyn.rows, dyn.cols)
            else:
                dvals = (dY[dyn.rows] * X[dyn.cols]).sum(-1)
        return dX, dvals, None


def spmm_vals(dyn: DynGraph, X, vals):
    return _SpMMVals.apply(X, vals, dyn)


EDGE_DOT = True


def _edge_width_served(d):
    return d in SLICE_WIDTHS or (d > 0 and d % EMB_DIM == 0 and d <= 6 * EMB_DIM)


def edge_dot_served(A, B, rows, cols):
    def table(t):
        return (isinstance(t, torch.Tensor) and t.is_cuda and t.dtype == torch.float32 and t.dim() == 2 and
                t.is_contiguous())

    def ids(t):
        return isinstance(t, torch.Tensor) and t.is_cuda and t.dtype == torch.int64 and t.dim() == 1 and t.is_contiguous()
    return bool(EDGE_DOT and table(A) and table(B) and A.shape[1] == B.shape[1] and _edge_width_served(A.shape[1]) and
                ids(rows) and ids(cols) and rows.numel() == cols.numel())


def _edge_dot_fwd(A, B, rows, cols):
    lib = _lib.load()
    out = torch.empty(rows.numel(), dtype=torch.float32, device=A.device)
    _lib.check(lib.mmrec_edge_dot_f32(_p(A), A.shape[0], _p(B), B.shape[0], _p(rows), _p(cols), rows.numel(), A.shape[1],
                                      _p(out), _stream()), "edge_dot")
    return out


class _EdgeDot(torch.autograd.Function):

    @staticmethod
    def forward(ctx, A, B, rows, cols, dyn):
        ctx.same = B is None
        if ctx.same:
            B = A
        ctx.dyn, ctx.deterministic = dyn, DETERMINISTIC
        ctx.save_for_backward(A, B, rows, cols)
        return _edge_dot_fwd(A, B, rows, cols)

    @staticmethod
    def backward(ctx, g):
        A, B, rows, cols = ctx.saved_tensors
        dyn, same = ctx.dyn, ctx.same
        want_a, want_b = ctx.needs_input_grad[0], (ctx.needs_input_grad[0] if same else ctx.needs_input_grad[1])
        g = g.contiguous()
        dA = dB = None
        if dyn is None and ctx.deterministic and rows.numel():
            dyn = DynGraph(rows, cols, A.shape[0], B.shape[0])
        if dyn is not None:
            if want_a:
                dyn.fwd.vals = g[dyn.perm].contiguous()
                dA = spmm_raw(dyn.fwd, B, Y=torch.empty(dyn.n_rows, A.shape[1], dtype=torch.float32, device=A.device))
            if want_b:
                dyn.bwd.vals = g[dyn.perm_t].contiguous()
                dB = spmm_raw(dyn.bwd, A, Y=torch.empty(dyn.n_cols, A.shape[1], dtype=torch.float32, device=A.device))
            if same:
                return (dA + dB if want_a else None), None, None, None, None
            return dA, dB, None, None, None
        if want_a:
            dA = torch.zeros_like(A)
        if same:
            dB = dA
        elif want_b:
            dB = torch.zeros_like(B)
        if want_a or want_b:
            _lib.check(_lib.load().mmrec_edge_dot_bwd_f32(_p(g), _p(A), A.shape[0], _p(B), B.shape[0], _p(rows), _p(cols),
                                                          rows.numel(), A.shape[1], _p(dA), _p(dB), _stream()), "edge_dot_bwd")
        return dA, (None if same else dB), None, None, None


def edge_dot(A, B, rows, cols, dyn=None):
    if edge_dot_served(A, B, rows, cols):
        return _EdgeDot.apply(A, None if A is B else B, rows, cols, dyn)
    return (A[rows] * B[cols]).sum(-1)


EDGE_SOFTMAX = True


def segment_softmax_torch(score, index, n, eps=1e-16):
    mx = torch.full((n,), float('-inf'), dtype=score.dtype, device=score.device)
    mx = mx.scatter_reduce(0, index, score.detach(), 'amax', include_self=True)
    e = (score - mx[index]).exp()
    den = torch.zeros(n, dtype=score.dtype, device=score.device).index_add_(0, index, e)
    return e / (den[index] + eps)


def segment_softmax_group_max():
    return int(_lib.load().mmrec_segment_softmax_group_max())


def segment_long_rows(rowptr_host):
    lib = _lib.load()
    rp = np.ascontiguousarray(rowptr_host, dtype=np.int32)
    n_rows, thr = rp.size - 1, segment_softmax_group_max()
    n_long, n_chunks = ctypes.c_int32(0), ctypes.c_int32(0)
    ptr = rp.ctypes.data_as(ctypes.c_void_p)
    _lib.check(lib.mmrec_spmm_plan_count(ptr, n_rows, thr, ctypes.byref(n_long), ctypes.byref(n_chunks)), "spmm_plan_count")
    lr, cp = np.empty(n_long.value, dtype=np.int32), np.empty(n_long.value + 1, dtype=np.int32)
    if n_long.value:
        _lib.check(lib.mmrec_spmm_plan_fill(ptr, n_rows, thr, lr.ctypes.data_as(ctypes.c_void_p),
                                            cp.ctypes.data_as(ctypes.c_void_p)), "spmm_plan_fill")
    want = np.flatnonzero(np.diff(rp.astype(np.int64)) > thr).astype(np.int32)
    if not np.array_equal(lr, want):
        raise _lib.MMRecHipError("segment softmax: the plan's long rows are not the rows longer than %d" % thr)
    return lr


def _softmax_side(dyn, by):
    if by not in ("row", "col"):
        raise ValueError("edge_softmax: by must be 'row' or 'col', got %r" % (by,))
    g, perm = (dyn.fwd, dyn.perm) if by == "row" else (dyn.bwd, dyn.perm_t)
    cache = dyn.__dict__.setdefault("_softmax_long", {})
    if by not in cache:
        lr = segment_long_rows(g.rowptr_host)
        cache[by] = torch.from_numpy(lr).to(g.rowptr.device) if lr.size else None
    return g, perm, cache[by]


def edge_softmax_served(score, dyn):
    return bool(EDGE_SOFTMAX and isinstance(score, torch.Tensor) and score.is_cuda and score.dtype == torch.float32 and
                score.dim() == 1 and score.is_contiguous() and score.numel() == dyn.rows.numel())


class _EdgeSoftmax(torch.autograd.Function):
    @staticmethod
    def forward(ctx, score, dyn, by, eps):
        g, perm, long_rows = _softmax_side(dyn, by)
        n_long = 0 if long_rows is None else long_rows.numel()
        alpha = torch.empty_like(score)
        _lib.check(_lib.load().mmrec_segment_softmax_f32(_p(g.rowptr), g.n_rows, _p(perm), _p(long_rows), n_long, _p(score),
                                                         score.numel(), eps, _p(alpha), _stream()), "segment_softmax")
        ctx.dyn, ctx.by = dyn, by
        ctx.save_for_backward(alpha)
        return alpha

    @staticmethod
    def backward(ctx, grad):
        (alpha,) = ctx.saved_tensors
        g, perm, long_rows = _softmax_side(ctx.dyn, ctx.by)
        n_long = 0 if long_rows is None else long_rows.numel()
        grad = grad.contiguous()
        ds = torch.empty_like(alpha)
        _lib.check(_lib.load().mmrec_segment_softmax_bwd_f32(_p(g.rowptr), g.n_rows, _p(perm), _p(long_rows), n_long,
                                                             _p(alpha), _p(grad), alpha.numel(), _p(ds), _stream()),
                   "segment_softmax_bwd")
        return ds, None, None, None


def edge_softmax(score, dyn, by="row", eps=1e-16):
    if edge_softmax_served(score, dyn):
        return _EdgeSoftmax.apply(score, dyn, by, float(eps))
    if by not in ("row", "col"):
        raise ValueError("edge_softmax: by must be 'row' or 'col', got %r" % (by,))
    index, n = (dyn.rows, dyn.n_rows) if by == "row" else (dyn.cols, dyn.n_cols)
    return segment_softmax_torch(score, index, n, eps)


EDGE_ATTENTION = True
EDGE_ATTENTION_BWD = True


def edge_attention_group_max():
    return int(_lib.load().mmrec_edge_attention_group_max())


def _attention_long_rows(dyn):
    if edge_attention_group_max() != segment_softmax_group_max():
        raise _lib.MMRecHipError("edge attention: group maximum %d is not the segment softmax's %d"
                                 % (edge_attention_group_max(), segment_softmax_group_max()))
    return _softmax_side(dyn, "row")[2]


def edge_attention_served(Q, KV, dyn):
    def table(t, n):
        return (isinstance(t, torch.Tensor) and t.is_cuda and t.dtype == torch.float32 and t.dim() == 2 and
                t.shape[1] == EMB_DIM and t.is_contiguous() and t.shape[0] == n)
    return bool(EDGE_ATTENTION and table(Q, dyn.n_rows) and table(KV, dyn.n_cols))


def _spmm_with(g, vals, X):
    g.vals = vals
    return spmm_raw(g, X, Y=torch.empty(g.n_rows, X.shape[1], dtype=torch.float32, device=X.device))


class _EdgeAttention(torch.autograd.Function):

    @staticmethod
    def forward(ctx, Q, KV, dyn, eps, fused_backward=False):
        ctx.same = KV is None
        if ctx.same:
            KV = Q
        g, n_edges = dyn.fwd, dyn.rows.numel()
        long_rows = _attention_long_rows(dyn)
        n_long = 0 if long_rows is None else long_rows.numel()
        Y = (torch.empty if n_edges else torch.zeros)(dyn.n_rows, EMB_DIM, dtype=torch.float32, device=Q.device)
        alpha = torch.empty(n_edges, dtype=torch.float32, device=Q.device)
        _lib.check(_lib.load().mmrec_edge_attention_f32(_p(g.rowptr), g.n_rows, _p(g.colidx), _p(dyn.perm), _p(long_rows), n_long,
                                                        _p(Q), Q.shape[0], _p(KV), KV.shape[0], EMB_DIM, n_edges, eps, _p(Y),
                                                        _p(alpha), _stream()), "edge_attention")
        ctx.dyn = dyn
        ctx.fused_backward = bool(fused_backward and EDGE_ATTENTION_BWD)
        ctx.set_materialize_grads(False)
        if ctx.fused_backward:
            _softmax_side(dyn, "col")
            ctx.save_for_backward(Q, KV, alpha, Y)
        else:
            ctx.save_for_backward(Q, KV, alpha)
        return Y, alpha

    @staticmethod
    def backward(ctx, dY, dA):
        Q, KV, alpha = ctx.saved_tensors[:3]
        dyn, same = ctx.dyn, ctx.same
        want_q, want_kv = ctx.needs_input_grad[0], (ctx.needs_input_grad[0] if same else ctx.needs_input_grad[1])
        if (dY is None and dA is None) or not (want_q or want_kv) or not alpha.numel():
            zq = torch.zeros_like(Q) if want_q else None
            return zq, (None if same or not want_kv else torch.zeros_like(KV)), None, None, None
        if ctx.fused_backward:
            fwd, perm, long_rows = _softmax_side(dyn, "row")
            bwd, perm_t, long_cols = _softmax_side(dyn, "col")
            dY = None if dY is None else dY.contiguous()
            dA = None if dA is None else dA.contiguous()
            ds = torch.empty_like(alpha)
            dQ = torch.empty_like(Q) if want_q else None
            dKV = torch.empty_like(KV) if want_kv else None
            _lib.check(_lib.load().mmrec_edge_attention_bwd_f32(
                _p(fwd.rowptr), fwd.n_rows, _p(fwd.colidx), _p(perm), _p(long_rows), 0 if long_rows is None else long_rows.numel(),
                _p(bwd.rowptr), _p(bwd.colidx), _p(perm_t), _p(long_cols), 0 if long_cols is None else long_cols.numel(),
                _p(Q), Q.shape[0], _p(KV), KV.shape[0], _p(ctx.saved_tensors[3]), _p(alpha), _p(dY), _p(dA), EMB_DIM,
                alpha.numel(), _p(ds), _p(dQ), _p(dKV), _p(dQ) if same else None, _stream()), "edge_attention_bwd")
            return (dKV if same else dQ), (None if same else dKV), None, None, None
        g = None
        if dY is not None:
            dY = dY.contiguous()
            g = _edge_dot_fwd(dY, KV, dyn.rows, dyn.cols)
        if dA is not None:
            g = dA.contiguous() if g is None else g + dA
        fwd, perm, long_rows = _softmax_side(dyn, "row")
        n_long = 0 if long_rows is None else long_rows.numel()
        ds = torch.empty_like(alpha)
        _lib.check(_lib.load().mmrec_segment_softmax_bwd_f32(_p(fwd.rowptr), fwd.n_rows, _p(perm), _p(long_rows), n_long,
                                                             _p(alpha), _p(g), alpha.numel(), _p(ds), _stream()),
                   "segment_softmax_bwd")
        dQ = dKV = None
        if want_q:
            dQ = _spmm_with(dyn.fwd, ds[dyn.perm].contiguous(), KV)
        if want_kv:
            dKV = _spmm_with(dyn.bwd, ds[dyn.perm_t].contiguous(), Q)
            if dY is not None:
                dKV = _spmm_with(dyn.bwd, alpha[dyn.perm_t].contiguous(), dY) + dKV
        if same:
            return dQ + dKV, None, None, None, None
        return dQ, dKV, None, None, None


def edge_attention(Q, KV, dyn, eps=1e-16, fused_backward=False):
    if edge_attention_served(Q, KV, dyn):
        return _EdgeAttention.apply(Q, None if Q is KV else KV, dyn, float(eps), bool(fused_backward))
    alpha = edge_softmax(edge_dot(Q, KV, dyn.rows, dyn.cols, dyn=dyn), dyn, eps=eps)
    return spmm_vals(dyn, KV, alpha), alpha


def flat_to_csr(flat, lens, device):
    lens = np.asarray(lens, dtype=np.int64)
    flat = np.asarray(flat, dtype=np.int64)
    rowptr = np.zeros(lens.shape[0] + 1, dtype=np.int64)
    np.cumsum(lens, out=rowptr[1:])
    if flat.size:
        stride = np.int64(flat.max()) + 1
        key = np.repeat(np.arange(lens.shape[0], dtype=np.int64), lens) * stride + flat
        key.sort()
        flat = key % stride
    else:
        flat = np.zeros(1, np.int64)
    return (torch.from_numpy(rowptr.astype(np.int32)).to(device),
            torch.from_numpy(flat.astype(np.int32)).to(device))


def lists_to_csr(lists, device):
    lens = np.fromiter((len(x) for x in lists), dtype=np.int64, count=len(lists))
    flat = np.concatenate([np.asarray(x, dtype=np.int64) for x in lists]) if len(lists) else np.zeros(0, np.int64)
    return flat_to_csr(flat, lens, device)


def sample_negatives(users, hist_rowptr, hist_col, cand_items, seed, counter):
    lib = _lib.load()
    _chk(users, torch.int64, "users", 1), _chk(hist_rowptr, torch.int32, "hist_rowptr", 1)
    _chk(hist_col, torch.int32, "hist_col", 1), _chk(cand_items, torch.int32, "cand_items", 1)
    out = torch.empty_like(users)
    _lib.check(lib.mmrec_sample_negatives_i64(_p(users), users.numel(), _p(hist_rowptr), _p(hist_col),
                                              _p(cand_items), cand_items.numel(), int(seed) & (2 ** 64 - 1),
                                              int(counter) & (2 ** 64 - 1), _p(out), _stream()),
               "sample_negatives")
    return out


def topk_metrics_per_user(topk_idx, gt_rowptr, gt_col, ks, want_hits=False):
    lib = _lib.load()
    topk_idx = _chk(topk_idx.contiguous(), torch.int64, "topk_idx", 2)
    _chk(gt_rowptr, torch.int32, "gt_rowptr", 1), _chk(gt_col, torch.int32, "gt_col", 1)
    n, k = topk_idx.shape
    dev = topk_idx.device
    ks = sorted(int(x) for x in ks)
    if ks[-1] > k or ks[0] < 1:
        raise _lib.MMRecHipError("cut-offs must lie in [1, k]")
    disc = 1.0 / np.log2(np.arange(1, k + 1, dtype=np.float64) + 1)
    d_disc = torch.from_numpy(disc).to(dev)
    d_idcg = torch.from_numpy(np.cumsum(disc)).to(dev)
    d_ks = torch.tensor(ks, dtype=torch.int32, device=dev)
    out = torch.empty(n, 4, len(ks), dtype=torch.float64, device=dev)
    hits = torch.empty(n, k, dtype=torch.uint8, device=dev) if want_hits else None
    _lib.check(lib.mmrec_topk_metrics_f64(_p(topk_idx), n, k, _p(gt_rowptr), _p(gt_col), _p(d_disc),
                                          _p(d_idcg), _p(d_ks), len(ks), _p(hits), _p(out), _stream()),
               "topk_metrics")
    return (out, hits) if want_hits else out
```

Measured before the change: 31.44 billion.

## Use precomputed per-chunk descriptors for long rows, optional wave-per-row mid path

```diff
diff --git a/include/mmrec_hip.h b/include/mmrec_hip.h
--- a/include/mmrec_hip.h
+++ b/include/mmrec_hip.h
@@ -22,6 +22,7 @@
 #ifndef MMREC_SPMM_CHUNK
 #define MMREC_SPMM_CHUNK 512
 #endif
+#define MMREC_SPMM_MID_ROW_MAX 64
 #define MMREC_SPMM_LONG_ROW_DEFAULT 32
 
 int mmrec_spmm_csr_f32(const int32_t* rowptr, const int32_t* colidx, const float* vals,
@@ -62,6 +63,22 @@
 int mmrec_spmm_row_keys(const int32_t* rowptr, const int32_t* colidx, const int32_t* col_degree, int32_t n_rows,
                         int32_t long_row_threshold, int32_t key_deg_max, int32_t* key, int32_t* key_degree,
                         mmrec_stream_t stream);
+int mmrec_spmm_csr_sched_desc_f32(const int32_t* rowptr, const int32_t* colidx, const float* vals, const float* X, float* Y,
+                                  const float* Z, const float* acc_in, float* acc_out, int32_t n_rows, int32_t d, float alpha,
+                                  float beta, float acc_scale, int32_t long_row_threshold, const int32_t* long_rows,
+                                  const int32_t* long_chunk_ptr, int32_t n_long, int32_t n_chunks, float* partials,
+                                  int32_t* long_tickets, const int32_t* sched_row, const int32_t* sched_span,
+                                  const int32_t* sched_col, const float* sched_val, int32_t n_short, const int32_t* long_desc,
+                                  int32_t n_mid, mmrec_stream_t stream);
+int mmrec_spmm_csr_sched_desc_f32_layergcn(const int32_t* rowptr, const int32_t* colidx, const float* vals, const float* X,
+                                           float* Y, const float* ego, float* scaled, float* w, const float* acc_in,
+                                           float* acc_out, int32_t n_rows, int32_t d, int32_t long_row_threshold,
+                                           const int32_t* long_rows, const int32_t* long_chunk_ptr, int32_t n_long,
+                                           int32_t n_chunks, float* partials, int32_t* long_tickets, const int32_t* sched_row,
+                                           const int32_t* sched_span, const int32_t* sched_col, const float* sched_val,
+                                           int32_t n_short, const int32_t* long_desc, int32_t n_mid, mmrec_stream_t stream);
+int mmrec_spmm_plan_desc_fill(const int32_t* rowptr_host, int32_t n_rows, int32_t long_row_threshold, int32_t mid_row_max,
+                              int32_t* long_desc, int32_t* n_mid);
 int mmrec_spmm_plan_count(const int32_t* rowptr_host, int32_t n_rows, int32_t long_row_threshold,
                           int32_t* n_long, int32_t* n_chunks);
 int mmrec_spmm_plan_fill(const int32_t* rowptr_host, int32_t n_rows, int32_t long_row_threshold,
diff --git a/mmrec_amd/_lib.py b/mmrec_amd/_lib.py
--- a/mmrec_amd/_lib.py
+++ b/mmrec_amd/_lib.py
@@ -24,6 +24,13 @@
                                            _P, _P, _P, _P, c_int32, _P]),
     "mmrec_spmm_csr_sched_f32_layergcn": (c_int32, [_P, _P, _P, _P, _P, _P, _P, _P, _P, _P, c_int32, c_int32, c_int32,
                                                     _P, _P, c_int32, c_int32, _P, _P, _P, _P, _P, _P, c_int32, _P]),
+    "mmrec_spmm_csr_sched_desc_f32": (c_int32, [_P, _P, _P, _P, _P, _P, _P, _P, c_int32, c_int32, c_float,
+                                                c_float, c_float, c_int32, _P, _P, c_int32, c_int32, _P, _P,
+                                                _P, _P, _P, _P, c_int32, _P, c_int32, _P]),
+    "mmrec_spmm_csr_sched_desc_f32_layergcn": (c_int32, [_P, _P, _P, _P, _P, _P, _P, _P, _P, _P, c_int32, c_int32, c_int32,
+                                                         _P, _P, c_int32, c_int32, _P, _P, _P, _P, _P, _P, c_int32, _P, c_int32,
+                                                         _P]),
+    "mmrec_spmm_plan_desc_fill": (c_int32, [_P, c_int32, c_int32, c_int32, _P, _P]),
     "mmrec_spmm_row_keys": (c_int32, [_P, _P, _P, c_int32, c_int32, c_int32, _P, _P, _P]),
     "mmrec_spmm_plan_count": (c_int32, [_P, c_int32, c_int32, _P, _P]),
     "mmrec_spmm_plan_fill": (c_int32, [_P, c_int32, c_int32, _P, _P]),
diff --git a/mmrec_amd/csrc/spmm.hip b/mmrec_amd/csrc/spmm.hip
--- a/mmrec_amd/csrc/spmm.hip
+++ b/mmrec_amd/csrc/spmm.hip
@@ -40,6 +40,25 @@
     const float* val;
     int n_short;
 };
+
+struct LongBlocks {
+    const int4* desc;
+    int n_mid;
+};
+constexpr bool kLongBlocksServed = MMREC_SPMM_CHUNK == 512;
+static_assert(MMREC_SPMM_MID_ROW_MAX == 64, "a mid-length row is four 16-nonzero spans: one per 16-lane group of a wave");
+
+#ifdef MMREC_SPMM_STAMPS
+__device__ unsigned long long* g_spmm_stamps;
+struct BlockStamp {
+    __device__ BlockStamp() {
+        if (threadIdx.x == 0 && g_spmm_stamps) g_spmm_stamps[2 * blockIdx.x] = wall_clock64();
+    }
+    __device__ ~BlockStamp() {
+        if (threadIdx.x == 0 && g_spmm_stamps) g_spmm_stamps[2 * blockIdx.x + 1] = wall_clock64();
+    }
+};
+#endif
 
 template <int DCH, bool LG>
 __device__ __forceinline__ void store_row(const RowEpilogue& ep, int row, int lane16, const float4 (&sum)[DCH]) {
@@ -134,13 +153,16 @@
     }
 }
 
-template <int DCH, bool LG, bool SCHED>
+template <int DCH, bool LG, bool SCHED, bool DESC>
 __global__ __launch_bounds__(256) void spmm_rows_kernel(
     const int32_t* __restrict__ rowptr, const int32_t* __restrict__ colidx,
     const float* __restrict__ vals, const float* __restrict__ X, RowEpilogue ep, int n_rows,
     int long_t, int rows_per_group, const int32_t* __restrict__ long_rows,
     const int32_t* __restrict__ long_chunk_ptr, int n_long, int n_chunks,
-    float* __restrict__ partials, int32_t* __restrict__ tickets, RowSchedule sched) {
+    float* __restrict__ partials, int32_t* __restrict__ tickets, RowSchedule sched, LongBlocks lb) {
+#ifdef MMREC_SPMM_STAMPS
+    BlockStamp stamp;
+#endif
     __shared__ float4 red[16][16 * DCH];
     __shared__ int s_last;
     const int lane16 = threadIdx.x & 15;
@@ -148,14 +170,26 @@
     const float4* X4 = reinterpret_cast<const float4*>(X);
     if ((int)blockIdx.x < n_chunks) {
         const int chunk = blockIdx.x;
-        int lo = 0, hi = n_long;
-        while (hi - lo > 1) {
-            const int mid = (lo + hi) >> 1;
-            if (long_chunk_ptr[mid] <= chunk) lo = mid; else hi = mid;
-        }
-        const int row = long_rows[lo];
-        const int cs = rowptr[row] + (chunk - long_chunk_ptr[lo]) * MMREC_SPMM_CHUNK;
-        const int ce = min(cs + MMREC_SPMM_CHUNK, rowptr[row + 1]);
+        int lo = 0, row, cs, ce;
+        int row_chunks = 0, row_begin = 0;
+        if (DESC) {
+            const int4 r = lb.desc[chunk];
+            row = r.x;
+            cs = r.y;
+            ce = cs + (r.z & (MMREC_SPMM_CHUNK - 1)) + 1;
+            row_chunks = (int)((unsigned)r.z >> 9);
+            lo = r.w;
+            if (row_chunks > 1) row_begin = rowptr[row];
+        } else {
+            int hi = n_long;
+            while (hi - lo > 1) {
+                const int mid = (lo + hi) >> 1;
+                if (long_chunk_ptr[mid] <= chunk) lo = mid; else hi = mid;
+            }
+            row = long_rows[lo];
+            cs = rowptr[row] + (chunk - long_chunk_ptr[lo]) * MMREC_SPMM_CHUNK;
+            ce = min(cs + MMREC_SPMM_CHUNK, rowptr[row + 1]);
+        }
         float4 acc[DCH];
 #pragma unroll
         for (int ch = 0; ch < DCH; ++ch) acc[ch] = f4_zero();
@@ -172,7 +206,7 @@
 #pragma unroll
                 for (int i = 1; i < 16; ++i) t[ch] = f4_add(t[ch], red[i][ch * 16 + lane16]);
             }
-            if (long_chunk_ptr[lo + 1] - long_chunk_ptr[lo] == 1) {
+            if ((DESC ? row_chunks : long_chunk_ptr[lo + 1] - long_chunk_ptr[lo]) == 1) {
                 store_row<DCH, LG>(ep, row, lane16, t);
             } else {
 #pragma unroll
@@ -182,7 +216,14 @@
                 }
             }
         }
-        const int c0 = long_chunk_ptr[lo], c1 = long_chunk_ptr[lo + 1];
+        int c0, c1;
+        if (DESC) {
+            c0 = chunk - (cs - row_begin) / MMREC_SPMM_CHUNK;
+            c1 = c0 + row_chunks;
+        } else {
+            c0 = long_chunk_ptr[lo];
+            c1 = long_chunk_ptr[lo + 1];
+        }
         if (!tickets || c1 - c0 == 1) return;
         if (threadIdx.x < 64) {
             __atomic_signal_fence(__ATOMIC_SEQ_CST);
@@ -199,8 +240,31 @@
         if (threadIdx.x == 0) __hip_atomic_store(tickets + lo, 0, __ATOMIC_RELAXED, __HIP_MEMORY_SCOPE_AGENT);
         return;
     }
+    const int mid_blocks = DESC ? (lb.n_mid + 3) >> 2 : 0;
+    if (DESC && (int)blockIdx.x < n_chunks + mid_blocks) {
+        const int m = ((int)blockIdx.x - n_chunks) * 4 + (threadIdx.x >> 6);
+        if (m >= lb.n_mid) return;
+        const int4 r = lb.desc[n_chunks + m];
+        const int cs = r.y + (g & 3) * 16, ce = r.y + (r.z & (MMREC_SPMM_CHUNK - 1)) + 1;
+        float4 acc[DCH];
+#pragma unroll
+        for (int ch = 0; ch < DCH; ++ch) acc[ch] = f4_zero();
+        gather_span<DCH>(colidx, vals, X4, cs, min(cs + 16, ce), lane16, acc);
+        float4 t[DCH];
+#pragma unroll
+        for (int ch = 0; ch < DCH; ++ch) {
+            t[ch] = acc[ch];
+#pragma unroll
+            for (int k = 1; k < 4; ++k)
+                t[ch] = f4_add(t[ch], make_float4(__shfl_down(acc[ch].x, 16 * k), __shfl_down(acc[ch].y, 16 * k),
+                                                  __shfl_down(acc[ch].z, 16 * k), __shfl_down(acc[ch].w, 16 * k)));
+            t[ch] = f4_add(t[ch], f4_zero());
+        }
+        if ((g & 3) == 0) store_row<DCH, LG>(ep, r.x, lane16, t);
+        return;
+    }
     if (SCHED) {
-        const int slot0 = ((int)blockIdx.x - n_chunks) * 16 * rows_per_group + g;
+        const int slot0 = ((int)blockIdx.x - n_chunks - mid_blocks) * 16 * rows_per_group + g;
 #pragma unroll 1
         for (int i = 0; i < rows_per_group; ++i) {
             const int slot = slot0 + i * 16;
@@ -241,18 +305,27 @@
     reduce_long_row<DCH, false, LG>(partials, c0, c1, long_rows[i], ep, red);
 }
 
-template <int DCH, bool LG = false, bool SCHED = false>
+template <int DCH, bool LG = false, bool SCHED = false, bool DESC = false>
 void launch_spmm(hipStream_t s, int blocks, int nch, const int32_t* rowptr, const int32_t* colidx,
                  const float* vals, const float* X, const RowEpilogue& ep, int n_rows, int long_t,
                  int rows_per_group, const int32_t* long_rows, const int32_t* long_chunk_ptr, int n_long,
-                 float* partials, int32_t* tickets, const RowSchedule& sched = RowSchedule{}) {
+                 float* partials, int32_t* tickets, const RowSchedule& sched = RowSchedule{},
+                 const LongBlocks& lb = LongBlocks{nullptr, 0}) {
+    if constexpr (DESC) {
+        const int grid = nch - lb.n_mid + (lb.n_mid + 3) / 4 + blocks;
+        hipLaunchKernelGGL((spmm_rows_kernel<DCH, LG, SCHED, true>), dim3(grid), dim3(256), 0, s, rowptr, colidx, vals, X, ep,
+                           n_rows, long_t, rows_per_group, long_rows, long_chunk_ptr, n_long, nch - lb.n_mid, partials,
+                           tickets, sched, lb);
+        return;
+    } else {
     if (blocks + nch > 0)
-        hipLaunchKernelGGL((spmm_rows_kernel<DCH, LG, SCHED>), dim3(blocks + nch), dim3(256), 0, s, rowptr, colidx, vals, X,
-                           ep, n_rows, long_t, rows_per_group, long_rows, long_chunk_ptr, n_long, nch, partials, tickets,
-                           sched);
+        hipLaunchKernelGGL((spmm_rows_kernel<DCH, LG, SCHED, false>), dim3(blocks + nch), dim3(256), 0, s, rowptr, colidx, vals,
+                           X, ep, n_rows, long_t, rows_per_group, long_rows, long_chunk_ptr, n_long, nch, partials, tickets,
+                           sched, lb);
     if (!tickets && n_long > 0 && nch > n_long)
         hipLaunchKernelGGL((spmm_long_reduce_kernel<DCH, LG>), dim3(n_long), dim3(256), 0, s, long_rows,
                            long_chunk_ptr, n_long, partials, ep);
+    }
 }
 
 __global__ __launch_bounds__(256) void cos_scale_fwd_kernel(const float* __restrict__ E,
@@ -444,6 +517,94 @@
 }
 }
 
+namespace {
+bool long_blocks_args_ok(const int32_t* long_desc, int32_t n_mid, int32_t n_long, int32_t n_chunks, int32_t n_rows,
+                         const int32_t* long_tickets) {
+    if (!long_desc) return n_mid == 0;
+    if (n_long <= 0 || n_long > n_rows || n_chunks < n_long) return false;
+    if (n_mid < 0 || n_mid > n_long) return false;
+    return n_chunks == n_long || long_tickets;
+}
+
+int spmm_sched_launch(const int32_t* rowptr, const int32_t* colidx, const float* vals, const float* X, float* Y, const float* Z,
+                      const float* acc_in, float* acc_out, int32_t n_rows, int32_t d, float alpha, float beta, float acc_scale,
+                      int32_t long_row_threshold, const int32_t* long_rows, const int32_t* long_chunk_ptr, int32_t n_long,
+                      int32_t n_chunks, float* partials, int32_t* long_tickets, const int32_t* sched_row,
+                      const int32_t* sched_span, const int32_t* sched_col, const float* sched_val, int32_t n_short,
+                      const int32_t* long_desc, int32_t n_mid, mmrec_stream_t stream) {
+    if (d <= 0 || d % MMREC_EMB_DIM || d / MMREC_EMB_DIM > 6) return MMREC_ERR_UNSUPPORTED;
+    if (long_desc && !kLongBlocksServed) return MMREC_ERR_UNSUPPORTED;
+    if (n_rows < 0 || n_long < 0 || n_chunks < 0 || long_row_threshold < 0) return MMREC_ERR_BAD_ARG;
+    if (n_rows == 0) return 0;
+    if (!rowptr || !X || (!Y && !acc_out)) return MMREC_ERR_BAD_ARG;
+    if (acc_out && !acc_in) return MMREC_ERR_BAD_ARG;
+    if (n_long > 0 && (!long_rows || !long_chunk_ptr || !partials || n_chunks <= 0))
+        return MMREC_ERR_BAD_ARG;
+    if (!sched_args_ok(sched_row, sched_span, sched_col, sched_val, n_short, n_rows)) return MMREC_ERR_BAD_ARG;
+    if (!long_blocks_args_ok(long_desc, n_mid, n_long, n_chunks, n_rows, long_tickets)) return MMREC_ERR_BAD_ARG;
+    if (Y == X || acc_out == X) return MMREC_ERR_BAD_ARG;
+    RowEpilogue ep{Z, Y, acc_in, acc_out, alpha, Z ? beta : 0.f, acc_scale, nullptr, nullptr, nullptr};
+    const RowSchedule sched{sched_row, reinterpret_cast<const int2*>(sched_span), sched_col, sched_val, n_short};
+    hipStream_t s = mmrec_stream(stream);
+    const int rows_per_group = MMREC_SPMM_RPG(n_rows);
+    const int blocks = (n_short + 16 * rows_per_group - 1) / (16 * rows_per_group);
+    const LongBlocks lb{reinterpret_cast<const int4*>(long_desc), n_mid};
+    const int long_t = n_long > 0 ? long_row_threshold : INT32_MAX;
+    const int nch = n_long > 0 ? n_chunks : 0;
+    int32_t* tickets = n_long > 0 ? long_tickets : nullptr;
+#define MMREC_SPMM_CASE(D)                                                                                              \
+    case D:                                                                                                             \
+        if (long_desc)                                                                                                  \
+            launch_spmm<D, false, true, true>(s, blocks, nch, rowptr, colidx, vals, X, ep, n_rows, long_t,              \
+                                              rows_per_group, long_rows, long_chunk_ptr, n_long, partials, tickets,     \
+                                              sched, lb);                                                               \
+        else                                                                                                            \
+            launch_spmm<D, false, true>(s, blocks, nch, rowptr, colidx, vals, X, ep, n_rows, long_t, rows_per_group,    \
+                                        long_rows, long_chunk_ptr, n_long, partials, tickets, sched);                   \
+        break;
+    switch (d / MMREC_EMB_DIM) {
+        MMREC_SPMM_CASE(1) MMREC_SPMM_CASE(2) MMREC_SPMM_CASE(3) MMREC_SPMM_CASE(4) MMREC_SPMM_CASE(5)
+        MMREC_SPMM_CASE(6)
+    }
+#undef MMREC_SPMM_CASE
+    MMREC_RETURN_LAUNCH_STATUS();
+}
+
+int spmm_sched_launch_layergcn(const int32_t* rowptr, const int32_t* colidx, const float* vals, const float* X, float* Y,
+                               const float* ego, float* scaled, float* w, const float* acc_in, float* acc_out, int32_t n_rows,
+                               int32_t d, int32_t long_row_threshold, const int32_t* long_rows, const int32_t* long_chunk_ptr,
+                               int32_t n_long, int32_t n_chunks, float* partials, int32_t* long_tickets,
+                               const int32_t* sched_row, const int32_t* sched_span, const int32_t* sched_col,
+                               const float* sched_val, int32_t n_short, const int32_t* long_desc, int32_t n_mid,
+                               mmrec_stream_t stream) {
+    if (d != MMREC_EMB_DIM) return MMREC_ERR_UNSUPPORTED;
+    if (long_desc && !kLongBlocksServed) return MMREC_ERR_UNSUPPORTED;
+    if (n_rows < 0 || n_long < 0 || n_chunks < 0 || long_row_threshold < 0) return MMREC_ERR_BAD_ARG;
+    if (n_rows == 0) return 0;
+    if (!rowptr || !X || !ego || !scaled || !w) return MMREC_ERR_BAD_ARG;
+    if (n_long > 0 && (!long_rows || !long_chunk_ptr || !partials || n_chunks <= 0)) return MMREC_ERR_BAD_ARG;
+    if (!sched_args_ok(sched_row, sched_span, sched_col, sched_val, n_short, n_rows)) return MMREC_ERR_BAD_ARG;
+    if (!long_blocks_args_ok(long_desc, n_mid, n_long, n_chunks, n_rows, long_tickets)) return MMREC_ERR_BAD_ARG;
+    if (Y == X || scaled == X || acc_out == X) return MMREC_ERR_BAD_ARG;
+    RowEpilogue ep{nullptr, Y, acc_in, acc_out, 1.f, 0.f, 1.f, ego, scaled, w};
+    const RowSchedule sched{sched_row, reinterpret_cast<const int2*>(sched_span), sched_col, sched_val, n_short};
+    hipStream_t s = mmrec_stream(stream);
+    const int rows_per_group = MMREC_SPMM_RPG(n_rows);
+    const int blocks = (n_short + 16 * rows_per_group - 1) / (16 * rows_per_group);
+    const LongBlocks lb{reinterpret_cast<const int4*>(long_desc), n_mid};
+    const int long_t = n_long > 0 ? long_row_threshold : INT32_MAX;
+    const int nch = n_long > 0 ? n_chunks : 0;
+    int32_t* tickets = n_long > 0 ? long_tickets : nullptr;
+    if (long_desc)
+        launch_spmm<1, true, true, true>(s, blocks, nch, rowptr, colidx, vals, X, ep, n_rows, long_t, rows_per_group, long_rows,
+                                         long_chunk_ptr, n_long, partials, tickets, sched, lb);
+    else
+        launch_spmm<1, true, true>(s, blocks, nch, rowptr, colidx, vals, X, ep, n_rows, long_t, rows_per_group, long_rows,
+                                   long_chunk_ptr, n_long, partials, tickets, sched);
+    MMREC_RETURN_LAUNCH_STATUS();
+}
+}
+
 extern "C" int mmrec_spmm_csr_sched_f32(const int32_t* rowptr, const int32_t* colidx, const float* vals,
                                         const float* X, float* Y, const float* Z, const float* acc_in,
                                         float* acc_out, int32_t n_rows, int32_t d, float alpha, float beta,
@@ -452,34 +613,9 @@
                                         int32_t n_long, int32_t n_chunks, float* partials, int32_t* long_tickets,
                                         const int32_t* sched_row, const int32_t* sched_span, const int32_t* sched_col,
                                         const float* sched_val, int32_t n_short, mmrec_stream_t stream) {
-    if (d <= 0 || d % MMREC_EMB_DIM || d / MMREC_EMB_DIM > 6) return MMREC_ERR_UNSUPPORTED;
-    if (n_rows < 0 || n_long < 0 || n_chunks < 0 || long_row_threshold < 0) return MMREC_ERR_BAD_ARG;
-    if (n_rows == 0) return 0;
-    if (!rowptr || !X || (!Y && !acc_out)) return MMREC_ERR_BAD_ARG;
-    if (acc_out && !acc_in) return MMREC_ERR_BAD_ARG;
-    if (n_long > 0 && (!long_rows || !long_chunk_ptr || !partials || n_chunks <= 0))
-        return MMREC_ERR_BAD_ARG;
-    if (!sched_args_ok(sched_row, sched_span, sched_col, sched_val, n_short, n_rows)) return MMREC_ERR_BAD_ARG;
-    if (Y == X || acc_out == X) return MMREC_ERR_BAD_ARG;
-    RowEpilogue ep{Z, Y, acc_in, acc_out, alpha, Z ? beta : 0.f, acc_scale, nullptr, nullptr, nullptr};
-    const RowSchedule sched{sched_row, reinterpret_cast<const int2*>(sched_span), sched_col, sched_val, n_short};
-    hipStream_t s = mmrec_stream(stream);
-    const int rows_per_group = MMREC_SPMM_RPG(n_rows);
-    const int blocks = (n_short + 16 * rows_per_group - 1) / (16 * rows_per_group);
-    const int long_t = n_long > 0 ? long_row_threshold : INT32_MAX;
-    const int nch = n_long > 0 ? n_chunks : 0;
-    int32_t* tickets = n_long > 0 ? long_tickets : nullptr;
-#define MMREC_SPMM_CASE(D)                                                                                      \
-    case D:                                                                                                     \
-        launch_spmm<D, false, true>(s, blocks, nch, rowptr, colidx, vals, X, ep, n_rows, long_t, rows_per_group, \
-                                    long_rows, long_chunk_ptr, n_long, partials, tickets, sched);               \
-        break;
-    switch (d / MMREC_EMB_DIM) {
-        MMREC_SPMM_CASE(1) MMREC_SPMM_CASE(2) MMREC_SPMM_CASE(3) MMREC_SPMM_CASE(4) MMREC_SPMM_CASE(5)
-        MMREC_SPMM_CASE(6)
-    }
-#undef MMREC_SPMM_CASE
-    MMREC_RETURN_LAUNCH_STATUS();
+    return spmm_sched_launch(rowptr, colidx, vals, X, Y, Z, acc_in, acc_out, n_rows, d, alpha, beta, acc_scale,
+                             long_row_threshold, long_rows, long_chunk_ptr, n_long, n_chunks, partials, long_tickets, sched_row,
+                             sched_span, sched_col, sched_val, n_short, nullptr, 0, stream);
 }
 
 extern "C" int mmrec_spmm_csr_sched_f32_layergcn(const int32_t* rowptr, const int32_t* colidx, const float* vals,
@@ -490,24 +626,37 @@
                                                  float* partials, int32_t* long_tickets, const int32_t* sched_row,
                                                  const int32_t* sched_span, const int32_t* sched_col,
                                                  const float* sched_val, int32_t n_short, mmrec_stream_t stream) {
-    if (d != MMREC_EMB_DIM) return MMREC_ERR_UNSUPPORTED;
-    if (n_rows < 0 || n_long < 0 || n_chunks < 0 || long_row_threshold < 0) return MMREC_ERR_BAD_ARG;
-    if (n_rows == 0) return 0;
-    if (!rowptr || !X || !ego || !scaled || !w) return MMREC_ERR_BAD_ARG;
-    if (n_long > 0 && (!long_rows || !long_chunk_ptr || !partials || n_chunks <= 0)) return MMREC_ERR_BAD_ARG;
-    if (!sched_args_ok(sched_row, sched_span, sched_col, sched_val, n_short, n_rows)) return MMREC_ERR_BAD_ARG;
-    if (Y == X || scaled == X || acc_out == X) return MMREC_ERR_BAD_ARG;
-    RowEpilogue ep{nullptr, Y, acc_in, acc_out, 1.f, 0.f, 1.f, ego, scaled, w};
-    const RowSchedule sched{sched_row, reinterpret_cast<const int2*>(sched_span), sched_col, sched_val, n_short};
-    hipStream_t s = mmrec_stream(stream);
-    const int rows_per_group = MMREC_SPMM_RPG(n_rows);
-    const int blocks = (n_short + 16 * rows_per_group - 1) / (16 * rows_per_group);
-    const int long_t = n_long > 0 ? long_row_threshold : INT32_MAX;
-    const int nch = n_long > 0 ? n_chunks : 0;
-    int32_t* tickets = n_long > 0 ? long_tickets : nullptr;
-    launch_spmm<1, true, true>(s, blocks, nch, rowptr, colidx, vals, X, ep, n_rows, long_t, rows_per_group, long_rows,
-                               long_chunk_ptr, n_long, partials, tickets, sched);
-    MMREC_RETURN_LAUNCH_STATUS();
+    return spmm_sched_launch_layergcn(rowptr, colidx, vals, X, Y, ego, scaled, w, acc_in, acc_out, n_rows, d, long_row_threshold,
+                                      long_rows, long_chunk_ptr, n_long, n_chunks, partials, long_tickets, sched_row, sched_span,
+                                      sched_col, sched_val, n_short, nullptr, 0, stream);
+}
+
+extern "C" int mmrec_spmm_csr_sched_desc_f32(const int32_t* rowptr, const int32_t* colidx, const float* vals,
+                                             const float* X, float* Y, const float* Z, const float* acc_in,
+                                             float* acc_out, int32_t n_rows, int32_t d, float alpha, float beta,
+                                             float acc_scale, int32_t long_row_threshold,
+                                             const int32_t* long_rows, const int32_t* long_chunk_ptr,
+                                             int32_t n_long, int32_t n_chunks, float* partials, int32_t* long_tickets,
+                                             const int32_t* sched_row, const int32_t* sched_span, const int32_t* sched_col,
+                                             const float* sched_val, int32_t n_short, const int32_t* long_desc,
+                                             int32_t n_mid, mmrec_stream_t stream) {
+    return spmm_sched_launch(rowptr, colidx, vals, X, Y, Z, acc_in, acc_out, n_rows, d, alpha, beta, acc_scale,
+                             long_row_threshold, long_rows, long_chunk_ptr, n_long, n_chunks, partials, long_tickets, sched_row,
+                             sched_span, sched_col, sched_val, n_short, long_desc, n_mid, stream);
+}
+
+extern "C" int mmrec_spmm_csr_sched_desc_f32_layergcn(const int32_t* rowptr, const int32_t* colidx, const float* vals,
+                                                      const float* X, float* Y, const float* ego, float* scaled, float* w,
+                                                      const float* acc_in, float* acc_out, int32_t n_rows, int32_t d,
+                                                      int32_t long_row_threshold, const int32_t* long_rows,
+                                                      const int32_t* long_chunk_ptr, int32_t n_long, int32_t n_chunks,
+                                                      float* partials, int32_t* long_tickets, const int32_t* sched_row,
+                                                      const int32_t* sched_span, const int32_t* sched_col,
+                                                      const float* sched_val, int32_t n_short, const int32_t* long_desc,
+                                                      int32_t n_mid, mmrec_stream_t stream) {
+    return spmm_sched_launch_layergcn(rowptr, colidx, vals, X, Y, ego, scaled, w, acc_in, acc_out, n_rows, d, long_row_threshold,
+                                      long_rows, long_chunk_ptr, n_long, n_chunks, partials, long_tickets, sched_row, sched_span,
+                                      sched_col, sched_val, n_short, long_desc, n_mid, stream);
 }
 
 extern "C" int mmrec_spmm_row_keys(const int32_t* rowptr, const int32_t* colidx, const int32_t* col_degree,
@@ -555,6 +704,44 @@
     return 0;
 }
 
+#ifdef MMREC_SPMM_STAMPS
+extern "C" int mmrec_spmm_lab_set_stamps(void* slots) {
+    return (int)hipMemcpyToSymbol(HIP_SYMBOL(g_spmm_stamps), &slots, sizeof(slots));
+}
+#endif
+
+extern "C" int mmrec_spmm_plan_desc_fill(const int32_t* rowptr_host, int32_t n_rows, int32_t long_row_threshold,
+                                         int32_t mid_row_max, int32_t* long_desc, int32_t* n_mid) {
+    if (!rowptr_host || !long_desc || !n_mid || n_rows < 0 || long_row_threshold < 0) return MMREC_ERR_BAD_ARG;
+    if (mid_row_max > MMREC_SPMM_MID_ROW_MAX) return MMREC_ERR_BAD_ARG;
+    if (!kLongBlocksServed) return MMREC_ERR_UNSUPPORTED;
+    const int32_t mid_max = mid_row_max > long_row_threshold ? mid_row_max : long_row_threshold;
+    int64_t at = 0;
+    int32_t nm = 0;
+    for (int pass = 0; pass < 2; ++pass) {
+        int32_t lo = 0;
+        for (int32_t r = 0; r < n_rows; ++r) {
+            const int32_t s = rowptr_host[r], deg = rowptr_host[r + 1] - s;
+            if (deg <= long_row_threshold) continue;
+            if ((deg <= mid_max) == (pass == 1)) {
+                const int32_t nch = (deg + MMREC_SPMM_CHUNK - 1) / MMREC_SPMM_CHUNK;
+                for (int32_t c = 0; c < nch; ++c, ++at) {
+                    const int32_t b = s + c * MMREC_SPMM_CHUNK;
+                    const int32_t len = (deg - c * MMREC_SPMM_CHUNK < MMREC_SPMM_CHUNK) ? deg - c * MMREC_SPMM_CHUNK : MMREC_SPMM_CHUNK;
+                    long_desc[4 * at + 0] = r;
+                    long_desc[4 * at + 1] = b;
+                    long_desc[4 * at + 2] = (int32_t)((uint32_t)(len - 1) | ((uint32_t)nch << 9));
+                    long_desc[4 * at + 3] = lo;
+                }
+                nm += pass;
+            }
+            ++lo;
+        }
+    }
+    *n_mid = nm;
+    return 0;
+}
+
 extern "C" int mmrec_cos_scale_fwd_f32(const float* E, const float* Ego, float* Out, float* w,
                                        float* acc, int32_t n_rows, int32_t d, mmrec_stream_t stream) {
     if (d != MMREC_EMB_DIM) return MMREC_ERR_UNSUPPORTED;
diff --git a/mmrec_amd/hip_ops.py b/mmrec_amd/hip_ops.py
--- a/mmrec_amd/hip_ops.py
+++ b/mmrec_amd/hip_ops.py
@@ -31,6 +31,17 @@
     import os
     forced = os.environ.get("MMREC_SPMM_KEY_DEG_MAX")
     return int(forced) if forced else SPMM_KEY_DEG_MAX
+
+
+SPMM_MID_ROW_MAX = 64
+
+
+def spmm_long_blocks():
+    import os
+    how = os.environ.get("MMREC_SPMM_LONG_BLOCKS") or "desc"
+    if how not in ("mid", "desc", "off"):
+        raise _lib.MMRecHipError("MMREC_SPMM_LONG_BLOCKS must be mid, desc or off, got %r" % how)
+    return how
 
 
 TOPK_MAX = 128
@@ -89,7 +100,7 @@
 class CsrGraph:
 
     def __init__(self, rowptr, colidx, vals, n_rows, n_cols, symmetric=False,
-                 long_row_threshold=LONG_ROW_DEFAULT, rowptr_host=None, row_schedule=None):
+                 long_row_threshold=LONG_ROW_DEFAULT, rowptr_host=None, row_schedule=None, long_blocks=None):
         self.rowptr = _chk(rowptr, torch.int32, "rowptr", 1)
         self.colidx = _chk(colidx, torch.int32, "colidx", 1)
         self.vals = _chk(vals, torch.float32, "vals", 1)
@@ -100,6 +111,9 @@
                                       else long_row_threshold)
         self._t = self if symmetric else None
         self.row_schedule = bool(self.n_cols > ROW_SCHEDULE_MIN_COLS if row_schedule is None else row_schedule)
+        self.long_blocks = spmm_long_blocks() if long_blocks is None else long_blocks
+        if self.long_blocks not in ("mid", "desc", "off"):
+            raise _lib.MMRecHipError("long_blocks must be mid, desc or off, got %r" % (long_blocks,))
         self._plan(rowptr_host)
 
     def _plan(self, rowptr_host):
@@ -129,8 +143,18 @@
             self.max_row_chunks = 1
         self._partials = {}
         self.sched = None
+        self.long_desc, self.n_mid = None, 0
         if self.row_schedule:
             self._plan_schedule()
+            how = self.long_blocks
+            if self.n_long > 0 and how != "off":
+                desc = np.empty((self.n_chunks, 4), dtype=np.int32)
+                n_mid = ctypes.c_int32(0)
+                _lib.check(lib.mmrec_spmm_plan_desc_fill(rp.ctypes.data_as(ctypes.c_void_p), self.n_rows, self.long_row_threshold,
+                                                         SPMM_MID_ROW_MAX if how == "mid" else 0,
+                                                         desc.ctypes.data_as(ctypes.c_void_p), ctypes.byref(n_mid)),
+                           "spmm_plan_desc_fill")
+                self.long_desc, self.n_mid = torch.from_numpy(desc).to(dev), n_mid.value
 
     def _plan_schedule(self):
         lib = _lib.load()
@@ -242,7 +266,8 @@
         dev = self.rowptr.device
         return CsrGraph(torch.from_numpy(rph).to(dev), self.colidx[s:e].contiguous(),
                         self.vals[s:e].contiguous(), r1 - r0, self.n_cols,
-                        long_row_threshold=self.long_row_threshold, rowptr_host=rph, row_schedule=self.row_schedule)
+                        long_row_threshold=self.long_row_threshold, rowptr_host=rph, row_schedule=self.row_schedule,
+                        long_blocks=self.long_blocks)
 
 
 def _mode_labels(rows, lab_c, n_rows, n_labels):
@@ -355,12 +380,14 @@
                 raise _lib.MMRecHipError("%s must be [>=%d, %d]" % (nm, g.n_rows, d))
     sc = g.scheduled(d)
     if sc is not None:
-        g.checked(lib.mmrec_spmm_csr_sched_f32(_p(g.rowptr), _p(g.colidx), _p(g.vals), _p(X), _p(Y), _p(Z),
-                                               _p(acc_in), _p(acc_out), g.n_rows, d, float(alpha),
-                                               float(beta), float(acc_scale), g.long_row_threshold,
-                                               _p(g.long_rows), _p(g.long_chunk_ptr), g.n_long, g.n_chunks,
-                                               _p(g.partials_for(d)), _p(g.long_tickets), _p(sc["row"]), _p(sc["span"]),
-                                               _p(sc["col"]), _p(sc["val"]), sc["n_short"], _stream()), "spmm_csr_sched_f32")
+        args = (_p(g.rowptr), _p(g.colidx), _p(g.vals), _p(X), _p(Y), _p(Z), _p(acc_in), _p(acc_out), g.n_rows, d, float(alpha),
+                float(beta), float(acc_scale), g.long_row_threshold, _p(g.long_rows), _p(g.long_chunk_ptr), g.n_long,
+                g.n_chunks, _p(g.partials_for(d)), _p(g.long_tickets), _p(sc["row"]), _p(sc["span"]), _p(sc["col"]),
+                _p(sc["val"]), sc["n_short"])
+        if g.long_desc is not None and g.long_tickets is not None:
+            g.checked(lib.mmrec_spmm_csr_sched_desc_f32(*args, _p(g.long_desc), g.n_mid, _stream()), "spmm_csr_sched_desc_f32")
+        else:
+            g.checked(lib.mmrec_spmm_csr_sched_f32(*args, _stream()), "spmm_csr_sched_f32")
         return Y if Y is not None else acc_out
     g.checked(lib.mmrec_spmm_csr_f32(_p(g.rowptr), _p(g.colidx), _p(g.vals), _p(X), _p(Y), _p(Z),
                                      _p(acc_in), _p(acc_out), g.n_rows, d, float(alpha),
@@ -671,7 +698,11 @@
                     _p(acc) if layer > 0 else None, _p(acc), g.n_rows, EMB_DIM, g.long_row_threshold, _p(g.long_rows),
                     _p(g.long_chunk_ptr), g.n_long, g.n_chunks, _p(g.partials_for(EMB_DIM)), _p(g.long_tickets))
             sc = g.scheduled(EMB_DIM)
-            if sc is not None:
+            if sc is not None and g.long_desc is not None and g.long_tickets is not None:
+                g.checked(lib.mmrec_spmm_csr_sched_desc_f32_layergcn(*args, _p(sc["row"]), _p(sc["span"]), _p(sc["col"]),
+                                                                     _p(sc["val"]), sc["n_short"], _p(g.long_desc), g.n_mid,
+                                                                     _stream()), "spmm_sched_desc_layergcn")
+            elif sc is not None:
                 g.checked(lib.mmrec_spmm_csr_sched_f32_layergcn(*args, _p(sc["row"]), _p(sc["span"]), _p(sc["col"]), _p(sc["val"]),
                                                                 sc["n_short"], _stream()), "spmm_sched_layergcn")
             else:
```

Result: no change. 31.71 billion (median of 6 runs) (+0.9%).
